# jamshed/CaPS-SA

Measured on AMD Instinct MI355X. Metric: suffixes/sec (SA+LCP build), higher is better.
Workload: dtype u32

## Files before the change

### caps-sa_amd/csrc/kernels.h

```cpp
#pragma once
#include "kernel_lang.h"
#include "text.h"

namespace caps {

#ifndef CAPS_TILE_E
#define CAPS_TILE_E 4096
#endif
#ifndef CAPS_TILE_NT
#define CAPS_TILE_NT 1024
#endif
#ifndef CAPS_TILE_WAVES
#define CAPS_TILE_WAVES 8
#endif
#ifndef CAPS_LOCK_K
#define CAPS_LOCK_K 4
#endif
constexpr uint32_t TILE_E = CAPS_TILE_E;
constexpr uint32_t TILE_NT = CAPS_TILE_NT;
constexpr uint32_t TILE_EPT = TILE_E / TILE_NT;
constexpr uint32_t LOCK_K = CAPS_LOCK_K < TILE_EPT ? CAPS_LOCK_K : TILE_EPT;
#define TILE_WAVES_PER_SIMD CAPS_TILE_WAVES
#ifdef CAPS_NO_WAVES_BOUND
#undef LAUNCH_BOUNDS2
// ... 557 lines not shown
#else
    constexpr uint32_t BPT = NBINS / TILE_NT;
    static_assert(BPT >= 1 && BPT * TILE_NT == NBINS, "counters per thread");
    __shared__ uint32_t wave_tot[TILE_NT / 64];
    const uint32_t tid = threadIdx.x, lane = tid & 63, wv = tid >> 6;
    uint32_t v[BPT], sum = 0;
    UNROLL
    for (uint32_t i = 0; i < BPT; ++i) { v[i] = h[tid * BPT + i]; sum += v[i]; }
    uint32_t x = sum;
#define CAPS_DPP_ADD(ctrl, rows) x += (uint32_t)__builtin_amdgcn_update_dpp(0, (int)x, ctrl, rows, 0xF, false)
    CAPS_DPP_ADD(0x111, 0xF);
    CAPS_DPP_ADD(0x112, 0xF);
    CAPS_DPP_ADD(0x114, 0xF);
    CAPS_DPP_ADD(0x118, 0xF);
    CAPS_DPP_ADD(0x142, 0xA);
    CAPS_DPP_ADD(0x143, 0xC);
#undef CAPS_DPP_ADD
    if (lane == 63) wave_tot[wv] = x;
    SYNC_LDS();
    uint32_t run = x - sum;
    if (TILE_NT / 64 <= 16) {
        const uint32_t wt = lane < TILE_NT / 64 ? wave_tot[lane] : 0u;
        uint32_t ws = wt;
#define CAPS_DPP_ADD(ctrl) ws += (uint32_t)__builtin_amdgcn_update_dpp(0, (int)ws, ctrl, 0xF, 0xF, false)
        CAPS_DPP_ADD(0x111);
        CAPS_DPP_ADD(0x112);
        CAPS_DPP_ADD(0x114);
        CAPS_DPP_ADD(0x118);
#undef CAPS_DPP_ADD
        const int wvs = __builtin_amdgcn_readfirstlane((int)wv);
        run += (uint32_t)__builtin_amdgcn_readlane((int)ws, wvs) - (uint32_t)__builtin_amdgcn_readlane((int)wt, wvs);
    } else {
        for (uint32_t w = 0; w < wv; ++w) run += wave_tot[w];
    }
    UNROLL
    for (uint32_t i = 0; i < BPT; ++i) { h[tid * BPT + i] = run; run += v[i]; }
    if (tid == TILE_NT - 1) h[NBINS] = run;
    SYNC_LDS();
#endif
}
DEV_INLINE void block_exclusive_scan_bins(KCTX uint32_t* hist) { block_exclusive_scan<TILE_BINS_>(KCTX_PASS hist); }

template <typename idx_t> struct FinalOut {
    idx_t* sa = nullptr;
    idx_t* lcp = nullptr;
    uint64_t* first_key = nullptr;
    uint64_t* last_key = nullptr;
    idx_t* first_sa = nullptr;
    idx_t* last_sa = nullptr;
};

#ifdef CAPS_EMUL
extern "C" void caps_emul_count_tile(bool fast, bool known_range);
extern "C" void caps_emul_count_tile2(bool two_level_ok);
extern "C" void caps_emul_count_tile3(bool equalised_ok);
#endif
constexpr uint32_t TILE_BINS = TILE_BINS_;
#ifndef CAPS_TILE_BIN_LIMIT
#define CAPS_TILE_BIN_LIMIT 48
#endif
#ifndef CAPS_EQ_BIN_LIMIT
#define CAPS_EQ_BIN_LIMIT 128
#endif
constexpr uint32_t TILE_BIN_LIMIT = CAPS_TILE_BIN_LIMIT;
constexpr uint32_t EQ_BIN_LIMIT = CAPS_EQ_BIN_LIMIT;

template <typename idx_t>
DEV_INLINE uint64_t lcp_capped(uint32_t l, uint64_t n, idx_t a, idx_t b)
{
    if (sizeof(idx_t) == 4) {
        const uint32_t room = (uint32_t)n - (uint32_t)(a > b ? a : b);
        return l < room ? l : room;
    }
    const uint64_t room = n - (uint64_t)(a > b ? a : b);
    return l < room ? l : room;
}
template <int BITS, bool RUNS, typename idx_t>
DEV_INLINE uint64_t tile_pair_lcp(const uint32_t* __restrict__ P, uint64_t n, uint64_t ka, idx_t a, uint64_t kb, idx_t b, uint32_t)
{
    const uint64_t x = ka ^ kb;
    if (x) return lcp_capped<idx_t>((uint32_t)caps_clz64(x) / BITS, n, a, b);
    return pair_lcp<BITS, RUNS>(P, n, ka, (uint64_t)a, kb, (uint64_t)b);
}
template <int BITS, bool RUNS, typename idx_t>
DEV_INLINE uint64_t tile_pair_lcp(const uint32_t* __restrict__ P, uint64_t n, uint32_t ka, idx_t a, uint32_t kb, idx_t b, uint32_t cs)
{
    return pair_lcp32<BITS, RUNS>(P, n, ka, (uint64_t)a, kb, (uint64_t)b, cs);
}

template <typename idx_t> HD idx_t tie_sentinel() { return (idx_t)~(idx_t)0; }
template <int BITS, bool RUNS, typename idx_t>
DEV_INLINE uint64_t deferring_pair_lcp(const uint32_t* __restrict__ P, uint64_t n, uint64_t* __restrict__ bflag, uint32_t g, uint64_t ka, idx_t a,
                                       uint64_t kb, idx_t b)
{
    if (bflag && ka == kb) { bflag[g] = 1; return (uint64_t)tie_sentinel<idx_t>(); }
    return tile_pair_lcp<BITS, RUNS>(P, n, ka, a, kb, b, 0u);
}

#if defined(CAPS_PHASE_CLOCK) && !defined(CAPS_EMUL)
__device__ unsigned long long caps_phase_clock[32];
#define PHASE_T0() unsigned long long pc_t_ = clock64()
#define PHASE_MARK(i) do { const unsigned long long t_ = clock64(); if (threadIdx.x == 0) atomicAdd(&caps_phase_clock[i], t_ - pc_t_); pc_t_ = clock64(); } while (0)
#else
#define PHASE_T0() ((void)0)
#define PHASE_MARK(i) ((void)0)
#endif

#if defined(CAPS_EQ_CHECK) && !defined(CAPS_EMUL)
__device__ unsigned int caps_eq_check[64];
#define EQ_OK(ok, id) ((ok) ? true : (atomicAdd(&caps_eq_check[id], 1u), false))
#else
#define EQ_OK(ok, id) (true)
#endif
#define EQ_CHK(ok, id) ((void)EQ_OK((ok), (id)))

DEV_INLINE const uint64_t* tile_src(const uint64_t* in, const uint64_t* out, bool from_out) { return from_out ? out : in; }
DEV_INLINE const uint32_t* tile_src(const uint32_t* in, const uint64_t*, bool) { return in; }

#define TILE_SORT_PROLOGUE                                                                                      \
    const uint32_t b = K_BLOCK_IDX;                                                                             \
    if (b >= sd.tile_off[sd.G]) return;                                                                         \
    const uint32_t g = sd.tile_rec[b].g;                                                                          \
    const TileInfo t = tile_info(sd, b);                                                                        \
    const uint64_t start = t.s0 + (uint64_t)t.tl * TILE_E;                                                      \
    const uint32_t cnt = (uint32_t)(t.s1 - start < TILE_E ? t.s1 - start : TILE_E);                             \
     \
     \
    const bool with_lcp = lcp_mode != 0 && (t.s1 - t.s0) <= TILE_E;                                             \
     \
     \
    const bool direct = with_lcp && fin.sa != nullptr;                                                          \
     \
     \
     \
     \
     \
     \
    const uint64_t in0 = slot_cap ? (uint64_t)g * slot_cap : start;
#define TILE_OUTGROWN (slot_cap != 0 && t.s1 - t.s0 > (uint64_t)slot_cap)

#define TILE_SRC_KEY in_key
#define TILE_SRC_SA in_sa
#define TILE_SORT_LOAD                                                                                          \
    PAR(tid) {                                                                                                  \
        if (tid == 0) { kmm[0] = ~0ull; kmm[1] = 0; flag[0] = 0; }                                              \
        for (uint32_t i = tid; i <= TILE_BINS; i += K_BLOCK_DIM) hist[i] = 0;                                   \
        UNROLL                                                                                                  \
        for (uint32_t k = 0; k < TILE_EPT; ++k) {                                                               \
            const uint32_t e = tid + k * TILE_NT;                                                               \
            if (e < cnt) {                                                                                      \
                uint64_t key;                                                                                   \
                idx_t sa;                                                                                       \
                if (FROM_TEXT) {                                                                                \
                    key = window64<BITS>(P, text_base + start + e);                                             \
                    sa = (idx_t)(text_base + start + e);                                                        \
                } else if (TILE_KEYS_FROM_TEXT) {    \
                    sa = STREAM_LOAD(&TILE_SRC_SA[in0 + e]);                                                    \
                    key = window64<BITS>(P, (uint64_t)sa);                                                      \
                } else {                                                                                        \
                    key = STREAM_LOAD(&TILE_SRC_KEY[in0 + e]);                                                  \
                    sa = STREAM_LOAD(&TILE_SRC_SA[in0 + e]);                                                    \
                }                                                                                               \
                TL(rk, tid, k) = (decltype(TL(rk, tid, k) + 0))key;                                             \
                TL(rs, tid, k) = sa;                                                                            \
            }                                                                                                   \
        }                                                                                                       \
    }

#define TILE_SYNC() SYNC()
#define TILE_SORT_RANGE                                                                                         \
    const bool known_range = seg_map != nullptr;                                                                \
    if (!known_range) {                                                                                         \
        TILE_SYNC();                                                                       \
        PAR(tid) {                                                                                              \
            uint64_t mn = ~0ull, mx = 0;                                                                        \
            UNROLL                                                                                              \
            for (uint32_t k = 0; k < TILE_EPT; ++k) {                                                           \
                const uint32_t e = tid + k * TILE_NT;                                                           \
                if (e < cnt) {                                                                                  \
                    const uint64_t key = (uint64_t)TL(rk, tid, k);                                              \
                    mn = key < mn ? key : mn;                                                                   \
                    mx = key > mx ? key : mx;                                                                   \
                }                                                                                               \
            }                                                                                                   \
            BLOCK_MINMAX_U64(&kmm[0], &kmm[1], mn, mx);                                                         \
        }                                                                                                       \
    }                                                                                                           \
    TILE_SYNC();                                                                                                \
    const BucketParams tb = known_range ? seg_map[g] : make_bucket_params(kmm[0], kmm[1], TILE_BINS);

#define TILE_SORT_PLACE_FINAL                                                                                   \
    PAR(tid) {                                                                                                  \
        UNROLL                                                                                                  \
        for (uint32_t k = 0; k < TILE_EPT; ++k) {                                                               \
            const uint32_t e = tid + k * TILE_NT;                                                               \
            if (e < cnt) {                                                                                      \
                const uint32_t d = TL(rd, tid, k);                                                              \
                skey[d] = TL(rk, tid, k);                                                                       \
                ssa[d] = TL(rs, tid, k);                                                                        \
            }                                                                                                   \
        }                                                                                                       \
    }                                                                                                           \
    TILE_SYNC();

#define TILE_SORT_EMIT TILE_SORT_EMIT_(0u)
#define TILE_EMIT_LCP_(ka, a, kb, b) tile_pair_lcp<BITS, TILE_RUNS>(P, n, ka, a, kb, b, TILE_KEY_SHIFT)
#define TILE_SORT_EMIT_(OV)                                                                                     \
    PAR(tid) {                                                                                                  \
        UNROLL                                                                                                  \
        for (uint32_t k = 0; k < TILE_EPT; ++k) {                                                               \
            const uint32_t e = tid + k * TILE_NT;                                                               \
            if (e < cnt) {                                                                                      \
                const uint64_t key = skey[e];                                                                   \
                const idx_t sa = ssa[e];                                                                        \
                uint64_t l = 0;                                                                                 \
                if (with_lcp && e) {                                                                            \
                    const uint32_t ov_ = (OV);                                                                  \
                    l = ov_ ? ov_ : TILE_EMIT_LCP_(skey[e - 1], ssa[e - 1], skey[e], sa);                          \
                }                                                                                               \
                if (direct) {                                                                                   \
                    STREAM_STORE(&fin.sa[start + e], sa);                                                       \
                    STREAM_STORE(&fin.lcp[start + e], (idx_t)l);                                                \
                    if (e == 0) { fin.first_key[g] = key; fin.first_sa[g] = sa; }                               \
                    if (e == cnt - 1) { fin.last_key[g] = key; fin.last_sa[g] = sa; }                           \
                } else {                                                                                        \
                    out_key[start + e] = key;                                                                   \
                    out_sa[start + e] = sa;                                                                     \
                    if (with_lcp) out_lcp[start + e] = (idx_t)l;                                                \
                }                                                                                               \
            }                                                                                                   \
        }                                                                                                       \
    }

template <typename idx_t, int BITS, bool FROM_TEXT, typename KT = uint64_t>
GLOBAL_FN LAUNCH_BOUNDS2(TILE_NT, TILE_WAVES_PER_SIMD) tile_sort_kernel(KCTX SegDesc sd, const uint32_t* __restrict__ P, uint64_t n,
                                                  uint64_t text_base, uint32_t lcp_mode, uint32_t slot_cap, const KT* in_key,
                                                  const idx_t* in_sa, uint64_t* out_key, idx_t* out_sa, idx_t* out_lcp,
                                                  FinalOut<idx_t> fin, const BucketParams* __restrict__ seg_map,
                                                  uint32_t* __restrict__ redo, const uint8_t* __restrict__ kshift)
{
    constexpr bool TILE_RUNS = false;
    constexpr bool K32 = sizeof(KT) == 4;
    constexpr bool TILE_KEYS_FROM_TEXT = false;
    static_assert(!K32 || !FROM_TEXT, "32-bit keys come from the slots of level B");
    TILE_SORT_PROLOGUE
    const uint32_t TILE_KEY_SHIFT = K32 ? kshift[g] : 0u;
    const uint32_t tie_from = K32 ? (TILE_KEY_SHIFT + 32u) / BITS : TextTraits<BITS>::KCH;
    SHARED_ARRAY(KT, skey, TILE_E);
    SHARED_ARRAY(idx_t, ssa, TILE_E);
    SHARED_ARRAY(uint32_t, hist, TILE_BINS + 1);
    SHARED_ARRAY(uint64_t, kmm, 2);
    SHARED_ARRAY(uint32_t, flag, 1);
    constexpr bool SLOT_ORDER = sizeof(idx_t) == 4;
    SHARED_ARRAY(uint16_t, sbin, SLOT_ORDER ? TILE_E : 1);
    SHARED_ARRAY(uint16_t, perm, SLOT_ORDER ? TILE_E : 1);
    TL_DECL(KT, rk, TILE_EPT);
    TL_DECL(idx_t, rs, TILE_EPT);
    TL_DECL(uint32_t, rd, TILE_EPT);
    TL_DECL(uint32_t, rb, TILE_EPT);

    PHASE_T0();
    TILE_SORT_LOAD
    TILE_SORT_RANGE
    PHASE_MARK(0);
    bool fast = cnt > 1 && tb.range > 0;
    if (fast) {
        PAR(tid) {
            UNROLL
            for (uint32_t k = 0; k < TILE_EPT; ++k) {
                const uint32_t e = tid + k * TILE_NT;
                if (e < cnt) {
                    const uint32_t bin = bucket_of(tb, TL(rk, tid, k));
                    const uint32_t r = FETCH_ADD_U32(&hist[bin], 1u);
                    if (r >= TILE_BIN_LIMIT) flag[0] = 1;
                    TL(rb, tid, k) = bin;
                    TL(rd, tid, k) = r;
                }
            }
        }
        SYNC();
        fast = flag[0] == 0;
        PHASE_MARK(1);
    }
    if (cnt == 1) {
        PAR(tid) { if (tid == 0) { skey[0] = TL(rk, tid, 0); ssa[0] = TL(rs, tid, 0); } }
        SYNC();
        fast = true;
    } else if (fast) {
        block_exclusive_scan_bins(KCTX_PASS hist);
        PHASE_MARK(2);
        PAR(tid) {
            UNROLL
            for (uint32_t k = 0; k < TILE_EPT; ++k) {
                const uint32_t e = tid + k * TILE_NT;
                if (e < cnt) {
                    const uint32_t slot = hist[TL(rb, tid, k)] + TL(rd, tid, k);
                    skey[slot] = TL(rk, tid, k);
                    ssa[slot] = TL(rs, tid, k);
                    if (SLOT_ORDER) sbin[slot] = (uint16_t)TL(rb, tid, k);
                    else TL(rd, tid, k) = slot;
                }
            }
        }
        SYNC();
        PHASE_MARK(3);
        PAR(tid) {
            UNROLL
            for (uint32_t k = 0; k < TILE_EPT; ++k) {
                const uint32_t e = tid + k * TILE_NT;
                if (e < cnt) {
                    const uint32_t slot = SLOT_ORDER ? e : TL(rd, tid, k), bin = SLOT_ORDER ? (uint32_t)sbin[slot] : TL(rb, tid, k);
                    const uint32_t bs = hist[bin], be = hist[bin + 1];
                    const uint64_t key = SLOT_ORDER ? (uint64_t)skey[slot] : (uint64_t)TL(rk, tid, k);
                    uint32_t less = 0;
                    for (uint32_t j = bs; j < be; ++j) {
                        const uint64_t kj = skey[j];
                        less += kj < key ? 1u : 0u;
                        if (kj == key && j != slot) {
                            const uint64_t sa = SLOT_ORDER ? (uint64_t)ssa[slot] : (uint64_t)TL(rs, tid, k);
                            const uint32_t c = suffix_less_tie_bounded<BITS>(P, n, (uint64_t)ssa[j], sa, tie_from);
                            if (c == 2u) flag[0] = 1;
                            less += c & 1u;
                        }
                    }
                    if (SLOT_ORDER) RACY_STORE_U16(&perm[bs + less], (uint16_t)slot);
                    else TL(rd, tid, k) = bs + less;
                }
            }
        }
        SYNC();
        fast = flag[0] == 0;
        PHASE_MARK(4);
        if (fast && !SLOT_ORDER) {
            TILE_SORT_PLACE_FINAL
            PHASE_MARK(5);
        }
    }
#ifdef CAPS_EMUL
    caps_emul_count_tile(fast, known_range);
#endif
    if (!fast) {
        PAR(tid) { if (tid == 0) redo[1 + FETCH_ADD_U32(&redo[0], 1u)] = b; }
        return;
    }
    if (SLOT_ORDER && cnt > 1) {
        PAR(tid) {
            UNROLL
            for (uint32_t k = 0; k < TILE_EPT; ++k) {
                const uint32_t e = tid + k * TILE_NT;
                if (e < cnt) {
                    const uint32_t sl = perm[e];
                    const KT key = skey[sl];
                    const idx_t sa = ssa[sl];
                    uint64_t l = 0;
                    if (with_lcp && e) { const uint32_t sp = perm[e - 1]; l = TILE_EMIT_LCP_(skey[sp], ssa[sp], key, sa); }
                    if (direct) {
                        STREAM_STORE(&fin.sa[start + e], sa);
                        STREAM_STORE(&fin.lcp[start + e], (idx_t)l);
                        if (e == 0) { fin.first_key[g] = key; fin.first_sa[g] = sa; }
                        if (e == cnt - 1) { fin.last_key[g] = key; fin.last_sa[g] = sa; }
                    } else {
                        out_key[start + e] = key;
                        out_sa[start + e] = sa;
                        if (with_lcp) out_lcp[start + e] = (idx_t)l;
                    }
                }
            }
        }
    } else {
        TILE_SORT_EMIT
    }
    PHASE_MARK(6);
}

GLOBAL_FN LAUNCH_BOUNDS(256) hot_tiles_kernel(KCTX SegDesc sd, uint32_t slot_cap, TileInfo* __restrict__ hot)
{
    PAR(tid) {
        const uint32_t nt = sd.tile_off[sd.G];
        const uint32_t i = K_BLOCK_IDX * K_BLOCK_DIM + tid;
        if (i < nt) {
            TileInfo t = sd.tile_rec[i];
            if (t.s1 - t.s0 > (uint64_t)slot_cap) { t.s1 = t.s0; t.tl = 0; }
            hot[i] = t;
        }
    }
}

GLOBAL_FN LAUNCH_BOUNDS(256) queue_all_tiles_kernel(KCTX SegDesc sd, uint32_t* __restrict__ redo)
{
    PAR(tid) {
        const uint32_t nt = sd.tile_off[sd.G];
        const uint32_t i = K_BLOCK_IDX * K_BLOCK_DIM + tid;
        if (i < nt) redo[1 + i] = i;
        if (i == 0) redo[0] = nt;
    }
}

#ifndef CAPS_EQ_ROUNDS
#define CAPS_EQ_ROUNDS 2
#endif
constexpr uint32_t EQ_ROUNDS = CAPS_EQ_ROUNDS;
#ifndef CAPS_TIE_G1
#define CAPS_TIE_G1 8
#endif
#ifndef CAPS_TIE_LIST_MAX
#define CAPS_TIE_LIST_MAX 2
#endif
constexpr uint32_t TIE_G1 = CAPS_TIE_G1;
constexpr uint32_t TIE_G2 = 64;
constexpr uint32_t TIE_LIST_CAP = TILE_E / 8;
constexpr uint32_t TIE_LIST_MAX = CAPS_TIE_LIST_MAX;
constexpr uint32_t TIE_DEEP_CAP = 64;
constexpr uint32_t TIE_VDEEP_CAP = 32;
constexpr uint32_t TIE_BIG_CAP = 1024;
constexpr uint32_t TIE_BIG_LANES = 64;
constexpr uint32_t EQ_FRAC_BITS = 13;
static_assert((uint64_t)TILE_BINS_ << EQ_FRAC_BITS <= (1u << 24), "positions fit 24 bits");

DEV_INLINE uint32_t eq_pos(const BucketParams& bp, uint64_t key)
{
    const uint32_t top = (bp.B << EQ_FRAC_BITS) - 1u;
    if (key <= bp.kmin) return 0;
    const uint64_t d = key - bp.kmin;
    if (d >= bp.range) return top;
    const uint32_t d32 = (uint32_t)((d << bp.shift) >> 32);
    const uint64_t prod = (uint64_t)d32 * bp.m;
    const uint32_t sh = 32u + bp.post;
    const uint32_t x = (uint32_t)(sh >= EQ_FRAC_BITS ? prod >> (sh - EQ_FRAC_BITS) : prod << (EQ_FRAC_BITS - sh));
    return x < top ? x : top;
}

DEV_INLINE uint32_t eq_big_lcp(const uint16_t* vslot, const uint32_t* vlcp, uint32_t cnt, uint32_t e)
{
    uint32_t l = 0;
    for (uint32_t q = 0; q < cnt && q < TIE_VDEEP_CAP; ++q)
        if (vslot[q] == e) l = vlcp[q];
    return l;
}

template <int BITS, bool TEXT, typename idx_t>
DEV_INLINE uint64_t eq_emit_lcp(const uint32_t* __restrict__ P, uint64_t n, uint64_t ka, idx_t a, uint64_t kb, idx_t b, uint32_t* lost, bool test_drop)
{
    if (TEXT) return pair_lcp<BITS, false>(P, n, ka, (uint64_t)a, kb, (uint64_t)b);
    const uint64_t x = ka ^ kb;
    if (x == 0) {
#ifdef CAPS_EMUL
        if (!test_drop) { std::fprintf(stderr, "eq_emit_lcp: neighbours %llu, %llu with equal keys and no lcp from the tie phases\n", (unsigned long long)a, (unsigned long long)b); std::abort(); }
#endif
        *lost = 1;
    }
    return lcp_capped<idx_t>(x ? (uint32_t)caps_clz64(x) / BITS : TextTraits<BITS>::KCH, n, a, b);
}

#ifndef CAPS_EQ_WAVES
#define CAPS_EQ_WAVES TILE_WAVES_PER_SIMD
// ... 1058 lines not shown
        PAR(tid) {
            const uint32_t x = tid & 31, y = tid >> 5;
            for (uint32_t yy = y; yy < 32; yy += 8)
                if (r0 + yy < rows && c0 + x < cols) tile[yy * 33 + x] = in[(uint64_t)(r0 + yy) * cols + c0 + x];
        }
        SYNC();
        PAR(tid) {
            const uint32_t x = tid & 31, y = tid >> 5;
            for (uint32_t yy = y; yy < 32; yy += 8)
                if (c0 + yy < cols && r0 + x < rows) out[(uint64_t)(c0 + yy) * rows + r0 + x] = tile[x * 33 + yy];
        }
        SYNC();
    }
}

template <typename idx_t>
DEV_INLINE uint32_t run_of(const idx_t* row, uint32_t lo, uint32_t hi, uint64_t x)
{
    while (lo < hi) {
        const uint32_t mid = (lo + hi + 1) >> 1;
        if ((uint64_t)row[mid] <= x) lo = mid; else hi = mid - 1;
    }
    return lo;
}

template <typename idx_t>
GLOBAL_FN LAUNCH_BOUNDS(256) runs_plan_kernel(KCTX SegDesc sd, const idx_t* __restrict__ rulerT, uint32_t G1,
                                              uint32_t* __restrict__ first_run)
{
    PAR(tid) {
        const uint64_t b = (uint64_t)K_BLOCK_IDX * K_BLOCK_DIM + tid;
        if (b < sd.tile_off[sd.G]) {
            const uint32_t j = sd.tile_rec[b].g;
            const TileInfo t = tile_info(sd, (uint32_t)b);
            first_run[b] = run_of<idx_t>(rulerT + (uint64_t)j * G1, 0u, G1 - 1, (uint64_t)t.tl * TILE_E);
        }
    }
}

#define RUNS_TILE_SETUP                                                                                         \
    const uint32_t run_a = FROM_RUNS ? rsrc.first_run[b] : 0u;                                                  \
    const uint32_t run_b = !FROM_RUNS ? 0u : (start + cnt >= t.s1) ? rsrc.G1 - 1 : rsrc.first_run[b + 1];       \
    const uint32_t run_ns = run_b - run_a + 1;                                                                  \
    const bool runs_staged = run_ns <= TILE_E;                                                                  \
    const idx_t* run_rowR = rsrc.rulerT + (uint64_t)g * rsrc.G1;                                                \
    const idx_t* run_rowA = rsrc.PmT + (uint64_t)g * rsrc.G1;                                                   \
    const uint64_t run_x0 = start - t.s0;                                                                       \
    (void)run_a; (void)run_b; (void)run_ns; (void)runs_staged; (void)run_rowR; (void)run_rowA; (void)run_x0;

#define RUNS_STAGE(tid)                                                                                         \
    if (runs_staged)                                                                                            \
        for (uint32_t k = tid; k < run_ns; k += K_BLOCK_DIM) {                                                  \
            const idx_t r = run_rowR[run_a + k];                                                                \
            lrow[k] = r;                                                                                        \
            lsrc[k] = rsrc.sub_start[run_a + k] + (uint64_t)run_rowA[run_a + k] - (uint64_t)r;                  \
        }

template <typename idx_t>
DEV_INLINE uint64_t run_source(const RunSrc<idx_t>& rsrc, bool staged, const idx_t* lrow, const uint64_t* lsrc, uint32_t ns,
                               const idx_t* rowR, const idx_t* rowA, uint32_t ga, uint32_t gb, uint64_t x)
{
    if (staged) return lsrc[run_of<idx_t>(lrow, 0u, ns - 1, x)] + x;
    const uint32_t r = run_of<idx_t>(rowR, ga, gb, x);
    return rsrc.sub_start[r] + (uint64_t)rowA[r] + (x - (uint64_t)rowR[r]);
}

constexpr int SRC_ARRAYS = 0, SRC_TEXT = 1, SRC_RUNS = 2;

#ifndef CAPS_BUCKET_EIGHTHS
#define CAPS_BUCKET_EIGHTHS 7
#endif
#ifndef CAPS_SCATTER_SWZ
#define CAPS_SCATTER_SWZ 1
#endif
#ifndef CAPS_COLLATE_SWZ
#define CAPS_COLLATE_SWZ 0
#endif
#ifndef CAPS_TILE_SWZ
#define CAPS_TILE_SWZ 0
#endif
constexpr uint32_t BUCKET_TARGET = (TILE_E * CAPS_BUCKET_EIGHTHS) / 8;
constexpr uint32_t BUCKET_LDS = TILE_BINS_;

DEV_INLINE void key32_range(uint64_t& kmin, uint64_t& kmax, bool kmin_exclusive, uint32_t cs)
{
    const uint64_t lo = kmin_exclusive ? kmin + 1 : kmin;
    if (lo > kmax || (kmin_exclusive && kmin == ~0ull)) { kmin = kmax = 0; return; }
    kmin = key32_of(lo, cs);
    kmax = key32_of(kmax, cs);
}

GLOBAL_FN LAUNCH_BOUNDS(256) bucket_plan_kernel(KCTX const uint64_t* __restrict__ seg_start, const uint64_t* __restrict__ seg_end,
                                                uint32_t G, uint32_t range_mode,
                                                const uint64_t* __restrict__ pkey, uint32_t part_off, uint32_t part_total,
                                                uint32_t enable, uint32_t fine, uint32_t sub,
                                                BucketParams* __restrict__ bp, uint64_t* __restrict__ segB,
                                                const uint8_t* __restrict__ gshift)
{
    PAR(tid) {
        const uint32_t g = K_BLOCK_IDX * K_BLOCK_DIM + tid;
        if (g < G) {
            const uint32_t parent = g / sub, first = parent * sub;
            uint64_t len = 0;
            for (uint32_t x = 0; x < sub && first + x < G; ++x) len += seg_end_of(seg_start, seg_end, first + x) - seg_start[first + x];
            uint64_t kmin = 0, kmax = ~0ull;
            if (range_mode >= 1) {
                const uint32_t j = part_off + parent;
                if (j > 0) kmin = pkey[j - 1];
                if (j + 1 < part_total) kmax = pkey[j];
                if (range_mode == 2) key32_range(kmin, kmax, j > 0, gshift[j]);
            }
            uint32_t B = 1;
            if (enable && len > TILE_E && kmax > kmin) B = (uint32_t)((len + BUCKET_TARGET - 1) / BUCKET_TARGET);
            if (sub > 1 && B < 2) B = 2;
            if (fine > 1 && B > 1 && B <= BUCKET_LDS) {
                const uint32_t k = BUCKET_LDS / B < fine ? BUCKET_LDS / B : fine;
                B *= k;
            }
            const BucketParams q = make_bucket_params(kmin, kmax, B);
            bp[g] = q;
            segB[g] = (g % sub == sub - 1 || g == G - 1) ? B : 0;
        }
    }
}

GLOBAL_FN LAUNCH_BOUNDS(256) bucket_group_kernel(KCTX uint32_t G, const uint64_t* __restrict__ segB, const uint64_t* __restrict__ bstart,
                                                 const uint64_t* __restrict__ fsegB, const uint64_t* __restrict__ fstart,
                                                 const uint64_t* __restrict__ fcount, uint64_t* __restrict__ count,
                                                 uint32_t* __restrict__ gfirst)
{
    SHARED_ARRAY(uint64_t, fc, BUCKET_LDS);
    for (uint32_t g = K_BLOCK_IDX; g < G; g += K_GRID_DIM) {
        const uint32_t B = (uint32_t)segB[g], F = (uint32_t)fsegB[g];
        const uint64_t b0 = bstart[g], f0 = fstart[g];
        if (B > BUCKET_LDS || F <= B || F > BUCKET_LDS) {
            PAR(tid) {
                for (uint32_t i = tid; i < B; i += K_BLOCK_DIM) { count[b0 + i] = i < F ? fcount[f0 + i] : 0; gfirst[b0 + i] = i; }
            }
            continue;
        }
        PAR(tid) { for (uint32_t f = tid; f < F; f += K_BLOCK_DIM) fc[f] = fcount[f0 + f]; }
        SYNC();
        PAR(tid) {
            if (tid == 0) {
                uint64_t cap = TILE_E, total = 0;
                for (uint32_t f = 0; f < F; ++f) total += fc[f];
                for (uint64_t lo = TILE_E, hi = total > TILE_E ? total : TILE_E;;) {
                    const uint64_t c_try = lo == TILE_E ? lo : (lo + hi) / 2;
                    uint32_t need = 1;
                    uint64_t run = 0;
                    for (uint32_t f = 0; f < F; ++f) {
                        const uint64_t c = fc[f];
                        if (run > 0 && run + c > c_try) { ++need; run = 0; }
                        run += c;
                    }
                    if (need <= B) { cap = c_try; hi = c_try; if (c_try == TILE_E) break; }
                    else lo = c_try + 1;
                    if (lo >= hi) { cap = hi; break; }
                }
                uint32_t gi = 0;
                uint64_t sum = 0;
                gfirst[b0] = 0;
                for (uint32_t f = 0; f < F; ++f) {
                    const uint64_t c = fc[f];
                    if (sum > 0 && sum + c > cap && gi + 1 < B) {
                        count[b0 + gi] = sum;
                        ++gi;
                        gfirst[b0 + gi] = f;
                        sum = 0;
                    }
                    sum += c;
                }
                count[b0 + gi] = sum;
                for (uint32_t i = gi + 1; i < B; ++i) { count[b0 + i] = 0; gfirst[b0 + i] = F; }
            }
        }
        SYNC();
    }
}

GLOBAL_FN LAUNCH_BOUNDS(256) bucket_ranges_kernel(KCTX const uint64_t* __restrict__ bstart, uint32_t G,
                                                  const BucketParams* __restrict__ bps, const uint64_t* __restrict__ pkey,
                                                  uint32_t range_mode, uint32_t part_off, uint32_t part_total, uint32_t sub,
                                                  BucketParams* __restrict__ tile_map,
                                                  const BucketParams* __restrict__ fbps, const uint32_t* __restrict__ gfirst,
                                                  const uint8_t* __restrict__ gshift, uint8_t* __restrict__ kshift)
{
    PAR(tid) {
        const uint64_t i = (uint64_t)K_BLOCK_IDX * K_BLOCK_DIM + tid;
        if (i < bstart[G]) {
            uint32_t a = 0, b = G;
            while (b - a > 1) {
                const uint32_t mid = (a + b) / 2;
                if (bstart[mid] <= i) a = mid; else b = mid;
            }
            const uint32_t g = a;
            const BucketParams bp = bps[g];
            uint64_t kmin = 0, kmax = ~0ull;
            if (range_mode >= 1) {
                const uint32_t j = part_off + g / sub;
                if (j > 0) kmin = pkey[j - 1];
                if (j + 1 < part_total) kmax = pkey[j];
                if (range_mode == 2) { key32_range(kmin, kmax, j > 0, gshift[j]); kshift[i] = gshift[j]; }
            }
            const uint32_t bk = (uint32_t)(i - bstart[g]);
            const double range1 = (double)(kmax - kmin) + 1.0;
            uint64_t l = kmin, h = kmax;
            if (bp.B > 1) {
                uint32_t lo = bk, hi = bk + 1, div = bp.B;
                if (gfirst) {
                    div = fbps[g].B;
                    lo = gfirst[i];
                    hi = bk + 1 < bp.B ? gfirst[i + 1] : div;
                    if (hi <= lo) hi = lo + 1;
                }
                const double dl = (double)lo / (double)div * range1, dh = (double)hi / (double)div * range1;
                if (lo > 0) l = kmin + (uint64_t)dl;
                if (hi < div) h = kmin + (uint64_t)dh;
                if (h < l) h = l;
            }
            tile_map[i] = make_bucket_params(l, h, TILE_BINS);
        }
    }
}

constexpr uint32_t TEXT_WIN = TILE_E / 4 + 24;
constexpr uint32_t SPLIT_LUT_BITS = TILE_E >= 4096 ? 12 : TILE_E >= 256 ? 8 : 4;
constexpr uint32_t SPLIT_LUT_CELLS = 1u << SPLIT_LUT_BITS;

template <int BITS> HD uint64_t text_win_base(uint64_t pos0) { return pos0 / TextTraits<BITS>::CPW; }

constexpr int MAP_LINEAR = 0, MAP_GROUPED = 1, MAP_SPLIT = 2;
HD uint32_t lds_swz(uint32_t i) { return i ^ ((i >> 4) & 15u) ^ ((i >> 8) & 15u); }
#ifdef CAPS_GA_NO_SWZ
#define GA_SWZ(i) (i)
#else
#define GA_SWZ(i) lds_swz(i)
#endif
constexpr uint32_t COUNT_CHUNK = 8;

template <typename idx_t, int BITS, int SRC, int MAP = MAP_LINEAR>
GLOBAL_FN LAUNCH_BOUNDS(TILE_NT) bucket_count_kernel(KCTX SegDesc sd, const uint32_t* __restrict__ P, uint64_t n_words,
                                                     uint64_t text_base, const uint64_t* __restrict__ in_key, RunSrc<idx_t> rsrc,
                                                     const BucketParams* __restrict__ bps, const uint64_t* __restrict__ bstart,
                                                     uint64_t* __restrict__ count, const uint64_t* __restrict__ split,
                                                     uint32_t split_stride, uint32_t in_sub, uint16_t* __restrict__ bid)
{
    constexpr bool FROM_TEXT = SRC == SRC_TEXT, FROM_RUNS = SRC == SRC_RUNS;
    SHARED_ARRAY(uint32_t, hist, BUCKET_LDS);
    SHARED_ARRAY(uint64_t, stab, MAP == MAP_SPLIT ? BUCKET_LDS : 1);
    SHARED_ARRAY(uint32_t, twin, FROM_TEXT ? TEXT_WIN : 1);
    SHARED_ARRAY(uint64_t, lsrc, FROM_RUNS ? TILE_E : 1);
    SHARED_ARRAY(idx_t, lrow, FROM_RUNS ? TILE_E : 1);
    const uint32_t n_tiles = sd.tile_off[sd.G];
    const uint32_t want = n_tiles / (4u * K_GRID_DIM);
    const uint32_t CH = want < 1u ? 1u : want > COUNT_CHUNK ? COUNT_CHUNK : want;
    const uint32_t n_chunks = (n_tiles + CH - 1) / CH;
    for (uint32_t v = K_BLOCK_IDX; v < n_chunks; v += K_GRID_DIM) {
    uint64_t cur_b0 = ~0ull;
    uint32_t cur_B = 0;
    const uint32_t b_end = (v + 1) * CH < n_tiles ? (v + 1) * CH : n_tiles;
    for (uint32_t b = v * CH; b < b_end; ++b) {
        const uint32_t g = sd.tile_rec[b].g;
        const TileInfo t = tile_info(sd, b);
        const uint64_t start = t.s0 + (uint64_t)t.tl * TILE_E;
        const uint32_t cnt = (uint32_t)(t.s1 - start < TILE_E ? t.s1 - start : TILE_E);
        const BucketParams bp = bps[g];
        const uint64_t b0 = bstart[g];
        if (bp.B == 1) {
            PAR(tid) { if (tid == 0) ATOMIC_ADD_U64(&count[b0], (uint64_t)cnt); }
            continue;
        }
        const bool lds = bp.B <= BUCKET_LDS;
        const uint64_t w0 = text_win_base<BITS>(text_base + start);
        RUNS_TILE_SETUP
        const uint32_t n_split = MAP == MAP_SPLIT ? bp.B - 1 : 0u;
        const uint64_t* tab = MAP == MAP_SPLIT ? split + (uint64_t)(g / in_sub) * split_stride : nullptr;
        const bool fresh = !lds || b0 != cur_b0 || bp.B != cur_B;
        PAR(tid) {
            if (fresh) {
                for (uint32_t i = tid; i < cur_B; i += K_BLOCK_DIM)
                    if (hist[i]) ATOMIC_ADD_U64(&count[cur_b0 + i], (uint64_t)hist[i]);
                if (lds) for (uint32_t i = tid; i < bp.B; i += K_BLOCK_DIM) hist[i] = 0;
                if (MAP == MAP_SPLIT && lds) for (uint32_t i = tid; i < n_split; i += K_BLOCK_DIM) stab[lds_swz(i)] = tab[i];
            }
            if (FROM_TEXT)
// ... 338 lines not shown
                    STREAM_STORE2(&out_key[dst], skey[q]);
                    STREAM_STORE2(&out_sa[dst], ssa[q]);
                }
            }
        }
        if (SPILL) {
            const uint32_t nl = nlong[0];
            for (uint32_t r = 0; r < nl && r < SPILL_LONG_CAP; ++r) {
                const uint64_t at = lr_at[r];
                const idx_t old = lr_old[r];
                const uint32_t c = lr_c[r], bb = lr_b[r];
                for (uint32_t j = tid; j < c; j += K_BLOCK_DIM) { spill.bucket[at + j] = bb; spill.rel[at + j] = (idx_t)(old + j); }
            }
        }
    }
}

template <typename idx_t>
GLOBAL_FN LAUNCH_BOUNDS(256) spill_gather_kernel(KCTX const uint64_t* __restrict__ seg_start, uint32_t NB, uint64_t slot_cap,
                                                 const uint8_t* __restrict__ skip, const uint64_t* __restrict__ slot_key,
                                                 const idx_t* __restrict__ slot_sa, uint64_t* __restrict__ dst_key,
                                                 idx_t* __restrict__ dst_sa)
{
    SHARED_ARRAY(uint32_t, lst, 256);
    SHARED_ARRAY(uint32_t, ln, 1);
    for (uint64_t base = (uint64_t)K_BLOCK_IDX * 256u; base < NB; base += (uint64_t)K_GRID_DIM * 256u) {
        PAR(tid) { if (tid == 0) ln[0] = 0; }
        SYNC();
        PAR(tid) {
            const uint64_t b = base + tid;
            if (b < NB) {
                const uint64_t len = seg_start[b + 1] - seg_start[b];
                if (len > slot_cap || (len && skip && skip[b])) lst[FETCH_ADD_U32(&ln[0], 1u)] = (uint32_t)b;
            }
        }
        SYNC();
        const uint32_t m = ln[0];
        for (uint32_t q = 0; q < m; ++q) {
            const uint32_t b = lst[q];
            const uint64_t s0 = seg_start[b], len = seg_start[b + 1] - s0;
            const uint64_t cnt = len < slot_cap ? len : slot_cap;
            PAR(tid) {
                for (uint64_t i = tid; i < cnt; i += K_BLOCK_DIM) {
                    dst_key[s0 + i] = slot_key[(uint64_t)b * slot_cap + i];
                    dst_sa[s0 + i] = slot_sa[(uint64_t)b * slot_cap + i];
                }
            }
        }
        SYNC();
    }
}

template <typename idx_t>
GLOBAL_FN LAUNCH_BOUNDS(256) spill_place_kernel(KCTX Spill<idx_t> sp, uint64_t cnt, const uint64_t* __restrict__ seg_start,
                                                uint64_t* __restrict__ dst_key, idx_t* __restrict__ dst_sa)
{
    PAR(tid) {
        for (uint64_t i = (uint64_t)K_BLOCK_IDX * K_BLOCK_DIM + tid; i < cnt; i += (uint64_t)K_GRID_DIM * K_BLOCK_DIM) {
            const uint32_t b = sp.bucket[i];
            if (b == ~0u) continue;
            const uint64_t d = seg_start[b] + (uint64_t)sp.rel[i];
            dst_key[d] = sp.key[i];
            dst_sa[d] = sp.sa[i];
        }
    }
}

#ifndef CAPS_GA_TILES
#define CAPS_GA_TILES 4
#endif
constexpr uint32_t GA_TILES = CAPS_GA_TILES;
constexpr uint32_t GA_E = GA_TILES * TILE_E;
constexpr uint32_t GA_EPT = GA_E / TILE_NT;
static_assert(GA_E <= (1u << 14) && BUCKET_LDS <= (1u << 11), "group << 14 | position fits a register");

template <typename idx_t, int BITS, typename KT = uint64_t>
GLOBAL_FN LAUNCH_BOUNDS2(TILE_NT, TILE_WAVES_PER_SIMD) group_scatter_kernel(KCTX const uint32_t* __restrict__ P, uint64_t n_words,
                                                      uint64_t text_base, uint64_t len, const uint64_t* __restrict__ split, uint32_t K1,
                                                      const uint16_t* __restrict__ split_lut, const uint32_t* __restrict__ split_span,
                                                      uint32_t sub, uint64_t slot_cap, idx_t* __restrict__ cursor,
                                                      KT* __restrict__ out_key, idx_t* __restrict__ out_sa,
                                                      uint32_t tile_first, uint32_t tile_stride,
                                                      const uint64_t* __restrict__ region_start, const uint64_t* __restrict__ region_cap,
                                                      const uint8_t* __restrict__ gshift, uint32_t own_lo, uint32_t own_hi)
{
    constexpr bool K32 = sizeof(KT) == 4;
    constexpr uint32_t DROP = ~0u;
    SHARED_ARRAY(uint8_t, scs, K32 ? BUCKET_LDS : 1);
    constexpr uint32_t CPW = TextTraits<BITS>::CPW;
    constexpr uint32_t WIN = GA_E / CPW + 8;
    const idx_t NO_SLOT = (idx_t)~(idx_t)0;
    SHARED_ARRAY(uint32_t, twin, WIN);
    SHARED_ARRAY(uint64_t, stab, BUCKET_LDS);
    SHARED_ARRAY(uint16_t, slut, SPLIT_LUT_CELLS + 2);
    SHARED_ARRAY(uint32_t, hist, TILE_BINS + 1);
    SHARED_ARRAY(idx_t, obase, TILE_BINS);
    SHARED_ARRAY(uint32_t, perm, TILE_E);
    TL_DECL(uint32_t, pk, GA_EPT);
    const uint64_t start = ((uint64_t)tile_first + (uint64_t)K_BLOCK_IDX * tile_stride) * GA_E;
    if (start >= len) return;
    const uint32_t cnt = (uint32_t)(len - start < GA_E ? len - start : GA_E);
    const uint32_t sx = sub > 1 ? K_BLOCK_IDX % sub : 0u;
    const uint32_t n_split = K1 - 1;
    const uint64_t pos0 = text_base + start;
    const uint64_t w0 = pos0 / CPW;
    const uint32_t top = pow2_above(split_span[0]);
    PAR(tid) {
        for (uint32_t i = tid; i <= TILE_BINS; i += K_BLOCK_DIM) hist[i] = 0;
        for (uint32_t i = tid; i < WIN; i += K_BLOCK_DIM) twin[i] = w0 + i < n_words ? P[w0 + i] : 0u;
        for (uint32_t i = tid; i < n_split; i += K_BLOCK_DIM) stab[GA_SWZ(i)] = split[i];
        for (uint32_t i = tid; i <= SPLIT_LUT_CELLS; i += K_BLOCK_DIM) slut[i] = split_lut[i];
        if (K32) for (uint32_t i = tid; i < K1; i += K_BLOCK_DIM) scs[i] = gshift[i];
    }
    SYNC();
    const bool RUN_OF_POS = BITS == 2 && GA_EPT == CPW && pos0 % CPW == 0;
    PAR(tid) {
        uint64_t wA = 0;
        uint32_t wC = 0;
        if (RUN_OF_POS) {
            const uint32_t wi = (uint32_t)(pos0 / CPW - w0) + tid;
            wA = ((uint64_t)twin[wi] << 32) | twin[wi + 1];
            wC = twin[wi + 2];
        }
        UNROLL
        for (uint32_t kk = 0; kk < GA_EPT; kk += 4) {
            uint64_t key[4];
            uint32_t lo[4], hi[4];
            UNROLL
            for (uint32_t j = 0; j < 4; ++j) {
                const uint32_t e = RUN_OF_POS ? tid * GA_EPT + kk + j : tid + (kk + j) * TILE_NT;
                const uint32_t sh = BITS * (kk + j);
                key[j] = e >= cnt ? 0 : !RUN_OF_POS ? window64<BITS>(twin, pos0 + e - w0 * CPW)
                                                    : sh ? (wA << sh) | (uint64_t)(wC >> (32u - sh)) : wA;
                const uint32_t cell = (uint32_t)(key[j] >> (64 - SPLIT_LUT_BITS));
                lo[j] = slut[cell];
                hi[j] = slut[cell + 1];
            }
            for (uint32_t st = top >> 1; st >= 1; st >>= 1) {
                UNROLL
                for (uint32_t j = 0; j < 4; ++j) {
                    const uint32_t idx = lo[j] + st - 1;
                    const uint64_t mk = stab[GA_SWZ(idx < n_split ? idx : (n_split ? n_split - 1 : 0))];
                    if (idx < hi[j] && mk < key[j]) lo[j] += st;
                }
            }
            UNROLL
            for (uint32_t j = 0; j < 4; ++j) {
                const uint32_t e = RUN_OF_POS ? tid * GA_EPT + kk + j : tid + (kk + j) * TILE_NT;
                uint32_t v = DROP;
                if (e < cnt && lo[j] >= own_lo && lo[j] < own_hi) v = (lo[j] << 14) | FETCH_ADD_U32(&hist[lo[j]], 1u);
                TL(pk, tid, kk + j) = v;
            }
        }
    }
    SYNC();
    constexpr uint32_t GPT = (TILE_BINS + TILE_NT - 1) / TILE_NT;
    TL_DECL(idx_t, co, GPT);
    TL_DECL(uint32_t, cc, GPT);
    PAR(tid) {
        UNROLL
        for (uint32_t j = 0; j < GPT; ++j) {
            const uint32_t i = tid + j * TILE_NT;
            const uint32_t c = i < K1 ? hist[i] : 0u;
            TL(cc, tid, j) = c;
            TL(co, tid, j) = 0;
            if (c) TL(co, tid, j) = caps_fetch_add(&cursor[(uint64_t)sx * K1 + i], (idx_t)c);
        }
    }
    block_exclusive_scan_bins(KCTX_PASS hist);
    PAR(tid) {
        UNROLL
        for (uint32_t k = 0; k < GA_EPT; ++k) {
            const uint32_t v = TL(pk, tid, k), g = v >> 14;
            if (v != DROP) TL(pk, tid, k) = (g << 14) | (hist[g] + (v & 0x3FFFu));
        }
        UNROLL
        for (uint32_t j = 0; j < GPT; ++j) {
            const uint32_t i = tid + j * TILE_NT;
            if (i < K1) {
                const uint32_t c = TL(cc, tid, j);
                idx_t ob = 0;
                if (c) {
                    const idx_t old = TL(co, tid, j);
                    const uint64_t st = (uint64_t)(i - own_lo) * sub + sx;
                    const uint64_t r0 = region_start ? region_start[st] - region_start[0] : st * slot_cap, rc = region_start ? region_cap[st] : slot_cap;
                    ob = (uint64_t)old + c <= rc ? (idx_t)(r0 + old) : NO_SLOT;
                }
                obase[i] = ob;
            }
        }
    }
    const uint32_t kept = hist[TILE_BINS];
    for (uint32_t c0 = 0; c0 < kept; c0 += TILE_E) {
        PAR(tid) {
            UNROLL
            for (uint32_t k = 0; k < GA_EPT; ++k) {
                const uint32_t e = RUN_OF_POS ? tid * GA_EPT + k : tid + k * TILE_NT;
                const uint32_t v = TL(pk, tid, k), q = v & 0x3FFFu;
                if (v != DROP && q - c0 < TILE_E) perm[q - c0] = (v & ~0x3FFFu) | e;
            }
        }
        SYNC_LDS();
        PAR(tid) {
            UNROLL
            for (uint32_t k = 0; k < TILE_EPT; ++k) {
                const uint32_t q = c0 + tid + k * TILE_NT;
                if (q < kept) {
                    const uint32_t v = perm[q - c0], g = v >> 14, e = v & 0x3FFFu;
                    const idx_t ob = obase[g];
                    if (ob != NO_SLOT) {
                        const uint64_t dst = (uint64_t)ob + (q - hist[g]);
                        const uint64_t key = window64<BITS>(twin, pos0 + e - w0 * CPW);
                        STREAM_STORE2(&out_key[dst], K32 ? (KT)key32_of(key, scs[g]) : (KT)key);
                        STREAM_STORE2(&out_sa[dst], (idx_t)(pos0 + e));
                    }
                }
            }
        }
        SYNC_LDS();
    }
}

template <typename idx_t>
GLOBAL_FN LAUNCH_BOUNDS(256) stream_report_kernel(KCTX const idx_t* __restrict__ cursor, uint32_t n_streams, uint64_t cap,
                                                  const uint32_t* __restrict__ flag, uint64_t* __restrict__ out,
                                                  const uint64_t* __restrict__ region_cap, uint32_t K1, uint32_t sub, uint32_t own_lo,
                                                  uint32_t own_hi)
{
    PAR(tid) {
        const uint32_t s = K_BLOCK_IDX * K_BLOCK_DIM + tid;
        if (s < n_streams) {
            const uint64_t z = (uint64_t)cursor[s];
            out[s] = z;
            uint64_t room = cap;
            if (region_cap) {
                const uint32_t g = s % K1, sx = s / K1;
                room = g >= own_lo && g < own_hi ? region_cap[(uint64_t)(g - own_lo) * sub + sx] : 0;
            }
            if (z > room) ATOMIC_MAX_U64(&out[n_streams + 1], z);
        }
        if (s == n_streams) out[n_streams] = flag[0];
    }
}

template <typename idx_t>
GLOBAL_FN LAUNCH_BOUNDS(256) widen_kernel(KCTX const idx_t* __restrict__ in, uint64_t cnt, uint64_t* __restrict__ out)
{
    PAR(tid) {
        const uint64_t i = (uint64_t)K_BLOCK_IDX * K_BLOCK_DIM + tid;
        if (i < cnt) out[i] = (uint64_t)in[i];
    }
}

template <typename idx_t>
GLOBAL_FN LAUNCH_BOUNDS(256) unify_kernel(KCTX SegDesc sd, const uint64_t* __restrict__ key1, const idx_t* __restrict__ sa1,
                                          uint64_t* __restrict__ key0, idx_t* __restrict__ sa0)
{
    const uint32_t b = K_BLOCK_IDX;
    if (b >= sd.tile_off[sd.G]) return;
    const TileInfo t = tile_info(sd, b);
    if ((passes_for(t.s1 - t.s0) & 1u) == 0) return;
    const uint64_t start = t.s0 + (uint64_t)t.tl * TILE_E;
    const uint32_t cnt = (uint32_t)(t.s1 - start < TILE_E ? t.s1 - start : TILE_E);
    PAR(tid) {
        for (uint32_t e = tid; e < cnt; e += K_BLOCK_DIM) {
            key0[start + e] = key1[start + e];
            sa0[start + e] = sa1[start + e];
        }
    }
}

template <typename idx_t>
GLOBAL_FN LAUNCH_BOUNDS(256) sample_kernel(KCTX const uint64_t* __restrict__ seg_start, uint32_t G, uint32_t ppp,
                                           const uint64_t* __restrict__ key, const idx_t* __restrict__ sa,
                                           uint64_t* __restrict__ out_key, idx_t* __restrict__ out_sa)
{
    PAR(tid) {
        const uint64_t t = (uint64_t)K_BLOCK_IDX * K_BLOCK_DIM + tid;
        if (t < (uint64_t)G * ppp) {
            const uint32_t g = (uint32_t)(t / ppp), k = (uint32_t)(t % ppp);
            const uint64_t s0 = seg_start[g], len = seg_start[g + 1] - s0;
            const uint64_t at = s0 + ((uint64_t)(2 * k + 1) * len) / (2 * (uint64_t)ppp);
            out_key[t] = key[at];
            out_sa[t] = sa[at];
        }
    }
}

template <typename idx_t>
GLOBAL_FN LAUNCH_BOUNDS(256) pick_pivots_kernel(KCTX const uint64_t* __restrict__ skey, const idx_t* __restrict__ ssa, uint64_t m,
                                                uint32_t p, uint64_t* __restrict__ pkey, idx_t* __restrict__ psa)
{
    PAR(tid) {
        const uint64_t j = (uint64_t)K_BLOCK_IDX * K_BLOCK_DIM + tid;
        if (j + 1 < p) {
            const uint64_t at = ((j + 1) * m) / p;
            pkey[j] = skey[at];
            psa[j] = ssa[at];
        }
    }
}

DEV_INLINE uint64_t mix64(uint64_t x)
{
    x += 0x9E3779B97F4A7C15ull;
    x = (x ^ (x >> 30)) * 0xBF58476D1CE4E5B9ull;
    x = (x ^ (x >> 27)) * 0x94D049BB133111EBull;
    return x ^ (x >> 31);
}

template <typename idx_t, int BITS>
GLOBAL_FN LAUNCH_BOUNDS(256) sample_text_kernel(KCTX const uint32_t* __restrict__ P, uint64_t pos0, uint64_t len, uint64_t m,
                                                uint64_t* __restrict__ out_key, idx_t* __restrict__ out_sa)
{
    PAR(tid) {
        const uint64_t t = (uint64_t)K_BLOCK_IDX * K_BLOCK_DIM + tid;
        if (t < m) {
            const uint64_t q = len / m, r = len % m;
            const uint64_t lo = t * q + (t * r) / m, hi = (t + 1) * q + ((t + 1) * r) / m;
            const uint64_t pos = pos0 + lo + mix64(t) % (hi - lo);
            out_key[t] = window64<BITS>(P, pos);
            out_sa[t] = (idx_t)pos;
        }
    }
}

GLOBAL_FN LAUNCH_BOUNDS(256) group_keys_kernel(KCTX const uint64_t* __restrict__ pkey, uint32_t p, uint32_t PG, uint32_t K1,
                                               uint64_t* __restrict__ gkey, uint32_t* __restrict__ flag)
{
    PAR(tid) {
        const uint32_t j = K_BLOCK_IDX * K_BLOCK_DIM + tid;
        if (j + 2 < p && pkey[j] >= pkey[j + 1]) {
            flag[0] = 1;
            if (j == 0 || pkey[j - 1] != pkey[j]) {
                uint32_t len = 2;
                while (j + len < p - 1 && pkey[j + len] == pkey[j]) ++len;
#ifdef CAPS_EMUL
                if (len > flag[3]) flag[3] = len;
#else
                atomicMax(&flag[3], len);
#endif
            }
        }
        if (j + 1 < K1) gkey[j] = pkey[(uint64_t)(j + 1) * PG - 1];
        if (j + 1 == K1) gkey[j] = ~0ull;
    }
}

GLOBAL_FN LAUNCH_BOUNDS(256) group_shift_kernel(KCTX const uint64_t* __restrict__ gkey, uint32_t K1, uint8_t* __restrict__ gshift)
{
    PAR(tid) {
        const uint32_t g = K_BLOCK_IDX * K_BLOCK_DIM + tid;
        if (g < K1) {
            const uint64_t lo = g ? gkey[g - 1] + 1 : 0, hi = g + 1 < K1 ? gkey[g] : ~0ull;
            const uint64_t x = lo ^ hi;
            const uint32_t c = x ? (uint32_t)caps_clz64(x) : 32u;
            gshift[g] = (uint8_t)(lo > hi ? 0u : c < 32u ? c : 32u);
        }
    }
}


GLOBAL_FN LAUNCH_BOUNDS(256) split_lut_kernel(KCTX const uint64_t* __restrict__ split, uint32_t n_split, uint16_t* __restrict__ lut,
                                              uint32_t* __restrict__ span)
{
    PAR(tid) {
        const uint32_t c = K_BLOCK_IDX * K_BLOCK_DIM + tid;
        if (c <= SPLIT_LUT_CELLS) {
            uint32_t lo = 0, hi = n_split;
            if (c < SPLIT_LUT_CELLS) {
                const uint64_t cell_lo = (uint64_t)c << (64 - SPLIT_LUT_BITS);
                while (lo < hi) { const uint32_t mid = (lo + hi) >> 1; if (split[mid] < cell_lo) lo = mid + 1; else hi = mid; }
            } else lo = n_split;
            lut[c] = (uint16_t)lo;
            if (c < SPLIT_LUT_CELLS) {
                uint32_t a = lo, z = n_split;
                if (c + 1 < SPLIT_LUT_CELLS) {
                    const uint64_t next_lo = (uint64_t)(c + 1) << (64 - SPLIT_LUT_BITS);
                    while (a < z) { const uint32_t mid = (a + z) >> 1; if (split[mid] < next_lo) a = mid + 1; else z = mid; }
                } else a = n_split;
#ifdef CAPS_EMUL
                if (a - lo > span[0]) span[0] = a - lo;
#else
                if (a > lo) atomicMax(&span[0], a - lo);
#endif
            }
        }
    }
}

template <typename idx_t>
GLOBAL_FN LAUNCH_BOUNDS(256) slot_segments_kernel(KCTX const idx_t* __restrict__ sizes, uint32_t K1, uint32_t sub, uint32_t stream_major,
                                                  uint64_t cap, const uint64_t* __restrict__ region_start,
                                                  const uint64_t* __restrict__ region_cap, uint64_t* __restrict__ seg_start,
                                                  uint64_t* __restrict__ seg_end, uint64_t* __restrict__ total)
{
    PAR(tid) {
        const uint32_t G = K1 * sub;
        const uint32_t s = K_BLOCK_IDX * K_BLOCK_DIM + tid;
        if (s < G) {
            const uint64_t z = (uint64_t)sizes[stream_major ? (uint64_t)(s % sub) * K1 + s / sub : s];
            const uint64_t r0 = region_start ? region_start[s] : (uint64_t)s * cap, rc = region_start ? region_cap[s] : cap;
            seg_start[s] = r0;
            seg_end[s] = r0 + (z < rc ? z : rc);
            ATOMIC_ADD_U64(total, z);
            if (z > rc) ATOMIC_MAX_U64(total + 1, z);
        }
        if (s == G) seg_start[s] = region_start ? region_start[G - 1] + region_cap[G - 1] : (uint64_t)G * cap;
    }
}

constexpr double SKEW_MIN = 0.7;

GLOBAL_FN LAUNCH_BOUNDS(256) skew_probe_kernel(KCTX const uint64_t* __restrict__ pkey, uint32_t p, uint32_t PG, uint32_t K1,
                                               uint32_t* __restrict__ flag)
{
    PAR(tid) {
        const uint32_t j = K_BLOCK_IDX * K_BLOCK_DIM + tid;
        if (j < p) {
            const uint32_t g = j / PG, j0 = g * PG, j1 = (j0 + PG < p ? j0 + PG : p);
            if (j1 - j0 >= 2) {
                const double glo = j0 ? (double)pkey[j0 - 1] : 0.0, ghi = j1 < p ? (double)pkey[j1 - 1] : 18446744073709551615.0;
                const double lo = j ? (double)pkey[j - 1] : 0.0, hi = j + 1 < p ? (double)pkey[j] : 18446744073709551615.0;
                if (ghi > glo && (hi - lo) * (double)(j1 - j0) < SKEW_MIN * (ghi - glo)) flag[0] = 1;
            }
        }
    }
}

GLOBAL_FN LAUNCH_BOUNDS(256) knots_kernel(KCTX const uint64_t* __restrict__ skey, uint64_t m, uint64_t NB, uint32_t KPG, uint32_t K1,
                                          uint64_t* __restrict__ knots, uint64_t* __restrict__ gkey)
{
    PAR(tid) {
        const uint64_t k = (uint64_t)K_BLOCK_IDX * K_BLOCK_DIM + tid;
        if (k < NB) {
            uint64_t v = k + 1 < NB ? skey[((k + 1) * m) / NB] : ~0ull;
            if (k + 2 < NB) {
                const uint64_t nx = skey[((k + 2) * m) / NB];
                const uint64_t pv = k ? skey[(k * m) / NB] : 0;
                if (nx == v && (k == 0 ? v > 0 : pv + 1 < v)) --v;
// ... 1190 lines not shown
```

### caps-sa_amd/csrc/pipeline.h

```cpp
#pragma once
#include <algorithm>
#include <cmath>
#include <cstdlib>
#include <cstdio>
#include <limits>
#include <stdexcept>
#include <string>
#include <vector>

#include "kernels.h"
#include "bounded.h"
#include "../../include/caps_sa_hip.h"

#ifndef CAPS_BACKEND_DEFINED
#include "hip_backend.h"
#endif

namespace caps {

template <typename idx_t> struct ElemBuf {
    uint64_t* key = nullptr;
    idx_t* sa = nullptr;
    idx_t* lcp = nullptr;
    size_t region_bytes = 0;
};

struct Arena {
    char* base = nullptr;
    size_t off = 0;
    template <typename T> T* take(size_t count)
    {
        off = (off + 255) & ~size_t(255);
        T* p = base ? reinterpret_cast<T*>(base + off) : nullptr;
        off += count * sizeof(T);
        return p;
    }
};

struct SegBufs {
    uint64_t* seg_start = nullptr;
    uint64_t* seg_end = nullptr;
    uint32_t* tile_off = nullptr;
    TileInfo* tile_rec = nullptr;
    uint64_t* out2 = nullptr;
    uint32_t G = 0;
    SegDesc desc() const { return SegDesc{seg_start, tile_off, tile_rec, G}; }
};

constexpr uint32_t kMaxPasses = 96;

#ifndef CAPS_DIRECT_SUB
#define CAPS_DIRECT_SUB 8
#endif
constexpr uint32_t DIRECT_SUB = CAPS_DIRECT_SUB;
#ifndef CAPS_BUCKET_Q_32NDS
#define CAPS_BUCKET_Q_32NDS 24
#endif
#ifndef CAPS_QUANTILE_SPB
#define CAPS_QUANTILE_SPB 64
#endif
constexpr uint32_t BUCKET_Q = (TILE_E * CAPS_BUCKET_Q_32NDS) / 32;
constexpr uint32_t QUANTILE_SPB = CAPS_QUANTILE_SPB;

#ifndef CAPS_EQ_FINE
#define CAPS_EQ_FINE 16
#endif
constexpr uint32_t EQ_FINE = CAPS_EQ_FINE;

struct BucketBufs {
    BucketParams* params = nullptr;
    uint64_t* segB = nullptr;
    uint64_t* bstart = nullptr;
    uint64_t* count = nullptr;
    void* cursor = nullptr;
    uint64_t* scan_tmp = nullptr;
    uint64_t *first_key = nullptr, *last_key = nullptr;
    BucketParams* tile_map = nullptr;
    void *first_sa = nullptr, *last_sa = nullptr;
    SegBufs sub;
    BucketParams* fparams = nullptr;
    uint64_t* fsegB = nullptr;
    uint64_t* fstart = nullptr;
    uint64_t* fcount = nullptr;
    uint32_t* gfirst = nullptr;
    uint8_t* kshift = nullptr;
    uint8_t* skip = nullptr;
    uint64_t* run_list = nullptr;
    uint32_t nb_cap = 0;
    uint64_t tile_cap = 0;
    static uint32_t bucket_bound(uint64_t n_elems, uint32_t G) { return (uint32_t)(n_elems / BUCKET_Q + 2 * (uint64_t)G + 2); }
};

template <typename idx_t> struct Plan {
    uint64_t n = 0;
    int text_bits = 8;
    uint32_t p = 0;
    uint32_t ppp = 0;
    uint64_t m = 0;
    uint64_t tile_cap = 0;
    uint32_t* P = nullptr;
    ElemBuf<idx_t> A, B, SA_, SB_;
    uint64_t* pkey = nullptr;
    idx_t* psa = nullptr;
    idx_t* Pm = nullptr;
    idx_t* ruler = nullptr;
    idx_t* PmT = nullptr;
    idx_t* rulerT = nullptr;
    uint64_t* sizes = nullptr;
    uint64_t* gkey = nullptr;
    uint64_t* dstat = nullptr;
    idx_t* dcur = nullptr;
    uint16_t* glut = nullptr;
    uint8_t* gshift = nullptr;
    uint64_t* knots = nullptr;
    uint64_t* rcap = nullptr;
    uint64_t* rstart = nullptr;
    uint64_t* partial = nullptr;
    SegBufs seg1, seg2, segS;
    TileDesc* desc = nullptr;
    BucketBufs bk;
    uint64_t* pass_elems = nullptr;
    uint32_t* present = nullptr;
    uint8_t* lut = nullptr;
    size_t bytes = 0;
};

inline void effective_params(uint64_t n, uint64_t p_arg, uint32_t* p_eff, uint32_t* ppp)
{
    uint64_t p = p_arg > 0 ? p_arg : 8192;
    if (n / 16 < p) p = n / 16;
    if (p < 2) { *p_eff = (uint32_t)p; *ppp = 0; return; }
    const uint64_t a = (uint64_t)std::ceil(32.0 * std::log((double)n));
    const uint64_t b = n / p - 1;
    *p_eff = (uint32_t)p;
    *ppp = (uint32_t)(a < b ? a : b);
}

template <typename idx_t>
Plan<idx_t> make_plan(uint64_t n, uint64_t p_arg, char* base, int text_bits = 8)
{
    Plan<idx_t> pl;
    pl.n = n;
    pl.text_bits = text_bits;
    effective_params(n, p_arg, &pl.p, &pl.ppp);
    Arena ar;
    ar.base = base;
    const uint64_t nn = n ? n : 1;
    const bool split = pl.p >= 2;
    const uint32_t p = split ? pl.p : 1;
    const uint32_t gseg = std::max<uint32_t>(p, DIRECT_SUB * std::min<uint32_t>(p, BUCKET_LDS));
    pl.m = split ? (uint64_t)p * pl.ppp : 0;
    pl.bk.nb_cap = BucketBufs::bucket_bound(nn, p);
    pl.bk.tile_cap = nn / TILE_E + pl.bk.nb_cap + 2;
    pl.tile_cap = pl.bk.tile_cap;
    pl.P = ar.take<uint32_t>(text_alloc_words(nn, text_bits));
    for (ElemBuf<idx_t>* b : {&pl.A, &pl.B}) {
        b->key = ar.take<uint64_t>(nn);
        const size_t at = ar.off - nn * sizeof(uint64_t);
        b->sa = ar.take<idx_t>(nn);
        b->lcp = ar.take<idx_t>(nn);
        b->region_bytes = ar.off - at;
    }
    auto segs = [&](SegBufs& s, uint32_t G, uint64_t cap) {
        s.G = G;
        s.seg_start = ar.take<uint64_t>((size_t)G + 1);
        s.tile_off = ar.take<uint32_t>((size_t)G + 1);
        s.tile_rec = ar.take<TileInfo>(cap);
        s.out2 = ar.take<uint64_t>(2);
    };
    segs(pl.seg1, p, pl.tile_cap);
    if (split) {
        for (ElemBuf<idx_t>* b : {&pl.SA_, &pl.SB_}) {
            b->key = ar.take<uint64_t>(pl.m);
            b->sa = ar.take<idx_t>(pl.m);
            b->lcp = ar.take<idx_t>(pl.m);
        }
        pl.pkey = ar.take<uint64_t>(p);
        pl.psa = ar.take<idx_t>(p);
        pl.Pm = ar.take<idx_t>((size_t)p * (p + 1));
        pl.ruler = ar.take<idx_t>((size_t)p * p);
        pl.PmT = ar.take<idx_t>((size_t)p * (p + 1));
        pl.rulerT = ar.take<idx_t>((size_t)p * p);
        pl.sizes = ar.take<uint64_t>(p);
        pl.gkey = ar.take<uint64_t>(p);
        pl.dstat = ar.take<uint64_t>(4);
        pl.dcur = ar.take<idx_t>(gseg);
        pl.glut = ar.take<uint16_t>(SPLIT_LUT_CELLS + 2);
        pl.gshift = ar.take<uint8_t>(gseg);
        pl.knots = ar.take<uint64_t>(pl.bk.nb_cap);
        pl.rcap = ar.take<uint64_t>(gseg);
        pl.rstart = ar.take<uint64_t>((size_t)gseg + 1);
        pl.partial = ar.take<uint64_t>((size_t)PART_CHUNKS * p);
        segs(pl.seg2, gseg, pl.tile_cap);
        pl.seg2.G = p;
        pl.seg2.seg_end = ar.take<uint64_t>((size_t)gseg + 1);
        segs(pl.segS, 1, pl.m / TILE_E + 3);
    }
    pl.desc = ar.take<TileDesc>(pl.tile_cap + 1);
    pl.bk.params = ar.take<BucketParams>(gseg);
    pl.bk.segB = ar.take<uint64_t>(gseg);
    pl.bk.bstart = ar.take<uint64_t>((size_t)gseg + 1);
    pl.bk.count = ar.take<uint64_t>(pl.bk.nb_cap);
    pl.bk.cursor = ar.take<idx_t>(pl.bk.nb_cap);
    pl.bk.scan_tmp = ar.take<uint64_t>(2 * ((size_t)pl.bk.nb_cap / SCAN_CHUNK + 2));
    pl.bk.tile_map = ar.take<BucketParams>(pl.bk.nb_cap);
    pl.bk.first_key = ar.take<uint64_t>(pl.bk.nb_cap);
    pl.bk.last_key = ar.take<uint64_t>(pl.bk.nb_cap);
    pl.bk.first_sa = ar.take<idx_t>(pl.bk.nb_cap);
    pl.bk.last_sa = ar.take<idx_t>(pl.bk.nb_cap);
    segs(pl.bk.sub, pl.bk.nb_cap, pl.bk.tile_cap);
    pl.bk.fparams = ar.take<BucketParams>(gseg);
    pl.bk.fsegB = ar.take<uint64_t>(gseg);
    pl.bk.fstart = ar.take<uint64_t>((size_t)gseg + 1);
    pl.bk.fcount = ar.take<uint64_t>((size_t)EQ_FINE * pl.bk.nb_cap);
    pl.bk.gfirst = ar.take<uint32_t>(pl.bk.nb_cap);
    pl.bk.kshift = ar.take<uint8_t>(pl.bk.nb_cap);
    pl.bk.skip = ar.take<uint8_t>(pl.bk.nb_cap);
    pl.bk.run_list = ar.take<uint64_t>(1 + 4 * RUN_BUCKET_MAX);
    pl.pass_elems = ar.take<uint64_t>(kMaxPasses);
    pl.present = ar.take<uint32_t>(16);
    pl.lut = ar.take<uint8_t>(256);
    pl.bytes = ar.off + 256;
    return pl;
}

struct KernelClock {
    std::vector<std::pair<BackendEvent, BackendEvent>> spans;
    std::vector<uint64_t> elems;
};

inline int build_lut(const uint32_t present[8], uint8_t lut[256])
{
    int sigma = 0;
    for (int c = 0; c < 256; ++c) sigma += (present[c >> 5] >> (c & 31)) & 1;
    if (sigma <= 4) {
        for (int c = 0; c < 256; ++c) lut[c] = 0xFF;
        int rank = 0;
        for (int v = -128; v < 128; ++v) {
            const int c = v & 0xFF;
            if ((present[c >> 5] >> (c & 31)) & 1) lut[c] = (uint8_t)rank++;
        }
        return 2;
    }
    for (int c = 0; c < 256; ++c) lut[c] = (uint8_t)(c ^ 0x80);
    return 8;
}

#define CAPS_UNPAREN(...) __VA_ARGS__
#define CAPS_LAUNCH_RUNS(kernel, targs, grid, block, be, ...)                                            \
    do {                                                                                                 \
        if ((be).long_runs) CAPS_LAUNCH((kernel<CAPS_UNPAREN targs, true>), grid, block, be, __VA_ARGS__); \
        else CAPS_LAUNCH((kernel<CAPS_UNPAREN targs, false>), grid, block, be, __VA_ARGS__);             \
    } while (0)

inline void build_run_table(Backend& be, uint32_t* P, uint64_t n, int bits)
{
    const uint64_t entries = run_table_entries(n, bits);
    const uint32_t chunks = (uint32_t)run_table_chunks(entries);
    uint64_t* R = run_table_mut(P, n, bits);
    uint64_t* flag = R - 2;
    uint64_t* longest = R - 1;
    uint64_t* head = R + entries;
    uint64_t* carry = head + chunks;
    be.memset(flag, 0, 2 * sizeof(uint64_t));
    const uint64_t want = (entries + 255) / 256;
    const uint32_t grid = (uint32_t)(want < 16384 ? want : 16384);
    if (bits == 2) CAPS_LAUNCH(run_blocks_kernel<2>, grid, 256, be, (const uint32_t*)P, n, entries, R, flag);
    else CAPS_LAUNCH(run_blocks_kernel<8>, grid, 256, be, (const uint32_t*)P, n, entries, R, flag);
    CAPS_LAUNCH(run_chunk_heads_kernel, chunks, RUN_NT, be, (const uint64_t*)R, entries, (const uint64_t*)flag, head);
    CAPS_LAUNCH(run_carry_kernel, 1, 1024, be, (const uint64_t*)head, chunks, (const uint64_t*)flag, carry);
    CAPS_LAUNCH(run_resolve_kernel, chunks, RUN_NT, be, R, entries, (const uint64_t*)flag, (const uint64_t*)carry,
                (uint32_t)(64 / bits), longest);
    uint64_t longest_host = 0;
    be.d2h(&longest_host, longest, sizeof longest_host);
    be.sync();
    be.long_runs = longest_host >= RUN_LONG;
}

struct AlphabetError : std::length_error { AlphabetError() : std::length_error("the text has more than 4 distinct bytes, the workspace was sized for 2-bit codes") {} };
inline int prepare_text(Backend& be, const uint8_t* dT, uint64_t n, uint32_t* P, uint32_t* present_dev, uint8_t* lut_dev, int arena_bits = 8)
{
    auto alphabet = [&](uint64_t len, uint32_t present[8]) {
        be.memset(present_dev, 0, 16 * sizeof(uint32_t));
        const uint64_t want = (len + 16 * 256 - 1) / (16 * 256);
        const uint32_t grid = (uint32_t)(want < 4096 ? (want ? want : 1) : 4096);
        CAPS_LAUNCH(alphabet_kernel, grid, 256, be, dT, len, present_dev);
        be.d2h(present, present_dev, 8 * sizeof(uint32_t));
        be.sync();
    };
    auto pack = [&](int bits, const uint8_t lut[256], uint32_t* bad) {
        be.h2d(lut_dev, lut, 256);
        const uint64_t n_words = packed_words(n, bits);
        const uint64_t want = (n_words / (bits == 2 ? 1 : 4) + 255) / 256 + 1;
        const uint32_t grid = (uint32_t)(want < 65536 ? want : 65536);
        if (bits == 2) CAPS_LAUNCH(pack_kernel<2>, grid, 256, be, dT, n, (const uint8_t*)lut_dev, P, n_words, bad);
        else CAPS_LAUNCH(pack_kernel<8>, grid, 256, be, dT, n, (const uint8_t*)lut_dev, P, n_words, bad);
    };
    uint32_t present[8];
    uint8_t lut[256];
// ... 26 lines not shown
    const uint32_t chunks = (G + SCAN_CHUNK - 1) / SCAN_CHUNK;
    uint64_t* sums = tmp;
    uint64_t* offs = tmp + chunks + 1;
    CAPS_LAUNCH((block_scan_kernel<OutT>), chunks ? chunks : 1, 1024, be, in, (uint64_t)G, out, sums);
    CAPS_LAUNCH(scan_sizes_kernel, 1, 1024, be, (const uint64_t*)sums, chunks, offs);
    CAPS_LAUNCH((add_offsets_kernel<OutT>), chunks ? chunks : 1, 1024, be, out, (uint64_t)G, (const uint64_t*)offs, chunks);
}

#ifdef CAPS_EMUL
constexpr uint32_t kSmallScan = 48;
#else
constexpr uint32_t kSmallScan = 32768;
#endif

inline void prepare_segments(Backend& be, const SegBufs& s, uint64_t tile_bound, uint64_t* big_tmp = nullptr,
                             uint64_t* big_cnt = nullptr, bool use_end = false, const uint8_t* skip = nullptr)
{
    be.memset(s.out2, 0, 2 * sizeof(uint64_t));
    const uint64_t* send = use_end ? s.seg_end : nullptr;
    if (s.G <= kSmallScan || !big_tmp) {
        CAPS_LAUNCH(seg_prepare_kernel, 1, 1024, be, (const uint64_t*)s.seg_start, send, s.G, s.tile_off, s.out2, skip);
    } else {
        CAPS_LAUNCH(tile_count_kernel, (s.G + 255) / 256, 256, be, (const uint64_t*)s.seg_start, send, s.G, big_cnt, s.out2, skip);
        device_exclusive_scan<uint32_t>(be, big_cnt, s.G, s.tile_off, big_tmp);
        CAPS_LAUNCH(tile_total_kernel, 1, 64, be, (const uint32_t*)s.tile_off, s.G, s.out2);
    }
    const uint32_t grid = (uint32_t)((tile_bound + 255) / 256);
    CAPS_LAUNCH(tile_map_kernel, grid ? grid : 1, 256, be, (const uint64_t*)s.seg_start, send, (const uint32_t*)s.tile_off, s.G, s.tile_rec);
}

inline uint32_t tiles_of(uint64_t len) { return (uint32_t)((len + TILE_E - 1) / TILE_E); }

template <typename idx_t> struct SortResult {
    ElemBuf<idx_t> buf[2];
    uint32_t passes = 0;
    bool skip_finished = false;
    bool unified = false;
    bool k32 = false;
    bool failed = false;
    SegBufs segs;
    struct RunBucket { uint64_t s0, s1, key; };
    std::vector<RunBucket> run_buckets;
    SegBufs run_tables;
    const BucketBufs* run_bk = nullptr;
    TileDesc* run_desc = nullptr;
    uint64_t total = 0;
    uint64_t* defer_flags = nullptr;
    TileDesc* defer_desc = nullptr;
    uint64_t cap = 0;
    mutable bool msd_failed = false;
    KernelClock* finish_clock = nullptr;
    KernelClock* runb_clock = nullptr;
    KernelClock* msd_clock = nullptr;
    mutable uint64_t msd_groups = 0, msd_elems = 0;
    mutable uint32_t msd_levels = 0;
    uint32_t n_tiles = 0;
    FinalOut<idx_t> fin;
    ElemBuf<idx_t> uniform() const { return unified ? buf[0] : buf[passes & 1]; }
    PingPong<idx_t> pingpong() const
    {
        PingPong<idx_t> pp;
        for (int i = 0; i < 2; ++i) { pp.key[i] = buf[i].key; pp.sa[i] = buf[i].sa; pp.lcp[i] = buf[i].lcp; }
        return pp;
    }
};

struct SortOpts {
    bool from_text = false;
    uint64_t text_base = 0;
    bool need_lcp = false;
    bool skip_finished = false;
    bool no_equalise = false;
    const BucketBufs* bk = nullptr;
    uint32_t range_mode = 0;
    const uint64_t* pkey = nullptr;
    uint32_t part_off = 0, part_total = 0;
    bool speculate = false;
    uint32_t* slot_stats = nullptr;
    bool seg_ends = false;
    uint32_t sub = 1;
    const uint64_t* in_key = nullptr;
    const void* in_sa = nullptr;
    const uint8_t* gshift = nullptr;
    bool k32 = false;
    bool keys_only = false;
    bool comparison_only = false;
    bool skewed_keys = false;
    const uint64_t* knots = nullptr;
    uint32_t knots_per_parent = 0;
    bool knots_have_prev = false;
    bool spill_slots = false;
    TileInfo* hot_tile_rec = nullptr;
    uint64_t* spill_stats = nullptr;
    uint64_t in_extent = 0;
    const SegBufs* run_tables = nullptr;
    uint64_t* defer_flags = nullptr;
    const void* runs = nullptr;
    bool unify = false;
    void* final_sa = nullptr;
    void* final_lcp = nullptr;
    struct { uint64_t *first_key, *last_key; void *first_sa, *last_sa; } bnd = {nullptr, nullptr, nullptr, nullptr};
    KernelClock* tile_clock = nullptr;
    KernelClock* merge_clock = nullptr;
    KernelClock* scatter_clock = nullptr;
    KernelClock* count_clock = nullptr;
    uint64_t* pass_counters = nullptr;
};

template <typename idx_t, int BITS>
SortResult<idx_t> segmented_sort(Backend& be, const uint32_t* P, uint64_t n, TileDesc* desc, const SegBufs& s, uint32_t n_tiles,
                                 uint64_t max_len, ElemBuf<idx_t> cur, ElemBuf<idx_t> oth, uint64_t n_elems, const SortOpts& o)
{
    if (o.keys_only) {
        if (o.from_text || o.need_lcp || o.runs) throw std::invalid_argument("a keys-only sort takes (key, index) arrays and emits no LCPs");
        n = 0;
    }
    SortResult<idx_t> r;
    r.buf[0] = cur;
    r.buf[1] = oth;
    r.skip_finished = o.skip_finished;
    r.segs = s;
    r.n_tiles = n_tiles;
    if (n_tiles == 0) return r;
    const bool dbg = std::getenv("CAPS_SA_DEBUG") != nullptr;
    auto mark = [&](const char* what) { if (dbg) { be.sync(); std::fprintf(stderr, "[sort] %s\n", what); } };
    bool from_text = o.from_text;
    const BucketParams* seg_map = nullptr;
    SegBufs segs = s;
    bool skip = o.skip_finished;
    uint32_t slot_cap = 0;
    uint64_t* slot_key = nullptr;
    idx_t* slot_sa = nullptr;
    if (o.bk && (max_len > TILE_E || o.seg_ends)) {
        const BucketBufs& bk = *o.bk;
        const SegDesc psd = s.desc();
        const uint64_t* s_end = o.seg_ends ? (const uint64_t*)s.seg_end : (const uint64_t*)nullptr;
        const bool by_knots = o.knots != nullptr;
        if (by_knots) {
            const uint64_t NB = (uint64_t)(s.G / o.sub) * o.knots_per_parent;
            if (NB > bk.nb_cap) throw std::invalid_argument("more knot buckets than the bucket tables hold");
            CAPS_LAUNCH(knot_plan_kernel, (s.G + 255) / 256, 256, be, s.G, o.sub, o.knots_per_parent, bk.params, bk.segB);
            CAPS_LAUNCH(scan_sizes_kernel, 1, 1024, be, (const uint64_t*)bk.segB, s.G, bk.bstart);
            CAPS_LAUNCH(knot_ranges_kernel, (uint32_t)((NB + 255) / 256), 256, be, o.knots, NB, bk.tile_map, o.knots_have_prev ? 1u : 0u);
        } else {
        CAPS_LAUNCH(bucket_plan_kernel, (s.G + 255) / 256, 256, be, (const uint64_t*)s.seg_start, s_end, s.G, o.range_mode, o.pkey, o.part_off,
                    o.part_total ? o.part_total : s.G, 1u, 1u, o.sub,
                    bk.params, bk.segB, o.gshift);
        CAPS_LAUNCH(scan_sizes_kernel, 1, 1024, be, (const uint64_t*)bk.segB, s.G, bk.bstart);
        CAPS_LAUNCH(bucket_ranges_kernel, (bk.nb_cap + 255) / 256, 256, be, (const uint64_t*)bk.bstart, s.G,
                    (const BucketParams*)bk.params, o.pkey, o.range_mode, o.part_off, o.part_total ? o.part_total : s.G, o.sub,
                    bk.tile_map, (const BucketParams*)nullptr, (const uint32_t*)nullptr, o.gshift, bk.kshift);
        }
        seg_map = bk.tile_map;
        mark("bucket plan");
        const uint32_t pgrid = n_tiles < be.persistent_blocks() ? n_tiles : be.persistent_blocks();
        const bool runs = o.runs != nullptr;
        const RunSrc<idx_t> rsrc = runs ? *static_cast<const RunSrc<idx_t>*>(o.runs) : RunSrc<idx_t>();
        const uint64_t n_words = from_text ? packed_words(n, BITS) : 0;
        const uint64_t tbase = from_text ? o.text_base : 0;
        const uint64_t* src_key = o.in_key ? o.in_key : (const uint64_t*)cur.key;
        const idx_t* src_sa = o.in_key ? static_cast<const idx_t*>(o.in_sa) : (const idx_t*)cur.sa;
        uint16_t* bid = nullptr;
        if (by_knots && o.in_extent && !from_text && !o.runs && oth.region_bytes && !std::getenv("CAPS_SA_NO_BUCKET_IDS")) {
            const size_t room = (size_t)((reinterpret_cast<char*>(oth.key) + oth.region_bytes) - reinterpret_cast<char*>(oth.lcp));
            const uint64_t extent = o.in_key ? o.in_extent : n_elems;
            if (room >= extent * sizeof(uint16_t)) bid = reinterpret_cast<uint16_t*>(oth.lcp);
        }
        auto scatter = [&](const uint64_t* sub_start, uint32_t cap, uint64_t* okey, idx_t* osa, bool grouped = false) {
            const BucketParams* fbps = grouped ? bk.fparams : nullptr;
            const uint32_t* gfirst = grouped ? bk.gfirst : nullptr;
            BackendEvent s0 = be.record();
#define CAPS_SCATTER_LAUNCH(SRC_, MAP_, ikey, isa)                                                                          \
            CAPS_LAUNCH((bucket_scatter_kernel<idx_t, BITS, SRC_, MAP_>), n_tiles, TILE_NT, be, psd, P, n_words, tbase, ikey, isa, rsrc, \
                        (const BucketParams*)bk.params, (const uint64_t*)bk.bstart, sub_start, (uint64_t)cap, static_cast<idx_t*>(bk.cursor),       \
                        okey, osa, fbps, gfirst, o.knots, (const uint16_t*)nullptr, (const uint32_t*)nullptr, 1u, o.knots_per_parent, o.sub, \
                        (const uint16_t*)bid, Spill<idx_t>())
            const uint64_t* nokey = nullptr;
            const idx_t* nosa = nullptr;
            if (from_text) { if (grouped) CAPS_SCATTER_LAUNCH(SRC_TEXT, MAP_GROUPED, nokey, nosa); else CAPS_SCATTER_LAUNCH(SRC_TEXT, MAP_LINEAR, nokey, nosa); }
            else if (runs) { if (grouped) CAPS_SCATTER_LAUNCH(SRC_RUNS, MAP_GROUPED, src_key, src_sa);
                             else CAPS_SCATTER_LAUNCH(SRC_RUNS, MAP_LINEAR, src_key, src_sa); }
            else if (by_knots) CAPS_SCATTER_LAUNCH(SRC_ARRAYS, MAP_SPLIT, src_key, src_sa);
            else { if (grouped) CAPS_SCATTER_LAUNCH(SRC_ARRAYS, MAP_GROUPED, src_key, src_sa);
                   else CAPS_SCATTER_LAUNCH(SRC_ARRAYS, MAP_LINEAR, src_key, src_sa); }
#undef CAPS_SCATTER_LAUNCH
            BackendEvent s1 = be.record();
            if (o.scatter_clock) { o.scatter_clock->spans.push_back({s0, s1}); o.scatter_clock->elems.push_back(n_elems); }
        };
        uint64_t out2[2] = {0, 0};
        auto adopt_buckets = [&]() {
            device_exclusive_scan<uint64_t>(be, bk.count, bk.nb_cap, bk.sub.seg_start, bk.scan_tmp);
        };
        const bool run_buckets = by_knots && o.need_lcp && o.final_sa && bk.skip && !std::getenv("CAPS_SA_NO_RUN_BUCKETS") &&
                                 n < (1ull << RunKey<(int)sizeof(idx_t)>::RB);
        auto bucket_tiles = [&]() {
            segs = bk.sub;
            segs.G = bk.nb_cap;
            uint64_t rl[1 + 4 * RUN_BUCKET_MAX];
            if (run_buckets) {
                const uint64_t NB = (uint64_t)(s.G / o.sub) * o.knots_per_parent;
                be.memset(bk.skip, 0, bk.nb_cap);
                be.memset(bk.run_list, 0, sizeof(uint64_t));
                CAPS_LAUNCH(run_bucket_mark_kernel, (uint32_t)((NB + 255) / 256), 256, be, o.knots, NB, o.knots_have_prev ? 1u : 0u, (uint32_t)BITS,
                            (const uint64_t*)bk.sub.seg_start, bk.skip, bk.run_list);
            }
            prepare_segments(be, segs, bk.tile_cap, bk.scan_tmp, bk.count, false, run_buckets ? bk.skip : nullptr);
            be.d2h(out2, segs.out2, sizeof out2);
            if (run_buckets) be.d2h(rl, bk.run_list, sizeof rl);
            be.sync();
            if (run_buckets) {
                const uint64_t cnt = rl[0] < RUN_BUCKET_MAX ? rl[0] : RUN_BUCKET_MAX;
                for (uint64_t j = 0; j < cnt; ++j) r.run_buckets.push_back({rl[2 + 4 * j], rl[3 + 4 * j], rl[4 + 4 * j]});
                std::sort(r.run_buckets.begin(), r.run_buckets.end(),
                          [](const typename SortResult<idx_t>::RunBucket& a, const typename SortResult<idx_t>::RunBucket& b) { return a.s0 < b.s0; });
                r.run_tables = o.run_tables ? *o.run_tables : bk.sub;
                r.run_bk = &bk;
                r.run_desc = desc;
                r.total = n_elems;
            }
        };
        const uint64_t nb_here = std::min<uint64_t>(bk.nb_cap, n_elems / BUCKET_TARGET + 2 * (uint64_t)(s.G / o.sub) + 2);
        const uint64_t slot_elems = nb_here * TILE_E;
        bool slots = false;
        if (by_knots && (from_text || runs)) throw std::invalid_argument("quantile buckets read (key, sa) arrays");
        if (o.k32 && (from_text || runs || by_knots || !o.speculate || !o.in_key || !o.final_sa))
            throw std::invalid_argument("32-bit keys: a slot split of (key32, sa) arrays with direct output");
        const bool can_slot = o.speculate && !by_knots &&
                              oth.region_bytes >= slot_elems * ((o.k32 ? sizeof(uint32_t) : sizeof(uint64_t)) + sizeof(idx_t)) &&
                              slot_elems + TILE_E < (uint64_t)std::numeric_limits<idx_t>::max();
        if (o.k32 && !can_slot) { r.failed = true; return r; }
        if (can_slot) {
            slot_key = oth.key;
            slot_sa = reinterpret_cast<idx_t*>(reinterpret_cast<char*>(oth.key) + slot_elems * sizeof(uint64_t));
            be.memset(bk.cursor, 0, (size_t)bk.nb_cap * sizeof(idx_t));
// ... 21 lines not shown
        }
        if (by_knots && o.spill_slots && o.hot_tile_rec && !from_text && !runs && o.final_sa && o.final_lcp && o.need_lcp &&
            !std::getenv("CAPS_SA_NO_SPILL_SLOTS")) {
            const uint64_t NB = (uint64_t)(s.G / o.sub) * o.knots_per_parent;
            const uint64_t idx_max = (uint64_t)std::numeric_limits<idx_t>::max() - TILE_E - 1;
            char* lcp_lo = reinterpret_cast<char*>((reinterpret_cast<uintptr_t>(o.final_lcp) + 15) & ~uintptr_t(15));
            char* lcp_hi = reinterpret_cast<char*>(static_cast<idx_t*>(o.final_lcp) + n_elems);
            char* sa_lo = reinterpret_cast<char*>((reinterpret_cast<uintptr_t>(o.final_sa) + 15) & ~uintptr_t(15));
            char* sa_hi = reinterpret_cast<char*>(static_cast<idx_t*>(o.final_sa) + n_elems);
            uint64_t scap = 0;
            if (lcp_hi > lcp_lo + 64 && sa_hi > sa_lo + 64)
                scap = std::min<uint64_t>((uint64_t)(lcp_hi - lcp_lo) / sizeof(uint64_t), (uint64_t)(sa_hi - sa_lo - 32) / (2 * sizeof(idx_t) + sizeof(uint32_t)));
            const char* cap_env = std::getenv("CAPS_SA_TEST_SPILL_CAP");
            if (cap_env) scap = std::min<uint64_t>(scap, std::strtoull(cap_env, nullptr, 10));
            uint64_t cap_s = TILE_E;
            if (NB) cap_s = std::min<uint64_t>(cap_s, oth.region_bytes / (sizeof(uint64_t) + sizeof(idx_t)) / NB);
            const uint64_t want_stream = std::min<uint64_t>(scap, n_elems / 8 + 1024);
            if (NB && idx_max > want_stream) cap_s = std::min<uint64_t>(cap_s, (idx_max - want_stream) / NB);
            cap_s &= ~uint64_t(31);
            const char* slot_env = std::getenv("CAPS_SA_TEST_SPILL_SLOT");
            if (slot_env) cap_s = std::min<uint64_t>(cap_s, std::strtoull(slot_env, nullptr, 10));
            const uint64_t slot_total = NB * cap_s;
            if (slot_total < idx_max) scap = std::min<uint64_t>(scap, idx_max - slot_total);
            const bool fits = NB != 0 && NB <= bk.nb_cap && o.knots_per_parent <= BUCKET_LDS && (cap_env ? scap >= 1 : scap >= 1024) && slot_total < idx_max &&
                              (slot_env || cap_s >= (BUCKET_Q / 6) * 7) &&
                              oth.region_bytes >= slot_total * (sizeof(uint64_t) + sizeof(idx_t)) && bk.run_list;
            if (fits) {
                slot_key = oth.key;
                slot_sa = reinterpret_cast<idx_t*>(reinterpret_cast<char*>(oth.key) + slot_total * sizeof(uint64_t));
                Spill<idx_t> sp;
                sp.count = bk.run_list;
                sp.cap = scap;
                sp.base = slot_total;
                sp.key = reinterpret_cast<uint64_t*>(lcp_lo);
                sp.sa = reinterpret_cast<idx_t*>(sa_lo);
                sp.rel = sp.sa + scap;
                sp.bucket = reinterpret_cast<uint32_t*>(sp.rel + scap);
                const uint64_t fixed = (uint64_t)n_tiles * SPILL_CHUNK <= scap / 4 && !std::getenv("CAPS_SA_NO_SPILL_CHUNKS") ? (uint64_t)n_tiles * SPILL_CHUNK : 0;
                sp.chunk = fixed ? SPILL_CHUNK : 0u;
                be.memset(bk.cursor, 0, (size_t)bk.nb_cap * sizeof(idx_t));
                be.h2d(sp.count, &fixed, sizeof(uint64_t));
                if (fixed) be.memset(sp.bucket, 0xFF, (size_t)fixed * sizeof(uint32_t));
                BackendEvent s0 = be.record();
                CAPS_LAUNCH((bucket_scatter_kernel<idx_t, BITS, SRC_ARRAYS, MAP_SPLIT, uint64_t, true>), n_tiles, TILE_NT, be, psd, P, (uint64_t)0,
                            (uint64_t)0, src_key, src_sa, rsrc, (const BucketParams*)bk.params, (const uint64_t*)bk.bstart,
                            (const uint64_t*)nullptr, cap_s, static_cast<idx_t*>(bk.cursor), slot_key, slot_sa,
                            (const BucketParams*)nullptr, (const uint32_t*)nullptr, o.knots, (const uint16_t*)nullptr,
                            (const uint32_t*)nullptr, 1u, o.knots_per_parent, o.sub, (const uint16_t*)nullptr, sp);
                uint64_t spilled = 0;
                be.d2h(&spilled, sp.count, sizeof spilled);
                CAPS_LAUNCH((widen_kernel<idx_t>), (bk.nb_cap + 255) / 256, 256, be, (const idx_t*)static_cast<idx_t*>(bk.cursor),
                            (uint64_t)bk.nb_cap, bk.count);
                adopt_buckets();
                bucket_tiles();
                slots = spilled <= scap;
                if (o.spill_stats) { ++o.spill_stats[slots ? 0 : 1]; o.spill_stats[2] += spilled; }
                if (dbg) std::fprintf(stderr, "[sort] split by knots with slots of %llu: %llu on the stream (room for %llu), largest bucket %llu -> %s\n",
                                      (unsigned long long)cap_s, (unsigned long long)spilled, (unsigned long long)scap, (unsigned long long)out2[1],
                                      slots ? "kept" : "redone");
                if (slots) {
                    const uint32_t ggrid_ = (uint32_t)std::min<uint64_t>((NB + 255) / 256, 16384);
                    CAPS_LAUNCH((spill_gather_kernel<idx_t>), ggrid_, 256, be, (const uint64_t*)bk.sub.seg_start, (uint32_t)NB, cap_s,
                                run_buckets ? (const uint8_t*)bk.skip : (const uint8_t*)nullptr, (const uint64_t*)slot_key, (const idx_t*)slot_sa,
                                cur.key, cur.sa);
                    if (spilled)
                        CAPS_LAUNCH((spill_place_kernel<idx_t>), (uint32_t)std::min<uint64_t>((spilled + 255) / 256, 16384), 256, be, sp, spilled,
                                    (const uint64_t*)bk.sub.seg_start, cur.key, cur.sa);
                    BackendEvent s1 = be.record();
                    if (o.scatter_clock) { o.scatter_clock->spans.push_back({s0, s1}); o.scatter_clock->elems.push_back(n_elems); }
                    slot_cap = (uint32_t)cap_s;
                } else {
                    BackendEvent s1 = be.record();
                    if (o.scatter_clock) { o.scatter_clock->spans.push_back({s0, s1}); o.scatter_clock->elems.push_back(n_elems); }
                }
            }
        }
        if (!slots) {
            const bool equalise = !by_knots && bk.fcount != nullptr && !o.no_equalise && !std::getenv("CAPS_SA_NO_EQUALISE");
            const BucketParams* cparams = bk.params;
            const uint64_t* cstart = bk.bstart;
            uint64_t* ccount = bk.count;
            if (equalise) {
                CAPS_LAUNCH(bucket_plan_kernel, (s.G + 255) / 256, 256, be, (const uint64_t*)s.seg_start, s_end, s.G, o.range_mode, o.pkey, o.part_off,
                            o.part_total ? o.part_total : s.G, 1u, EQ_FINE, o.sub, bk.fparams, bk.fsegB, o.gshift);
                CAPS_LAUNCH(scan_sizes_kernel, 1, 1024, be, (const uint64_t*)bk.fsegB, s.G, bk.fstart);
                be.memset(bk.fcount, 0, (size_t)EQ_FINE * bk.nb_cap * sizeof(uint64_t));
                cparams = bk.fparams;
                cstart = bk.fstart;
                ccount = bk.fcount;
            }
            be.memset(bk.count, 0, (size_t)bk.nb_cap * sizeof(uint64_t));
            be.memset(bk.cursor, 0, (size_t)bk.nb_cap * sizeof(idx_t));
            BackendEvent c0 = be.record();
            const uint64_t* no_tab = nullptr;
            if (from_text)
                CAPS_LAUNCH((bucket_count_kernel<idx_t, BITS, SRC_TEXT>), pgrid, TILE_NT, be, psd, P, n_words, tbase, (const uint64_t*)nullptr, rsrc,
                            cparams, cstart, ccount, no_tab, 0u, 1u, (uint16_t*)nullptr);
            else if (runs)
                CAPS_LAUNCH((bucket_count_kernel<idx_t, BITS, SRC_RUNS>), pgrid, TILE_NT, be, psd, P, n_words, tbase, src_key, rsrc,
                            cparams, cstart, ccount, no_tab, 0u, 1u, (uint16_t*)nullptr);
            else if (by_knots)
                CAPS_LAUNCH((bucket_count_kernel<idx_t, BITS, SRC_ARRAYS, MAP_SPLIT>), pgrid, TILE_NT, be, psd, P, n_words, tbase, src_key, rsrc,
                            cparams, cstart, ccount, o.knots, o.knots_per_parent, o.sub, bid);
            else
                CAPS_LAUNCH((bucket_count_kernel<idx_t, BITS, SRC_ARRAYS>), pgrid, TILE_NT, be, psd, P, n_words, tbase, src_key, rsrc,
                            cparams, cstart, ccount, no_tab, 0u, 1u, (uint16_t*)nullptr);
            if (equalise) {
                CAPS_LAUNCH(bucket_group_kernel, s.G < 16384 ? (s.G ? s.G : 1) : 16384, 256, be, s.G, (const uint64_t*)bk.segB, (const uint64_t*)bk.bstart,
                            (const uint64_t*)bk.fsegB, (const uint64_t*)bk.fstart, (const uint64_t*)bk.fcount, bk.count, bk.gfirst);
                CAPS_LAUNCH(bucket_ranges_kernel, (bk.nb_cap + 255) / 256, 256, be, (const uint64_t*)bk.bstart, s.G,
                            (const BucketParams*)bk.params, o.pkey, o.range_mode, o.part_off, o.part_total ? o.part_total : s.G, o.sub,
                            bk.tile_map, (const BucketParams*)bk.fparams, (const uint32_t*)bk.gfirst, o.gshift, bk.kshift);
            }
            BackendEvent c1 = be.record();
            if (o.count_clock) { o.count_clock->spans.push_back({c0, c1}); o.count_clock->elems.push_back(n_elems); }
            adopt_buckets();
            ElemBuf<idx_t> dst = from_text ? cur : oth;
            scatter((const uint64_t*)bk.sub.seg_start, 0u, dst.key, dst.sa, equalise);
            if (!from_text) {
                std::swap(cur, oth);
                r.buf[0] = cur;
                r.buf[1] = oth;
            }
            bucket_tiles();
        } else if (!slot_cap) {
            slot_cap = TILE_E;
        }
        mark("bucket scatter");
        n_tiles = (uint32_t)out2[0];
        max_len = out2[1];
        if (dbg) std::fprintf(stderr, "[sort] buckets: tiles %u max_len %llu\n", n_tiles, (unsigned long long)max_len);
        from_text = false;
        skip = true;
        r.skip_finished = true;
        r.segs = segs;
        r.n_tiles = n_tiles;
    }
    const SegDesc sd = segs.desc();
    SegDesc sd_hot = sd;
    if (slot_cap && max_len > slot_cap && o.hot_tile_rec) {
        CAPS_LAUNCH(hot_tiles_kernel, (n_tiles + 255) / 256, 256, be, sd, slot_cap, o.hot_tile_rec);
        sd_hot.tile_rec = o.hot_tile_rec;
    } else if (slot_cap && max_len > slot_cap) {
        throw std::invalid_argument("slots with outgrown buckets need room for the second tile table");
    }
    const uint32_t lcp_mode = o.need_lcp ? 1u : 0u;
    FinalOut<idx_t> fin;
    if (o.need_lcp && o.final_sa) {
        fin.sa = static_cast<idx_t*>(o.final_sa);
        fin.lcp = static_cast<idx_t*>(o.final_lcp);
        fin.first_key = o.bnd.first_key;
        fin.last_key = o.bnd.last_key;
        fin.first_sa = static_cast<idx_t*>(o.bnd.first_sa);
        fin.last_sa = static_cast<idx_t*>(o.bnd.last_sa);
    }
    r.fin = fin;
    uint32_t* redo = reinterpret_cast<uint32_t*>(desc);
    uint32_t* redo2 = redo + ((size_t)n_tiles + 2);
    uint32_t* redo3 = redo2 + ((size_t)n_tiles + 2);
    static_assert(sizeof(TileDesc) >= 3 * sizeof(uint32_t) + 1, "three queues fit the descriptor array");
    be.memset(redo, 0, sizeof(uint32_t));
    be.memset(redo2, 0, sizeof(uint32_t));
    be.memset(redo3, 0, sizeof(uint32_t));
    const uint32_t ggrid = n_tiles < 4 * be.persistent_blocks() ? n_tiles : 4 * be.persistent_blocks();
    const bool eq_tiles = !std::getenv("CAPS_SA_NO_EQ_TILES");
    const uint32_t drop = std::getenv("CAPS_SA_TEST_DROP_NOTE") ? 2u : 0u;
    if (!eq_tiles) redo3 = redo2 = redo;
    uint64_t* bflag = o.defer_flags && o.need_lcp && o.final_sa && !o.keys_only && !(o.k32 && slot_cap) ? o.defer_flags : nullptr;
    if (bflag) {
        be.memset(bflag, 0, (size_t)segs.G * sizeof(uint64_t));
        r.defer_flags = bflag;
        r.defer_desc = desc;
    }
    r.total = n_elems;
    r.cap = n_elems;
    auto defer_check = [&](uint32_t tiles_to_compare) {
        if (bflag && (uint64_t)tiles_to_compare * TILE_E > n_elems / 2) { bflag = nullptr; r.defer_flags = nullptr; }
    };
    BackendEvent t0 = be.record();
    if (o.seg_ends && segs.seg_start == s.seg_start)
        throw std::invalid_argument("segments in fixed-capacity regions must be bucketed (results are written compactly)");
    const uint64_t* in_key = slot_cap ? slot_key : (o.in_key && segs.seg_start == s.seg_start) ? o.in_key : cur.key;
    const idx_t* in_sa = slot_cap ? slot_sa : (o.in_key && segs.seg_start == s.seg_start) ? static_cast<const idx_t*>(o.in_sa) : cur.sa;
    const uint8_t* no_shift = nullptr;
    r.k32 = o.k32 && slot_cap != 0;
    if (from_text) {
        CAPS_LAUNCH((tile_sort_kernel<idx_t, BITS, true>), n_tiles, TILE_NT, be, sd, P, n, o.text_base, lcp_mode, 0u,
                    (const uint64_t*)nullptr, (const idx_t*)nullptr, cur.key, cur.sa, cur.lcp, fin, seg_map, redo, no_shift);
        if (eq_tiles) CAPS_LAUNCH((tile_sort_eq_kernel<idx_t, BITS, true>), ggrid, TILE_NT, be, sd, P, n, o.text_base, lcp_mode, 0u,
                    (const uint64_t*)nullptr, (const idx_t*)nullptr, cur.key, cur.sa, cur.lcp, fin, seg_map, (const uint32_t*)redo, redo3, 0u | drop, redo2);
        if (eq_tiles) CAPS_LAUNCH((tile_sort_eq_kernel<idx_t, BITS, true, true>), ggrid, TILE_NT, be, sd, P, n, o.text_base, lcp_mode, 0u,
                    (const uint64_t*)nullptr, (const idx_t*)nullptr, cur.key, cur.sa, cur.lcp, fin, seg_map, (const uint32_t*)redo2, redo3, 0u, (uint32_t*)nullptr);
        CAPS_LAUNCH_RUNS(tile_sort_general_kernel, (idx_t, BITS, true), ggrid, TILE_NT, be, sd, P, n, o.text_base, lcp_mode, 0u,
                    (const uint64_t*)nullptr, (const idx_t*)nullptr, cur.key, cur.sa, cur.lcp, fin, (const uint32_t*)redo3, 0u, bflag);
    } else if (r.k32) {
        CAPS_LAUNCH((tile_sort_kernel<idx_t, BITS, false, uint32_t>), n_tiles, TILE_NT, be, sd, P, n, (uint64_t)0, lcp_mode, slot_cap,
                    reinterpret_cast<const uint32_t*>(in_key), in_sa, cur.key, cur.sa, cur.lcp, fin, seg_map, redo, (const uint8_t*)o.bk->kshift);
        if (eq_tiles) CAPS_LAUNCH((tile_sort_eq_kernel<idx_t, BITS, false>), ggrid, TILE_NT, be, sd, P, n, (uint64_t)0, lcp_mode, slot_cap,
                    (const uint64_t*)nullptr, in_sa, cur.key, cur.sa, cur.lcp, fin, (const BucketParams*)nullptr, (const uint32_t*)redo, redo3, 1u | drop, redo2);
        if (eq_tiles) CAPS_LAUNCH((tile_sort_eq_kernel<idx_t, BITS, false, true>), ggrid, TILE_NT, be, sd, P, n, (uint64_t)0, lcp_mode, slot_cap,
                    (const uint64_t*)nullptr, in_sa, cur.key, cur.sa, cur.lcp, fin, (const BucketParams*)nullptr, (const uint32_t*)redo2, redo3, 1u, (uint32_t*)nullptr);
        CAPS_LAUNCH_RUNS(tile_sort_general_kernel, (idx_t, BITS, false), ggrid, TILE_NT, be, sd, P, n, (uint64_t)0, lcp_mode, slot_cap,
                    (const uint64_t*)nullptr, in_sa, cur.key, cur.sa, cur.lcp, fin, (const uint32_t*)redo3, 1u, bflag);
    } else {
        const bool all_queued = o.skewed_keys && eq_tiles && !o.comparison_only;
        const bool per_tile = all_queued && (uint64_t)n_tiles * TILE_NT <= 0xFFFFFFFFull && !std::getenv("CAPS_SA_EQ_PERSISTENT");
        if (o.comparison_only) {
            CAPS_LAUNCH(queue_all_tiles_kernel, (n_tiles + 255) / 256, 256, be, sd, redo3);
            CAPS_LAUNCH_RUNS(tile_sort_general_kernel, (idx_t, BITS, false), ggrid, TILE_NT, be, sd, P, n, (uint64_t)0, lcp_mode, slot_cap,
                        in_key, in_sa, cur.key, cur.sa, cur.lcp, fin, (const uint32_t*)redo3, 0u, bflag);
        } else {
        if (all_queued && !per_tile) CAPS_LAUNCH(queue_all_tiles_kernel, (n_tiles + 255) / 256, 256, be, sd, redo);
        else if (!all_queued) CAPS_LAUNCH((tile_sort_kernel<idx_t, BITS, false>), n_tiles, TILE_NT, be, sd_hot, P, n, (uint64_t)0, lcp_mode, slot_cap,
                    in_key, in_sa, cur.key, cur.sa, cur.lcp, fin, seg_map, redo, no_shift);
        if (per_tile) {
            CAPS_LAUNCH((tile_sort_eq_kernel<idx_t, BITS, false, false, false>), n_tiles, TILE_NT, be, sd_hot, P, n, (uint64_t)0, lcp_mode, slot_cap,
                        in_key, in_sa, cur.key, cur.sa, cur.lcp, fin, seg_map, (const uint32_t*)nullptr, redo3, 0u | drop, redo2);
            uint32_t qn[2] = {0, 0};
            be.d2h(&qn[0], redo2, sizeof(uint32_t));
            be.d2h(&qn[1], redo3, sizeof(uint32_t));
            be.sync();
            if (qn[0]) CAPS_LAUNCH((tile_sort_eq_kernel<idx_t, BITS, false, true, false>), qn[0], TILE_NT, be, sd, P, n, (uint64_t)0, lcp_mode, slot_cap,
                        in_key, in_sa, cur.key, cur.sa, cur.lcp, fin, seg_map, (const uint32_t*)redo2, redo3, 0u, (uint32_t*)nullptr);
            const uint32_t ng = qn[0] + qn[1];
            if (bflag && qn[0]) {
                uint32_t q3 = 0;
                be.d2h(&q3, redo3, sizeof q3);
                be.sync();
                defer_check(q3);
            } else defer_check(qn[1]);
            if (ng && be.long_runs)
                CAPS_LAUNCH((tile_sort_general_kernel<idx_t, BITS, false, true, false>), ng, TILE_NT, be, sd, P, n, (uint64_t)0, lcp_mode, slot_cap,
                            in_key, in_sa, cur.key, cur.sa, cur.lcp, fin, (const uint32_t*)redo3, 0u, bflag);
            else if (ng)
                CAPS_LAUNCH((tile_sort_general_kernel<idx_t, BITS, false, false, false>), ng, TILE_NT, be, sd, P, n, (uint64_t)0, lcp_mode, slot_cap,
                            in_key, in_sa, cur.key, cur.sa, cur.lcp, fin, (const uint32_t*)redo3, 0u, bflag);
        } else {
            if (eq_tiles) CAPS_LAUNCH((tile_sort_eq_kernel<idx_t, BITS, false>), ggrid, TILE_NT, be, sd_hot, P, n, (uint64_t)0, lcp_mode, slot_cap,
                        in_key, in_sa, cur.key, cur.sa, cur.lcp, fin, seg_map, (const uint32_t*)redo, redo3, 0u | drop, redo2);
            if (eq_tiles) CAPS_LAUNCH((tile_sort_eq_kernel<idx_t, BITS, false, true>), ggrid, TILE_NT, be, sd, P, n, (uint64_t)0, lcp_mode, slot_cap,
                        in_key, in_sa, cur.key, cur.sa, cur.lcp, fin, seg_map, (const uint32_t*)redo2, redo3, 0u, (uint32_t*)nullptr);
            if (bflag) {
                uint32_t ng = 0;
                be.d2h(&ng, redo3, sizeof ng);
                be.sync();
                defer_check(ng);
            }
            CAPS_LAUNCH_RUNS(tile_sort_general_kernel, (idx_t, BITS, false), ggrid, TILE_NT, be, sd, P, n, (uint64_t)0, lcp_mode, slot_cap,
                        in_key, in_sa, cur.key, cur.sa, cur.lcp, fin, (const uint32_t*)redo3, 0u, bflag);
        }
        }
    }
    BackendEvent t1 = be.record();
    mark("tile sort");
    if (dbg) {
        uint32_t q[3] = {0, 0, 0};
        be.d2h(&q[0], redo, 4); be.d2h(&q[1], redo2, 4); be.d2h(&q[2], redo3, 4);
        be.sync();
        std::fprintf(stderr, "[sort] queues after the tile sorts: %u %u %u of %u tiles, deferring %d\n", q[0], q[1], q[2], n_tiles, bflag ? 1 : 0);
    }
    if (o.tile_clock) { o.tile_clock->spans.push_back({t0, t1}); o.tile_clock->elems.push_back(n_elems); }
    const uint32_t grid = n_tiles < be.persistent_blocks() ? n_tiles : be.persistent_blocks();
    ElemBuf<idx_t> a = cur, b = oth;
    uint32_t* n_active = reinterpret_cast<uint32_t*>(desc + n_tiles);
    for (uint64_t R = TILE_E; R < max_len; R *= 2) {
        be.memset(n_active, 0, sizeof(uint32_t));
        CAPS_LAUNCH_RUNS(merge_partition_kernel, (idx_t, BITS), (n_tiles + 255) / 256, 256, be, sd, P, n, R, ~0ull, skip ? 1u : 0u,
                    lcp_mode, (const uint64_t*)a.key, (const idx_t*)a.sa, desc,
                    o.pass_counters ? o.pass_counters + r.passes : (uint64_t*)nullptr, bflag ? 1u : 0u, n_active);
        BackendEvent m0 = be.record();
        CAPS_LAUNCH_RUNS(merge_pass_kernel, (idx_t, BITS), grid, TILE_NT, be, (const TileDesc*)desc, (const uint32_t*)n_active, P, n,
                    (const uint64_t*)a.key, (const idx_t*)a.sa, b.key, b.sa, b.lcp, bflag);
        BackendEvent m1 = be.record();
        if (o.merge_clock) { o.merge_clock->spans.push_back({m0, m1}); o.merge_clock->elems.push_back(n_elems); }
        std::swap(a, b);
        ++r.passes;
        mark("merge pass");
    }
    if (o.unify && r.skip_finished && r.passes) {
        CAPS_LAUNCH((unify_kernel<idx_t>), n_tiles, 256, be, sd, (const uint64_t*)r.buf[1].key, (const idx_t*)r.buf[1].sa,
                    r.buf[0].key, r.buf[0].sa);
        r.unified = true;
    } else if (o.unify && r.skip_finished) {
        r.unified = true;
    }
    return r;
}

template <typename idx_t, int BITS>
void sort_run_buckets(Backend& be, const uint32_t* P, uint64_t n, const SortResult<idx_t>& r, idx_t* dSA, idx_t* dLCP)
{
    for (const auto& rb : r.run_buckets) {
        const uint64_t len = rb.s1 - rb.s0;
        const uint32_t grid = (uint32_t)std::min<uint64_t>((len + 255) / 256, 4096);
        SegBufs t = r.run_tables;
        t.G = 1;
        t.seg_end = nullptr;
// ... 539 lines not shown
            CAPS_LAUNCH((collate_kernel<idx_t>), n_tiles1, TILE_NT, be_, pl_.seg1.desc(), p, (const idx_t*)pl_.Pm,
                        (const idx_t*)pl_.ruler, (const uint64_t*)pl_.seg2.seg_start, (const uint32_t*)tile_plan,
                        (const uint64_t*)cur.key, (const idx_t*)cur.sa, oth.key, oth.sa);
            BackendEvent k1 = be_.record();
            collate_clock_.spans.push_back({k0, k1});
            collate_clock_.elems.push_back(n);
            in2 = oth;
            out2buf = cur;
        }
        e5_ = be_.record();

        SortOpts o2;
        o2.need_lcp = true;
        o2.skip_finished = true;
        o2.bk = &pl_.bk;
        o2.range_mode = 1;
        o2.pkey = pl_.pkey;
        if (fused) o2.runs = &rsrc;
        set_final(o2, dSA, dLCP);
        SortResult<idx_t> r2 = seg_sort<BITS>(pl_.seg2, n_tiles2, max_part_, in2, out2buf, n, o2, true);
        passes2_ = r2.passes;
        e6_ = be_.record();

        finalize<idx_t, BITS>(be_, pl_.P, n, r2, dSA, dLCP);
        e7_ = be_.record();
    }

    template <int BITS>
    bool run_direct(idx_t* dSA, idx_t* dLCP, uint32_t PG, uint32_t K1, BackendEvent e1, bool allow_k32 = true, bool defer = true)
    {
        const uint64_t n = pl_.n, m = pl_.m;
        const uint32_t p = pl_.p;
        CAPS_LAUNCH((sample_text_kernel<idx_t, BITS>), (uint32_t)((m + 255) / 256), 256, be_, (const uint32_t*)pl_.P, (uint64_t)0, n, m,
                    pl_.SA_.key, pl_.SA_.sa);
        CAPS_LAUNCH(uniform_segments_kernel, 1, 256, be_, pl_.segS.seg_start, 1u, m, m);
        prepare_segments(pl_.segS, tiles_of(m));
        SortOpts os;
        os.bk = &pl_.bk;
        os.unify = true;
        os.keys_only = true;
        SortResult<idx_t> rs = seg_sort<BITS>(pl_.segS, tiles_of(m), m, pl_.SA_, pl_.SB_, m, os, false);
        passesS_ = rs.passes;
        ElemBuf<idx_t> smp = rs.uniform();
        CAPS_LAUNCH((pick_pivots_kernel<idx_t>), (p + 255) / 256, 256, be_, (const uint64_t*)smp.key, (const idx_t*)smp.sa,
                    m, p, pl_.pkey, pl_.psa);
        be_.memset(pl_.dstat, 0, 4 * sizeof(uint64_t));
        uint32_t* dflag = reinterpret_cast<uint32_t*>(pl_.dstat + 2);
        CAPS_LAUNCH(group_keys_kernel, (p + 255) / 256, 256, be_, (const uint64_t*)pl_.pkey, p, PG, K1, pl_.gkey, dflag);
        CAPS_LAUNCH(skew_probe_kernel, (p + 255) / 256, 256, be_, (const uint64_t*)pl_.pkey, p, PG, K1, dflag + 2);
        uint32_t probe[4];
        be_.d2h(probe, dflag, sizeof probe);
        be_.sync();

        const ElemBuf<idx_t>& A = pl_.A;
        const uint32_t n_tilesA = tiles_of(n);
        const char* sub_env = std::getenv("CAPS_SA_DIRECT_SUB");
        uint32_t SUB = (n + GA_E - 1) / GA_E >= 32ull * DIRECT_SUB ? DIRECT_SUB : 1u;
        if (sub_env && std::atoi(sub_env) >= 1 && (uint32_t)std::atoi(sub_env) <= DIRECT_SUB) SUB = (uint32_t)std::atoi(sub_env);
        const uint32_t n_streams = K1 * SUB;
        uint64_t capA = A.region_bytes / ((sizeof(uint64_t) + sizeof(idx_t)) * (uint64_t)n_streams);
        const uint64_t idx_max = (uint64_t)std::numeric_limits<idx_t>::max() - TILE_E;
        if (capA > idx_max / n_streams) capA = idx_max / n_streams;
        capA = test_stream_cap(capA, n, n_streams);
        uint64_t* a_key = A.key;

        const char* mode_env = std::getenv("CAPS_SA_DIRECT_MODE");
        bool quantile = probe[0] != 0 || probe[2] != 0;
        if (mode_env && std::string(mode_env) == "linear") quantile = false;
        if (mode_env && std::string(mode_env) == "quantile") quantile = true;
        const uint64_t NBt = (n + BUCKET_Q - 1) / BUCKET_Q;
        const uint32_t KPG = (uint32_t)((NBt + K1 - 1) / K1);
        const uint64_t NB = (uint64_t)K1 * KPG;
        uint64_t m2 = NB * QUANTILE_SPB;
        if (m2 > n / 4) m2 = n / 4;
        if (quantile && (KPG < 2 || KPG > BUCKET_LDS || NB > pl_.bk.nb_cap || m2 < 8 * NB || m2 > (1ull << 31))) quantile = false;
        if (quantile && probe[3] > p / 4) { path_fallback_ = CAPS_SA_FB_PIVOT_TIES; return false; }
        if (!quantile && probe[0] != 0) { path_fallback_ = CAPS_SA_FB_PIVOT_TIES; return false; }
        uint64_t *rstart = nullptr, *rcap = nullptr;
        direct_quantile_ = quantile ? 1u : 0u;
        const char* keys_env = std::getenv("CAPS_SA_KEYS");
        const bool k32 = allow_k32 && !quantile && BITS == 2 && keys_env && std::string(keys_env) == "32";
        direct_k32_ = k32 ? 1u : 0u;
        idx_t* a_sa = reinterpret_cast<idx_t*>(reinterpret_cast<char*>(A.key) + (uint64_t)n_streams * capA * (k32 ? sizeof(uint32_t) : sizeof(uint64_t)));
        if (k32) CAPS_LAUNCH(group_shift_kernel, (K1 + 255) / 256, 256, be_, (const uint64_t*)pl_.gkey, K1, pl_.gshift);
        if (quantile) {
            CAPS_LAUNCH((sample_text_kernel<idx_t, BITS>), (uint32_t)((m2 + 255) / 256), 256, be_, (const uint32_t*)pl_.P, (uint64_t)0, n, m2,
                        pl_.A.key, pl_.A.sa);
            SegBufs sseg = pl_.seg1;
            sseg.G = 1;
            CAPS_LAUNCH(uniform_segments_kernel, 1, 256, be_, sseg.seg_start, 1u, m2, m2);
            prepare_segments(sseg, tiles_of(m2));
            SortOpts oq;
            oq.bk = &pl_.bk;
            oq.unify = true;
            oq.knots = pl_.gkey;
            oq.knots_per_parent = K1;
            oq.skewed_keys = probe[2] != 0;
            oq.keys_only = true;
            SortResult<idx_t> rq = seg_sort<BITS>(sseg, tiles_of(m2), m2, pl_.A, pl_.B, m2, oq, false);
            ElemBuf<idx_t> smp2 = rq.uniform();
            CAPS_LAUNCH(knots_kernel, (uint32_t)((NB + 255) / 256), 256, be_, (const uint64_t*)smp2.key, m2, NB, KPG, K1, pl_.knots, pl_.gkey);
            rstart = pl_.rstart;
            rcap = pl_.rcap;
            const uint64_t token = 2 * GA_E / K1 + 16;
            if (capA <= 2 * token) { path_fallback_ = CAPS_SA_FB_SHAPE; direct_quantile_ = 0; return false; }
            CAPS_LAUNCH(group_caps_kernel, (K1 + 255) / 256, 256, be_, (const uint64_t*)pl_.knots, NB, KPG, K1, SUB, capA - token, token, rcap);
            CAPS_LAUNCH(scan_sizes_kernel, 1, 1024, be_, (const uint64_t*)rcap, n_streams, rstart);
        }
        CAPS_LAUNCH(split_lut_kernel, (SPLIT_LUT_CELLS + 256) / 256, 256, be_, (const uint64_t*)pl_.gkey, K1 - 1, pl_.glut, dflag + 1);
        e3_ = be_.record();

        CAPS_LAUNCH(uniform_segments_kernel, 1, 256, be_, pl_.seg1.seg_start, 1u, n, n);
        SegBufs whole = pl_.seg1;
        whole.G = 1;
        prepare_segments(whole, n_tilesA);
        BucketParams one = make_bucket_params(0, ~0ull, K1);
        const uint64_t b01[2] = {0, K1};
        be_.h2d(pl_.bk.params, &one, sizeof one);
        be_.h2d(pl_.bk.bstart, b01, sizeof b01);
        be_.memset(pl_.dcur, 0, (size_t)n_streams * sizeof(idx_t));
        const char* la = std::getenv("CAPS_SA_LEVEL_A");
        const bool big_tiles = k32 || !(la && std::string(la) == "tile");
        {
            BackendEvent s0 = be_.record();
            if (k32)
                CAPS_LAUNCH((group_scatter_kernel<idx_t, BITS, uint32_t>), (uint32_t)((n + GA_E - 1) / GA_E), TILE_NT, be_, (const uint32_t*)pl_.P,
                            packed_words(n, BITS), (uint64_t)0, n, (const uint64_t*)pl_.gkey, K1, (const uint16_t*)pl_.glut,
                            (const uint32_t*)(dflag + 1), SUB, capA, pl_.dcur, reinterpret_cast<uint32_t*>(a_key), a_sa, 0u, 1u,
                            (const uint64_t*)rstart, (const uint64_t*)rcap, (const uint8_t*)pl_.gshift, 0u, K1);
            else if (big_tiles)
                CAPS_LAUNCH((group_scatter_kernel<idx_t, BITS>), (uint32_t)((n + GA_E - 1) / GA_E), TILE_NT, be_, (const uint32_t*)pl_.P,
                            packed_words(n, BITS), (uint64_t)0, n, (const uint64_t*)pl_.gkey, K1, (const uint16_t*)pl_.glut,
                            (const uint32_t*)(dflag + 1), SUB, capA, pl_.dcur, a_key, a_sa, 0u, 1u, (const uint64_t*)rstart, (const uint64_t*)rcap,
                            (const uint8_t*)nullptr, 0u, K1);
            else
                CAPS_LAUNCH((bucket_scatter_kernel<idx_t, BITS, SRC_TEXT, MAP_SPLIT>), n_tilesA, TILE_NT, be_, whole.desc(), (const uint32_t*)pl_.P,
                            packed_words(n, BITS), (uint64_t)0, (const uint64_t*)nullptr, (const idx_t*)nullptr, RunSrc<idx_t>(),
                            (const BucketParams*)pl_.bk.params, (const uint64_t*)pl_.bk.bstart, (const uint64_t*)nullptr, capA,
                            pl_.dcur, a_key, a_sa, (const BucketParams*)nullptr, (const uint32_t*)nullptr,
                            (const uint64_t*)pl_.gkey, (const uint16_t*)pl_.glut, (const uint32_t*)(dflag + 1), SUB, 0u, 1u, (const uint16_t*)nullptr,
                            Spill<idx_t>());
            BackendEvent s1 = be_.record();
            scatter_clock_.spans.push_back({s0, s1});
            scatter_clock_.elems.push_back(n);
            la0_ = s0;
            la1_ = s1;
        }
        SegBufs groups = pl_.seg2;
        groups.G = n_streams;
        CAPS_LAUNCH((slot_segments_kernel<idx_t>), (n_streams + 256) / 256, 256, be_, (const idx_t*)pl_.dcur, K1, SUB, big_tiles ? 1u : 0u, capA,
                    (const uint64_t*)rstart, (const uint64_t*)rcap, groups.seg_start, groups.seg_end, pl_.dstat);
        ::caps::prepare_segments(be_, groups, n / TILE_E + n_streams + 1, nullptr, nullptr, true);
        uint64_t out2[2], dstat[4];
        uint32_t W = (k32 || waves_ < 2 || !wave_scratch_.key) ? 1u : std::min<uint32_t>(waves_, K1);
        std::vector<idx_t> h_cur;
        if (W > 1) {
            h_cur.resize(n_streams);
            be_.d2h(h_cur.data(), pl_.dcur, (size_t)n_streams * sizeof(idx_t));
        }
        be_.d2h(out2, groups.out2, sizeof out2);
        be_.d2h(dstat, pl_.dstat, sizeof dstat);
        be_.sync();
        direct_groups_ = K1;
        direct_max_group_ = dstat[1] ? dstat[1] : out2[1];
        if (dstat[1] != 0 || dstat[0] != n) { path_fallback_ = CAPS_SA_FB_GROUP_OVERFLOW; return false; }
        max_part_ = out2[1];
        e2_ = e1;
        e4_ = e3_;
        e5_ = be_.record();

        SortOpts o2;
        o2.need_lcp = true;
        o2.skip_finished = true;
        o2.bk = &pl_.bk;
        o2.range_mode = 1;
        o2.pkey = pl_.gkey;
        o2.part_total = K1;
        o2.sub = SUB;
        o2.seg_ends = true;
        if (quantile) {
            o2.knots = pl_.knots;
            o2.knots_per_parent = KPG;
            o2.in_extent = (uint64_t)n_streams * capA;
            o2.spill_slots = spill_stats_[1] == 0;
            o2.spill_stats = spill_stats_;
            o2.hot_tile_rec = pl_.seg1.tile_rec;
        }
        o2.skewed_keys = quantile && probe[2] != 0 && !std::getenv("CAPS_SA_TRY_LINEAR_TILES");
        if (k32) { o2.k32 = true; o2.range_mode = 2; o2.gshift = pl_.gshift; }
        o2.in_key = a_key;
        o2.in_sa = a_sa;
        if (defer && !k32 && !std::getenv("CAPS_SA_NO_DEFER")) o2.defer_flags = pl_.bk.fcount;
        o2.run_tables = &pl_.seg1;
        passes2_ = 0;
        run_buckets_ = 0;
        tie_groups_ = tie_elems_ = 0;
        tie_levels_ = 0;
        std::vector<uint32_t> wave_end;
        if (W > 1) {
            auto group_size = [&](uint32_t g) {
                uint64_t z = 0;
                for (uint32_t x = 0; x < SUB; ++x) { const uint32_t s = g * SUB + x; z += (uint64_t)h_cur[big_tiles ? (size_t)(s % SUB) * K1 + s / SUB : s]; }
                return z;
            };
            const uint64_t target = std::min<uint64_t>((n + W - 1) / W, wave_scratch_elems_);
            uint64_t acc = 0;
            for (uint32_t g = 0; g < K1; ++g) {
                const uint64_t z = group_size(g);
                if (z > wave_scratch_elems_) { wave_end.clear(); break; }
                if (acc && acc + z > target) { wave_end.push_back(g); acc = 0; }
                acc += z;
                if (g + 1 == K1) wave_end.push_back(K1);
            }
            W = wave_end.empty() ? 1u : (uint32_t)wave_end.size();
        }
        uint64_t base = 0;
        for (uint32_t w = 0; w < W; ++w) {
            const uint32_t g0 = W > 1 && w ? wave_end[w - 1] : 0u, g1 = W > 1 ? wave_end[w] : K1;
            SegBufs gw = groups;
            uint32_t n_tiles_w = (uint32_t)out2[0];
            uint64_t max_len_w = out2[1], elems_w = n;
            SortOpts ow = o2;
            if (W > 1) {
                gw.seg_start = groups.seg_start + (size_t)g0 * SUB;
                gw.seg_end = groups.seg_end + (size_t)g0 * SUB;
                gw.G = (g1 - g0) * SUB;
                elems_w = 0;
                max_len_w = 0;
                uint64_t tiles = 0;
                for (uint32_t s = g0 * SUB; s < g1 * SUB; ++s) {
                    const uint64_t z = (uint64_t)h_cur[big_tiles ? (size_t)(s % SUB) * K1 + s / SUB : s];
                    elems_w += z;
                    max_len_w = std::max(max_len_w, z);
                    tiles += (z + TILE_E - 1) / TILE_E;
                }
                n_tiles_w = (uint32_t)tiles;
                ::caps::prepare_segments(be_, gw, tiles + 1, nullptr, nullptr, true);
                ow.part_off = g0;
                if (quantile) { ow.knots = pl_.knots + (size_t)g0 * KPG; ow.knots_have_prev = g0 > 0; }
            }
            set_final(ow, dSA + base, dLCP + base);
            if (elems_w) {
                SortResult<idx_t> r2 = seg_sort<BITS>(gw, n_tiles_w, max_len_w, W > 1 ? wave_scratch_ : pl_.A, pl_.B, elems_w, ow, true);
                if (r2.failed) {
                    if (sink_) sink_->reset(be_);
                    return run_direct<BITS>(dSA, dLCP, PG, K1, e1, false, defer);
                }
                passes2_ = std::max(passes2_, r2.passes);
                run_buckets_ += (uint32_t)r2.run_buckets.size();
                finalize<idx_t, BITS>(be_, pl_.P, n, r2, dSA + base, dLCP + base);
                if (r2.msd_failed) {
                    if (sink_) sink_->reset(be_);
                    return run_direct<BITS>(dSA, dLCP, PG, K1, e1, allow_k32, false);
                }
                tie_groups_ += r2.msd_groups;
                tie_elems_ += r2.msd_elems;
                tie_levels_ = std::max(tie_levels_, r2.msd_levels);
                if (base) CAPS_LAUNCH((wave_head_lcp_kernel<idx_t, BITS>), 1, 64, be_, (const uint32_t*)pl_.P, n, (const idx_t*)dSA, dLCP, base);
            }
            if (sink_ && elems_w) sink_->wave_done(be_, base, elems_w);
            base += elems_w;
        }
        sink_served_ = sink_ != nullptr;
        waves_used_ = W;
        e6_ = be_.record();
        e7_ = be_.record();
        return true;
    }

    template <int BITS>
    void run(idx_t* dSA, idx_t* dLCP, caps_sa_stats* st, BackendEvent e0, BackendEvent e1)
    {
// ... 93 lines not shown
```

### caps-sa_amd/csrc/shard.h

```cpp
#pragma once
#include <cstdio>
#include <cstdlib>
#include <memory>
#include <numeric>

#include "pipeline.h"

namespace caps {

struct DevAllocs;

struct ShardBase {
    virtual ~ShardBase() {}
    virtual void info(caps_sa_shard_info* out) const = 0;
    virtual void phase1(void* d_sample_keys, void* d_sample_sa) = 0;
    virtual void pivots(const void* d_all_keys, const void* d_all_sa, void* d_local_sizes) = 0;
    virtual void collate(const uint64_t* all_sizes, void* d_send_keys, void* d_send_sa, uint64_t* send_counts,
                         uint64_t* recv_counts) = 0;
    virtual void phase2(const void* d_recv_keys, const void* d_recv_sa, void* dSA, void* dLCP) = 0;
    virtual uint64_t last_sa() = 0;
    virtual void fix_first_lcp(uint64_t prev_sa, void* dLCP) = 0;
    virtual void scatter(void* d_send_keys, void* d_send_sa, void* d_report) = 0;
    virtual int plan(const uint64_t* all_reports, uint64_t* send_counts, uint64_t* recv_counts) = 0;
    virtual int sort_owned(const void* d_recv_keys, const void* d_recv_sa, void* dSA, void* dLCP) = 0;
    virtual void set_key_bits(int bits) = 0;
    virtual void phase1_arrays(void* d_keys_out, void* d_sa_out, uint64_t* count, uint64_t* subarray_len) = 0;
};

template <typename idx_t> class Shard : public ShardBase {
public:
    Shard(const void* dT, uint64_t n, uint64_t p_arg, int rank, int world, void* stream)
        : be_(static_cast<decltype(Backend::stream)>(stream)), dT_(static_cast<const uint8_t*>(dT)), n_(n), rank_(rank),
          world_(world)
    {
        effective_params(n, p_arg, &p_, &ppp_);
        if (p_ < 2) throw std::invalid_argument("sharded build needs an effective subproblem count >= 2 (n >= 32)");
        s_ = n / p_;
        g0_ = (uint32_t)((uint64_t)rank * p_ / world);
        g1_ = (uint32_t)((uint64_t)(rank + 1) * p_ / world);
        G_ = g1_ - g0_;
        text_base_ = (uint64_t)g0_ * s_;
        local_n_ = G_ ? (g1_ == p_ ? n : (uint64_t)g1_ * s_) - text_base_ : 0;
        m_local_ = (uint64_t)G_ * ppp_;
        m_total_ = (uint64_t)p_ * ppp_;
        direct_fb_ = direct_shape(n, p_, m_total_, &PG_, &K1_);
        if (const char* force = std::getenv("CAPS_SA_PATH")) if (std::string(force) == "classic") direct_fb_ = CAPS_SA_FB_FORCED;
        local_ = std::getenv("CAPS_SA_SHARD_EXCHANGE") == nullptr;
        const int tw = local_ ? 1 : world;
        const uint64_t ga_tiles = (n + GA_E - 1) / GA_E;
        my_tiles_ = local_ ? (uint32_t)ga_tiles : (uint32_t)(ga_tiles > (uint64_t)rank ? (ga_tiles - rank + world - 1) / world : 0);
        my_elems_ = (uint64_t)my_tiles_ * GA_E;
        if (my_tiles_ && (local_ || (ga_tiles - 1) % world == (uint64_t)rank)) my_elems_ -= ga_tiles * GA_E - n;
        if (direct_fb_ == CAPS_SA_FB_NONE) {
            SUB_ = ga_tiles / tw >= 32ull * DIRECT_SUB ? DIRECT_SUB : 1u;
            if (const char* e = std::getenv("CAPS_SA_DIRECT_SUB")) if (std::atoi(e) >= 1 && (uint32_t)std::atoi(e) <= DIRECT_SUB) SUB_ = (uint32_t)std::atoi(e);
            n_streams_ = K1_ * SUB_;
            own_lo_ = (uint32_t)((uint64_t)rank * K1_ / world);
            own_hi_ = (uint32_t)((uint64_t)(rank + 1) * K1_ / world);
            const double mean = (double)n / ((double)n_streams_ * tw);
            capA_ = (uint64_t)(mean * 1.10 + 6.0 * std::sqrt(mean) + 2.0 * GA_E / K1_ + 64.0);
            capA_ += capA_ & 1;
            capA_ = test_stream_cap(capA_, n, (uint64_t)n_streams_ * tw);
            if (n_streams_ * capA_ / (local_ ? world : 1) + TILE_E >= (uint64_t)std::numeric_limits<idx_t>::max()) direct_fb_ = CAPS_SA_FB_SHAPE;
            const uint64_t NBt = (n + BUCKET_Q - 1) / BUCKET_Q;
            KPG_ = (uint32_t)((NBt + K1_ - 1) / K1_);
            NB_ = (uint64_t)K1_ * KPG_;
            m2_ = NB_ * QUANTILE_SPB;
            if (m2_ > n / 4) m2_ = n / 4;
        }
        const uint32_t gseg = std::max<uint32_t>(p_, DIRECT_SUB * std::min<uint32_t>(p_, BUCKET_LDS)) + (uint32_t)world * DIRECT_SUB;
        try {
            const uint64_t share = n / (uint64_t)world + 1;
            cap_ = std::max<uint64_t>(local_n_, share + share / 4 + 16 * TILE_E);
            if (world == 1) cap_ = local_n_;
            if (direct_fb_ == CAPS_SA_FB_NONE) {
                const uint64_t own_max = ((uint64_t)K1_ + world - 1) / world * SUB_ * tw * capA_;
                cap_ = std::max<uint64_t>(cap_, own_max + TILE_E);
            }
            P_ = get<uint32_t>(text_alloc_words(n));
            present_ = get<uint32_t>(16);
            lut_ = get<uint8_t>(256);
            A_ = elems(cap_);
            B_ = elems(cap_);
            seg1_ = segs(G_ ? G_ : 1, cap_ / TILE_E + p_ + 2);
            seg1_.G = G_;
            seg2_ = segs(gseg, cap_ / TILE_E + gseg + 2);
            seg_cap_ = gseg;
            seg2_.G = p_;
            seg2_.seg_end = get<uint64_t>((size_t)gseg + 1);
            gkey_ = get<uint64_t>(p_);
            glut_ = get<uint16_t>(SPLIT_LUT_CELLS + 2);
            dcur_ = get<idx_t>(gseg);
            gshift_ = get<uint8_t>(gseg);
            rcap_ = get<uint64_t>((size_t)gseg + 1);
            rstart_ = get<uint64_t>((size_t)gseg + 2);
            quantile_ok_ = direct_fb_ == CAPS_SA_FB_NONE && local_ && KPG_ >= 2 && KPG_ <= BUCKET_LDS && m2_ >= 8 * NB_ && m2_ <= (1ull << 31) &&
                           m2_ <= cap_ && n_streams_ <= gseg && (uint64_t)(own_hi_ - own_lo_) * KPG_ <= BucketBufs::bucket_bound(cap_, gseg);
            knots_ = get<uint64_t>(quantile_ok_ ? NB_ : 1);
            dstat_ = get<uint64_t>(4);
            SA_ = elems(m_total_);
            SB_ = elems(m_total_);
            segS_ = segs(1, m_total_ / TILE_E + 3);
            pkey_ = get<uint64_t>(p_);
            psa_ = get<idx_t>(p_);
            Pm_ = get<idx_t>((size_t)(G_ ? G_ : 1) * (p_ + 1));
            ruler_ = get<idx_t>((size_t)(G_ ? G_ : 1) * p_);
            sizes_ = get<uint64_t>(p_);
            partial_ = get<uint64_t>((size_t)PART_CHUNKS * p_);
            lstart_ = get<uint64_t>((size_t)p_ + 1);
            bk_ = buckets(cap_, gseg);
            hot_rec_ = quantile_ok_ ? get<TileInfo>(bk_.tile_cap + 1) : nullptr;
            const uint64_t a = bk_.tile_cap + 3, b = m_total_ / TILE_E + 3;
            tdesc_ = get<TileDesc>(a > b ? a : b);
            desc_ = get<uint64_t>((size_t)3 * world * p_ + 3);
        } catch (...) {
            release();
            throw;
        }
    }
    ~Shard() override { release(); }

    void info(caps_sa_shard_info* o) const override
    {
        o->n = n_; o->p = p_; o->ppp = ppp_; o->rank = (uint32_t)rank_; o->world = (uint32_t)world_;
        o->g0 = g0_; o->g1 = g1_; o->bits_per_char = (uint32_t)bits_; o->idx_bytes = sizeof(idx_t);
        o->local_elems = local_n_; o->m_local = m_local_; o->m_total = m_total_;
        o->recv_total = recv_total_; o->slice_off = slice_off_; o->capacity = cap_;
        o->part_lo = jlo_; o->part_hi = jhi_;
        o->ms_phase1 = ms_phase1_; o->ms_pivots = ms_pivots_; o->ms_collate = ms_collate_; o->ms_phase2 = ms_phase2_;
        o->direct_fallback = (uint32_t)direct_fb_; o->direct_groups = K1_; o->direct_sub = SUB_;
        o->n_streams = n_streams_; o->stream_cap = capA_;
        o->send_capacity = std::max<uint64_t>(local_n_, direct_fb_ != CAPS_SA_FB_NONE ? 0 :
                                              local_ ? ((uint64_t)K1_ + world_ - 1) / world_ * SUB_ * capA_ : (uint64_t)n_streams_ * capA_);
        o->exchange = direct_fb_ == CAPS_SA_FB_NONE && local_ ? 0u : 1u;
        o->direct_quantile = quantile_ ? 1u : 0u;
        o->run_buckets = run_buckets_;
        o->tie_groups_deferred = tie_groups_;
        o->tie_levels = tie_levels_;
        o->reserved_ = 0;
        o->ms_scatter = ms_scatter_; o->ms_sort = ms_sort_;
        o->key_bytes = key_bits_ / 8;
        o->ms_level_a = ms_level_a_; o->ms_level_b = ms_level_b_ + ms_count_; o->ms_tile_sort = ms_tile_sort_; o->ms_merge_passes = ms_merge_;
        o->level_a_elems = my_elems_;
        o->slot_splits = slot_stats_[0]; o->slot_splits_redone = slot_stats_[1];
    }

    void phase1(void* d_sample_keys, void* d_sample_sa) override
    {
        slot_stats_[0] = slot_stats_[1] = 0;
        BackendEvent e0 = be_.record();
        bits_ = prepare_text(be_, dT_, n_, P_, present_, lut_);
        if (G_) {
            CAPS_LAUNCH(uniform_segments_kernel, (G_ + 256) / 256, 256, be_, seg1_.seg_start, G_, s_, local_n_);
            const uint64_t last = local_n_ - (uint64_t)(G_ - 1) * s_;
            n_tiles1_ = (G_ - 1) * tiles_of(s_) + tiles_of(last);
            prepare_segments(be_, seg1_, n_tiles1_);
            cur_ = (bits_ == 2 ? sort<2>(seg1_, n_tiles1_, last, true, A_, B_, local_n_, text_base_, false, false, &bk_, true)
                               : sort<8>(seg1_, n_tiles1_, last, true, A_, B_, local_n_, text_base_, false, false, &bk_, true)).uniform();
            oth_ = cur_.key == A_.key ? B_ : A_;
            CAPS_LAUNCH((sample_kernel<idx_t>), (uint32_t)((m_local_ + 255) / 256), 256, be_, (const uint64_t*)seg1_.seg_start, G_,
                        ppp_, (const uint64_t*)cur_.key, (const idx_t*)cur_.sa, static_cast<uint64_t*>(d_sample_keys),
                        static_cast<idx_t*>(d_sample_sa));
        }
        BackendEvent e1 = be_.record();
        be_.sync();
        ms_phase1_ = be_.elapsed_ms(e0, e1);
        be_.release_events();
    }

    void phase1_arrays(void* d_keys_out, void* d_sa_out, uint64_t* count, uint64_t* subarray_len) override
    {
        *count = local_n_;
        *subarray_len = s_;
        if (d_keys_out && cur_.key) be_.d2d(d_keys_out, cur_.key, local_n_ * sizeof(uint64_t));
        if (d_sa_out && cur_.sa) be_.d2d(d_sa_out, cur_.sa, local_n_ * sizeof(idx_t));
        be_.sync();
// ... 265 lines not shown
        BackendEvent e1 = be_.record();
        be_.sync();
        ms_sort_ = be_.elapsed_ms(e0, e1);
        double* out[4] = {&ms_tile_sort_, &ms_level_b_, &ms_count_, &ms_merge_};
        for (size_t c = 0; c < clocks_.size() && c < 4; ++c) {
            *out[c] = 0;
            for (auto& sp : clocks_[c].spans) *out[c] += be_.elapsed_ms(sp.first, sp.second);
        }
        clocks_.clear();
        be_.release_events();
        return code;
    }

    void set_key_bits(int bits) override { force64_ = bits == 64; }

    uint64_t last_sa() override
    {
        if (!recv_total_) return ~0ull;
        idx_t v = 0;
        be_.d2h(&v, dSA_ + (recv_total_ - 1), sizeof(idx_t));
        be_.sync();
        return (uint64_t)v;
    }

    void fix_first_lcp(uint64_t prev_sa, void* dLCP) override
    {
        if (!recv_total_ || prev_sa == ~0ull) return;
        if (bits_ == 2)
            CAPS_LAUNCH((first_lcp_kernel<idx_t, 2>), 1, 64, be_, (const uint32_t*)P_, n_, prev_sa, (const idx_t*)dSA_,
                        static_cast<idx_t*>(dLCP));
        else
            CAPS_LAUNCH((first_lcp_kernel<idx_t, 8>), 1, 64, be_, (const uint32_t*)P_, n_, prev_sa, (const idx_t*)dSA_,
                        static_cast<idx_t*>(dLCP));
        be_.sync();
    }

private:
    Backend be_;
    std::vector<void*> owned_;
    const uint8_t* dT_;
    uint64_t n_;
    int rank_, world_;
    uint32_t p_ = 0, ppp_ = 0, g0_ = 0, g1_ = 0, G_ = 0, G2_ = 0, jlo_ = 0, jhi_ = 0, n_tiles1_ = 0, n_tiles2_ = 0, n_desc_ = 0;
    uint64_t s_ = 0, text_base_ = 0, local_n_ = 0, m_local_ = 0, m_total_ = 0, recv_total_ = 0, slice_off_ = 0, max_len2_ = 0;
    int bits_ = 0;
    uint32_t slot_stats_[2] = {0, 0};
    uint32_t run_buckets_ = 0;
    uint64_t tie_groups_ = 0;
    uint32_t tie_levels_ = 0;
    uint32_t h_flag_ = 0;
    uint32_t* P_ = nullptr;
    uint32_t* present_ = nullptr;
    uint8_t* lut_ = nullptr;
    ElemBuf<idx_t> A_, B_, SA_, SB_, cur_, oth_;
    uint64_t cap_ = 0;
    idx_t* dSA_ = nullptr;
    BucketBufs bk_;
    TileDesc* tdesc_ = nullptr;
    SegBufs seg1_, segS_, seg2_;
    uint64_t *pkey_ = nullptr, *sizes_ = nullptr, *lstart_ = nullptr, *desc_ = nullptr, *partial_ = nullptr;
    idx_t *psa_ = nullptr, *Pm_ = nullptr, *ruler_ = nullptr;
    double ms_phase1_ = 0, ms_pivots_ = 0, ms_collate_ = 0, ms_phase2_ = 0, ms_scatter_ = 0, ms_sort_ = 0;
    double ms_level_a_ = 0, ms_level_b_ = 0, ms_tile_sort_ = 0, ms_count_ = 0, ms_merge_ = 0;
    BackendEvent a0_, a1_;
    std::vector<KernelClock> clocks_;
    int direct_fb_ = CAPS_SA_FB_SHAPE;
    bool direct_planned_ = false;
    uint32_t seg_cap_ = 0;
    bool local_ = true;
    bool quantile_ok_ = false, quantile_ = false, skewed_ = false, level_a_ran_ = false;
    uint32_t KPG_ = 0;
    uint64_t NB_ = 0, m2_ = 0;
    uint64_t *knots_ = nullptr, *rcap_ = nullptr, *rstart_ = nullptr;
    TileInfo* hot_rec_ = nullptr;
    uint64_t spill_stats_[3] = {0, 0, 0};
    std::vector<uint64_t> h_rstart_, h_rcap_;
    uint32_t PG_ = 0, K1_ = 0, SUB_ = 1, n_streams_ = 0, my_tiles_ = 0, own_lo_ = 0, own_hi_ = 0;
    uint64_t capA_ = 0, my_elems_ = 0;
    uint32_t key_bits_ = 64;
    const void* last_send_keys_ = nullptr;
    const void* last_send_sa_ = nullptr;
    bool force64_ = false;
    uint8_t* gshift_ = nullptr;
    uint64_t *gkey_ = nullptr, *dstat_ = nullptr;
    uint16_t* glut_ = nullptr;
    idx_t* dcur_ = nullptr;

    template <int BITS> void scatter_bits(void* d_send_keys, void* d_send_sa, uint32_t* dflag)
    {
        const uint64_t m = m_total_;
        CAPS_LAUNCH((sample_text_kernel<idx_t, BITS>), (uint32_t)((m + 255) / 256), 256, be_, (const uint32_t*)P_, (uint64_t)0, n_, m,
                    SA_.key, SA_.sa);
        CAPS_LAUNCH(uniform_segments_kernel, 1, 256, be_, segS_.seg_start, 1u, m, m);
        prepare_segments(be_, segS_, tiles_of(m));
        ElemBuf<idx_t> smp = sort<BITS>(segS_, tiles_of(m), m, false, SA_, SB_, m, 0, false, false).uniform();
        CAPS_LAUNCH((pick_pivots_kernel<idx_t>), (p_ + 255) / 256, 256, be_, (const uint64_t*)smp.key, (const idx_t*)smp.sa, m, p_,
                    pkey_, psa_);
        CAPS_LAUNCH(group_keys_kernel, (p_ + 255) / 256, 256, be_, (const uint64_t*)pkey_, p_, PG_, K1_, gkey_, dflag);
        const uint64_t* rs = nullptr;
        const uint64_t* rc = nullptr;
        if (quantile_ok_) {
            CAPS_LAUNCH(skew_probe_kernel, (p_ + 255) / 256, 256, be_, (const uint64_t*)pkey_, p_, PG_, K1_, dflag + 2);
            uint32_t probe[4];
            be_.d2h(probe, dflag, sizeof probe);
            be_.sync();
            quantile_ = probe[0] != 0 || probe[2] != 0 || be_.long_runs;
            if (const char* mode = std::getenv("CAPS_SA_DIRECT_MODE")) {
                if (std::string(mode) == "linear" && !be_.long_runs) quantile_ = false;
                if (std::string(mode) == "quantile") quantile_ = true;
            }
            skewed_ = probe[2] != 0;
            if (quantile_) key_bits_ = 64;
            const uint64_t token = 2 * GA_E / K1_ + 16;
            uint32_t& code = h_flag_;
            code = 0;
            if (quantile_ && probe[3] > p_ / 4) code = CAPS_SA_FB_PIVOT_TIES;
            else if (quantile_ && capA_ <= 2 * token) code = CAPS_SA_FB_SHAPE;
            if (quantile_ && code == 0) {
                CAPS_LAUNCH((sample_text_kernel<idx_t, BITS>), (uint32_t)((m2_ + 255) / 256), 256, be_, (const uint32_t*)P_, (uint64_t)0, n_, m2_,
                            A_.key, A_.sa);
                SegBufs sseg = seg1_;
                sseg.G = 1;
                CAPS_LAUNCH(uniform_segments_kernel, 1, 256, be_, sseg.seg_start, 1u, m2_, m2_);
                prepare_segments(be_, sseg, tiles_of(m2_));
                ElemBuf<idx_t> smp2 = sort<BITS>(sseg, tiles_of(m2_), m2_, false, A_, B_, m2_, 0, false, false, &bk_, true, false, nullptr, nullptr,
                                                 gkey_, K1_, skewed_).uniform();
                CAPS_LAUNCH(knots_kernel, (uint32_t)((NB_ + 255) / 256), 256, be_, (const uint64_t*)smp2.key, m2_, NB_, KPG_, K1_, knots_, gkey_);
                CAPS_LAUNCH(group_caps_kernel, (K1_ + 255) / 256, 256, be_, (const uint64_t*)knots_, NB_, KPG_, K1_, SUB_, capA_ - token, token, rcap_);
                CAPS_LAUNCH(scan_sizes_kernel, 1, 1024, be_, (const uint64_t*)rcap_, n_streams_, rstart_);
                const size_t own_streams = (size_t)(own_hi_ - own_lo_) * SUB_;
                h_rstart_.assign(own_streams + 1, 0);
                h_rcap_.assign(own_streams + 1, 0);
                be_.d2h(h_rstart_.data(), rstart_ + (size_t)own_lo_ * SUB_, (own_streams + 1) * sizeof(uint64_t));
                be_.d2h(h_rcap_.data(), rcap_ + (size_t)own_lo_ * SUB_, own_streams * sizeof(uint64_t));
                be_.sync();
                const uint64_t room = ((uint64_t)K1_ + world_ - 1) / world_ * SUB_ * capA_;
                if (h_rstart_[own_streams] - h_rstart_[0] > room) code = CAPS_SA_FB_GROUP_OVERFLOW;
                rs = rstart_ + (size_t)own_lo_ * SUB_;
                rc = rcap_ + (size_t)own_lo_ * SUB_;
            }
            if (quantile_ || code) be_.h2d(dflag, &code, sizeof code);
            if (code) { quantile_ = false; return; }
        }
        CAPS_LAUNCH(split_lut_kernel, (SPLIT_LUT_CELLS + 256) / 256, 256, be_, (const uint64_t*)gkey_, K1_ - 1, glut_, dflag + 1);
        be_.memset(dcur_, 0, (size_t)n_streams_ * sizeof(idx_t));
        if (key_bits_ == 32) CAPS_LAUNCH(group_shift_kernel, (K1_ + 255) / 256, 256, be_, (const uint64_t*)gkey_, K1_, gshift_);
        const uint32_t tile_first = local_ ? 0u : (uint32_t)rank_, tile_stride = local_ ? 1u : (uint32_t)world_;
        const uint32_t keep_lo = local_ ? own_lo_ : 0u, keep_hi = local_ ? own_hi_ : K1_;
        a0_ = be_.record();
        if (my_tiles_ && key_bits_ == 32)
            CAPS_LAUNCH((group_scatter_kernel<idx_t, BITS, uint32_t>), my_tiles_, TILE_NT, be_, (const uint32_t*)P_, packed_words(n_, BITS),
                        (uint64_t)0, n_, (const uint64_t*)gkey_, K1_, (const uint16_t*)glut_, (const uint32_t*)(dflag + 1), SUB_, capA_, dcur_,
                        static_cast<uint32_t*>(d_send_keys), static_cast<idx_t*>(d_send_sa), tile_first, tile_stride,
                        rs, rc, (const uint8_t*)gshift_, keep_lo, keep_hi);
        else if (my_tiles_)
            CAPS_LAUNCH((group_scatter_kernel<idx_t, BITS>), my_tiles_, TILE_NT, be_, (const uint32_t*)P_, packed_words(n_, BITS), (uint64_t)0,
                        n_, (const uint64_t*)gkey_, K1_, (const uint16_t*)glut_, (const uint32_t*)(dflag + 1), SUB_, capA_, dcur_,
                        static_cast<uint64_t*>(d_send_keys), static_cast<idx_t*>(d_send_sa), tile_first, tile_stride,
                        rs, rc, (const uint8_t*)nullptr, keep_lo, keep_hi);
        a1_ = be_.record();
        level_a_ran_ = true;
    }

    template <int BITS> bool sort_owned_bits(const void* d_recv_keys, const void* d_recv_sa, void* dSA, void* dLCP, bool defer, bool* retry)
    {
        *retry = false;
        tie_groups_ = 0;
        tie_levels_ = 0;
        SortOpts o;
        o.need_lcp = true;
        o.skip_finished = true;
        o.bk = &bk_;
        o.range_mode = 1;
        o.pkey = gkey_;
        o.part_off = jlo_;
        o.part_total = K1_;
        o.sub = (local_ ? 1u : (uint32_t)world_) * SUB_;
        o.seg_ends = true;
        o.in_key = static_cast<const uint64_t*>(d_recv_keys);
        o.in_sa = d_recv_sa;
        o.final_sa = dSA;
        o.final_lcp = dLCP;
        o.bnd.first_key = bk_.first_key;
        o.bnd.last_key = bk_.last_key;
        o.bnd.first_sa = bk_.first_sa;
        o.bnd.last_sa = bk_.last_sa;
        o.slot_stats = slot_stats_;
        o.speculate = std::getenv("CAPS_SA_NO_SLOTS") == nullptr;
        if (key_bits_ == 32) { o.k32 = true; o.range_mode = 2; o.gshift = gshift_; o.speculate = true; }
        if (defer && bk_.fcount) {
            o.defer_flags = bk_.fcount;
            o.run_tables = &seg1_;
        }
        if (quantile_) {
            o.knots = knots_ + (size_t)jlo_ * KPG_;
            o.knots_per_parent = KPG_;
            o.knots_have_prev = jlo_ > 0;
            o.in_extent = ((uint64_t)K1_ + world_ - 1) / world_ * SUB_ * capA_;
            o.skewed_keys = skewed_ && !std::getenv("CAPS_SA_TRY_LINEAR_TILES");
            o.spill_slots = hot_rec_ != nullptr;
            o.hot_tile_rec = hot_rec_;
            o.spill_stats = spill_stats_;
        }
        KernelClock tile_clock, scatter_clock, count_clock, merge_clock;
        o.tile_clock = &tile_clock;
        o.scatter_clock = &scatter_clock;
        o.count_clock = &count_clock;
        o.merge_clock = &merge_clock;
        SortResult<idx_t> r = segmented_sort<idx_t, BITS>(be_, P_, n_, tdesc_, seg2_, n_tiles2_, max_len2_, A_, B_, recv_total_, o);
        clocks_ = {tile_clock, scatter_clock, count_clock, merge_clock};
        run_buckets_ = (uint32_t)r.run_buckets.size();
        if (r.failed) return false;
        finalize<idx_t, BITS>(be_, P_, n_, r, static_cast<idx_t*>(dSA), static_cast<idx_t*>(dLCP));
        if (r.msd_failed) { *retry = true; return true; }
        tie_groups_ = r.msd_groups;
        tie_levels_ = r.msd_levels;
        return true;
    }

    template <typename T> T* get(size_t count)
    {
        T* p = static_cast<T*>(be_.alloc((count ? count : 1) * sizeof(T)));
        owned_.push_back(p);
        return p;
    }
    ElemBuf<idx_t> elems(uint64_t cnt)
    {
        ElemBuf<idx_t> b;
        const size_t c = cnt ? cnt : 1;
        const size_t key_bytes = (c * sizeof(uint64_t) + 255) & ~size_t(255), idx_bytes = (c * sizeof(idx_t) + 255) & ~size_t(255);
        char* base = get<char>(key_bytes + 2 * idx_bytes);
        b.key = reinterpret_cast<uint64_t*>(base);
        b.sa = reinterpret_cast<idx_t*>(base + key_bytes);
        b.lcp = reinterpret_cast<idx_t*>(base + key_bytes + idx_bytes);
        b.region_bytes = key_bytes + 2 * idx_bytes;
        return b;
    }
    SegBufs segs(uint32_t G, uint64_t cap)
    {
        SegBufs s;
        s.G = G;
        s.seg_start = get<uint64_t>((size_t)G + 1);
        s.tile_off = get<uint32_t>((size_t)G + 1);
        s.tile_rec = get<TileInfo>(cap);
        s.out2 = get<uint64_t>(2);
        return s;
    }
    void drop(void* p)
    {
        if (!p) return;
        for (size_t i = 0; i < owned_.size(); ++i)
            if (owned_[i] == p) { be_.free(p); owned_[i] = owned_.back(); owned_.pop_back(); return; }
    }
    void release()
    {
        for (void* p : owned_) be_.free(p);
        owned_.clear();
    }
    template <int BITS>
    SortResult<idx_t> sort(const SegBufs& s, uint32_t n_tiles, uint64_t max_len, bool from_text, ElemBuf<idx_t> a, ElemBuf<idx_t> b,
                           uint64_t n_elems, uint64_t text_base, bool need_lcp, bool skip_finished, const BucketBufs* bk = nullptr,
                           bool unify = false, bool between_pivots = false, void* final_sa = nullptr, void* final_lcp = nullptr,
                           const uint64_t* knots = nullptr, uint32_t knots_per_parent = 0, bool skewed = false)
    {
        SortOpts o;
        o.keys_only = knots != nullptr;
        o.knots = knots;
        o.knots_per_parent = knots_per_parent;
        o.skewed_keys = skewed;
        if (final_sa && bk) {
            o.final_sa = final_sa;
            o.final_lcp = final_lcp;
            o.bnd.first_key = bk->first_key;
            o.bnd.last_key = bk->last_key;
            o.bnd.first_sa = bk->first_sa;
            o.bnd.last_sa = bk->last_sa;
        }
        if (between_pivots) {
            o.range_mode = 1;
            o.pkey = pkey_;
            o.part_off = jlo_;
            o.part_total = p_;
        }
        o.from_text = from_text;
        o.text_base = text_base;
        o.need_lcp = need_lcp;
        o.skip_finished = skip_finished;
        o.bk = bk;
        o.unify = unify;
        o.slot_stats = slot_stats_;
        o.speculate = bk != nullptr && std::getenv("CAPS_SA_NO_SLOTS") == nullptr && slot_stats_[1] == 0;
        return segmented_sort<idx_t, BITS>(be_, P_, n_, tdesc_, s, n_tiles, max_len, a, b, n_elems, o);
    }
    BucketBufs buckets(uint64_t n_elems, uint32_t G)
    {
        BucketBufs k;
        k.nb_cap = BucketBufs::bucket_bound(n_elems ? n_elems : 1, G);
        k.tile_cap = (n_elems ? n_elems : 1) / TILE_E + k.nb_cap + 2;
        k.params = get<BucketParams>(G);
        k.segB = get<uint64_t>(G);
        k.bstart = get<uint64_t>((size_t)G + 1);
        k.count = get<uint64_t>(k.nb_cap);
        k.cursor = get<idx_t>(k.nb_cap);
        k.scan_tmp = get<uint64_t>(2 * ((size_t)k.nb_cap / SCAN_CHUNK + 2));
        k.tile_map = get<BucketParams>(k.nb_cap);
        k.first_key = get<uint64_t>(k.nb_cap);
        k.last_key = get<uint64_t>(k.nb_cap);
        k.first_sa = get<idx_t>(k.nb_cap);
        k.last_sa = get<idx_t>(k.nb_cap);
        k.sub = segs(k.nb_cap, k.tile_cap);
        k.fparams = get<BucketParams>(G);
        k.fsegB = get<uint64_t>(G);
        k.fstart = get<uint64_t>((size_t)G + 1);
        k.fcount = get<uint64_t>((size_t)EQ_FINE * k.nb_cap);
        k.gfirst = get<uint32_t>(k.nb_cap);
        k.kshift = get<uint8_t>(k.nb_cap);
        k.skip = get<uint8_t>(k.nb_cap);
        k.run_list = get<uint64_t>(1 + 4 * RUN_BUCKET_MAX);
        return k;
    }
};

}
```

### caps-sa_amd/csrc/text.h

```cpp
#pragma once
#include "kernel_lang.h"

namespace caps {

template <int BITS> struct TextTraits {
    static constexpr uint32_t CPW = 32 / BITS;
    static constexpr uint32_t KCH = 64 / BITS;
};

HD uint64_t packed_words(uint64_t n, int bits) { return (n + (32 / bits) - 1) / (32 / bits) + 4; }

template <int BITS>
HD uint64_t window64(const uint32_t* __restrict__ P, uint64_t pos)
{
    constexpr uint32_t CPW = TextTraits<BITS>::CPW;
    const uint64_t w = pos / CPW;
    const uint32_t sh = (uint32_t)(pos % CPW) * BITS;
    const uint64_t x0 = P[w], x1 = P[w + 1], x2 = P[w + 2];
#if defined(CAPS_W64_FUNNEL)
    const uint32_t a = (uint32_t)x0, b = (uint32_t)x1, c = (uint32_t)x2;
    const uint32_t hi = sh ? (a << sh) | (b >> (32u - sh)) : a, lo = sh ? (b << sh) | (c >> (32u - sh)) : b;
    return ((uint64_t)hi << 32) | lo;
#else
    return (((x0 << 32) | x1) << sh) | ((x2 << sh) >> 32);
// ... 33 lines not shown

template <int BITS> HD bool periodic128(uint64_t hi, uint64_t lo, uint32_t d)
{
    const uint32_t sh = d * BITS;
    return hi == ((hi << sh) | (lo >> (64 - sh))) && ((lo ^ (lo << sh)) >> sh) == 0;
}

#ifndef CAPS_RUN_ENTER
#define CAPS_RUN_ENTER 3
#endif
constexpr uint32_t RUN_ENTER = CAPS_RUN_ENTER;
template <int BITS, bool RUNS>
HD uint64_t deep_scan(const uint32_t* __restrict__ P, uint64_t n, uint64_t a, uint64_t b, uint64_t l, uint64_t maxlen,
                      uint64_t& wa, uint64_t& wb, bool in_run = false)
{
    constexpr uint32_t KCH = TextTraits<BITS>::KCH;
#ifdef CAPS_NO_RUN_TABLE
    constexpr bool plain = true;
#else
    constexpr bool plain = !RUNS;
#endif
    if (plain) {
        for (; l < maxlen; l += KCH) {
            wa = window64<BITS>(P, a + l);
            wb = window64<BITS>(P, b + l);
            if (wa != wb) return l + (uint32_t)caps_clz64(wa ^ wb) / BITS;
        }
        return maxlen;
    }
    for (uint32_t k = 0; k < (in_run ? 0u : RUN_ENTER) && l < maxlen; ++k, l += KCH) {
        wa = window64<BITS>(P, a + l);
        wb = window64<BITS>(P, b + l);
        if (wa != wb) return l + (uint32_t)caps_clz64(wa ^ wb) / BITS;
    }
    if (l >= maxlen) return maxlen;
    const uint64_t* __restrict__ R = run_table<BITS>(P, n);
    while (l < maxlen) {
        const uint64_t x = a + l, y = b + l;
        const uint64_t wa0 = window64<BITS>(P, x), wb0 = window64<BITS>(P, y);
        const uint64_t wa1 = window64<BITS>(P, x + KCH), wb1 = window64<BITS>(P, y + KCH);
        const uint64_t rx = R[(x + KCH - 1) / KCH], ry = R[(y + KCH - 1) / KCH];
        wa = wa0;
        wb = wb0;
        if (wa != wb) return l + (uint32_t)caps_clz64(wa ^ wb) / BITS;
        const uint64_t hi = wa;
        wa = wa1;
        wb = wb1;
        if (wa != wb) return l + KCH + (uint32_t)caps_clz64(wa ^ wb) / BITS;
        uint64_t step = 2 * KCH;
        if (rx) {
            const uint32_t d = (uint32_t)(rx >> 56);
            if ((uint32_t)(ry >> 56) == d && periodic128<BITS>(hi, wa, d)) {
                const uint64_t ex = (rx & RUN_POS_MASK) - x, ey = (ry & RUN_POS_MASK) - y;
                step = ex < ey ? ex : ey;
            }
        }
        l += step;
    }
    return maxlen;
}

template <int BITS, bool RUNS = true>
HD uint64_t deep_lcp(const uint32_t* __restrict__ P, uint64_t n, uint64_t a, uint64_t b, uint64_t from, bool in_run = false)
{
    if (a >= n || b >= n) return 0;
    const uint64_t maxlen = n - (a > b ? a : b);
    uint64_t wa, wb;
    const uint64_t l = deep_scan<BITS, RUNS>(P, n, a, b, from, maxlen, wa, wb, in_run);
    return l < maxlen ? l : maxlen;
}

template <int BITS, bool RUNS = true>
HD uint64_t pair_lcp(const uint32_t* __restrict__ P, uint64_t n, uint64_t ka, uint64_t a, uint64_t kb, uint64_t b)
{
    const uint64_t x = ka ^ kb;
    if (x) {
        const uint64_t maxlen = n - (a > b ? a : b);
        const uint64_t l = (uint32_t)caps_clz64(x) / BITS;
        return l < maxlen ? l : maxlen;
    }
    return deep_lcp<BITS, RUNS>(P, n, a, b, TextTraits<BITS>::KCH, RUNS && block_period<BITS>(ka) != 0);
}

HD uint32_t key32_of(uint64_t key, uint32_t cs) { return (uint32_t)((key << cs) >> 32); }

template <int BITS, bool RUNS = false>
HD uint64_t pair_lcp32(const uint32_t* __restrict__ P, uint64_t n, uint32_t ka, uint64_t a, uint32_t kb, uint64_t b, uint32_t cs)
{
    const uint32_t x = ka ^ kb;
    if (x) {
        const uint64_t maxlen = n - (a > b ? a : b);
        const uint64_t l = (cs + (uint32_t)__builtin_clz(x)) / BITS;
        return l < maxlen ? l : maxlen;
    }
    return deep_lcp<BITS, RUNS>(P, n, a, b, (cs + 32u) / BITS);
}

template <int BITS, bool RUNS = true>
HD bool suffix_less_tie(const uint32_t* __restrict__ P, uint64_t n, uint64_t a, uint64_t b, bool in_run = false)
{
    if (a >= n || b >= n) return a > b;
    const uint64_t maxlen = n - (a > b ? a : b);
    uint64_t wa = 0, wb = 0;
    const uint64_t l = deep_scan<BITS, RUNS>(P, n, a, b, TextTraits<BITS>::KCH, maxlen, wa, wb, in_run);
    if (l < maxlen) return wa < wb;
    return a > b;
}

#ifndef CAPS_TIE_WINDOWS
#define CAPS_TIE_WINDOWS 64
#endif
constexpr uint32_t TIE_WINDOWS = CAPS_TIE_WINDOWS;
template <int BITS>
HD uint32_t suffix_less_tie_bounded(const uint32_t* __restrict__ P, uint64_t n, uint64_t a, uint64_t b,
                                    uint32_t from = TextTraits<BITS>::KCH)
{
    constexpr uint32_t KCH = TextTraits<BITS>::KCH;
    if (a >= n || b >= n) return a > b ? 1u : 0u;
    const uint64_t maxlen = n - (a > b ? a : b);
    uint64_t l = from;
    for (uint32_t k = 0; k < TIE_WINDOWS && l < maxlen; ++k, l += KCH) {
        const uint64_t wa = window64<BITS>(P, a + l), wb = window64<BITS>(P, b + l);
        if (wa != wb) return wa < wb ? 1u : 0u;
    }
    if (l >= maxlen) return a > b ? 1u : 0u;
    return 2u;
}

template <int BITS>
HD uint32_t tie_order_lcp_bounded(const uint32_t* __restrict__ P, uint64_t n, uint64_t a, uint64_t b, uint32_t& lcp)
{
    constexpr uint32_t KCH = TextTraits<BITS>::KCH;
    lcp = 0;
    if (a >= n || b >= n) return a > b ? 1u : 0u;
    const uint64_t maxlen = n - (a > b ? a : b);
    uint64_t l = KCH;
    for (uint32_t k = 0; k < TIE_WINDOWS / 2 && l < maxlen; ++k, l += 2 * KCH) {
        const bool more = l + KCH < maxlen;
        const uint64_t l1 = more ? l + KCH : l;
        const uint64_t wa0 = window64<BITS>(P, a + l), wb0 = window64<BITS>(P, b + l);
        const uint64_t wa1 = window64<BITS>(P, a + l1), wb1 = window64<BITS>(P, b + l1);
        if (wa0 != wb0) {
            const uint64_t d = l + (uint32_t)caps_clz64(wa0 ^ wb0) / BITS;
            lcp = (uint32_t)(d < maxlen ? d : maxlen);
            return wa0 < wb0 ? 1u : 0u;
        }
        if (wa1 != wb1) {
            const uint64_t d = l1 + (uint32_t)caps_clz64(wa1 ^ wb1) / BITS;
            lcp = (uint32_t)(d < maxlen ? d : maxlen);
            return wa1 < wb1 ? 1u : 0u;
        }
    }
    if (l >= maxlen) { lcp = (uint32_t)maxlen; return a > b ? 1u : 0u; }
    return 2u;
}
static_assert(64 / 2 + TIE_WINDOWS * (64 / 2) < (1u << 15) && 64 / 8 + TIE_WINDOWS * (64 / 8) < (1u << 15), "bounded tie lcps fit 15 bits");

template <int BITS> HD uint64_t letter_pattern(uint32_t c)
{
    uint64_t p = c;
    for (uint32_t s = BITS; s < 64; s <<= 1) p |= p << s;
    return p;
}
template <int BITS> HD bool is_letter_key(uint64_t key)
{
    return key == letter_pattern<BITS>((uint32_t)(key >> (64 - BITS)));
}

template <int BITS>
HD uint64_t letter_run_end(const uint32_t* __restrict__ P, uint64_t n, uint64_t pos, uint64_t key)
{
    constexpr uint32_t KCH = TextTraits<BITS>::KCH;
    const uint64_t* __restrict__ R = run_table<BITS>(P, n);
    uint64_t x = pos + KCH;
    while (x < n) {
        const uint64_t w = window64<BITS>(P, x);
        if (w != key) { x += (uint32_t)caps_clz64(w ^ key) / BITS; break; }
        const uint64_t rb = R[(x - 1) / KCH];
        if ((rb >> 56) == 1u) { x = rb & RUN_POS_MASK; break; }
        x += KCH;
    }
    return x < n ? x : n;
}

template <int IDX_BYTES> struct RunKey {
    static constexpr uint32_t RB = IDX_BYTES == 4 ? 32 : 40;
    static constexpr uint32_t FB = 63 - RB;
    static constexpr uint64_t RMASK = (1ull << RB) - 1;
};
template <int IDX_BYTES, int BITS>
HD uint64_t run_key(const uint32_t* __restrict__ P, uint64_t n, uint64_t pos, uint64_t key)
{
    using RK = RunKey<IDX_BYTES>;
    const uint64_t e = letter_run_end<BITS>(P, n, pos, key);
    const uint64_t r = e - pos;
    if (e >= n) return r << RK::FB;
    const uint64_t w = window64<BITS>(P, e);
    const uint64_t cls = (w >> (64 - BITS)) < (key >> (64 - BITS)) ? 0u : 1u;
    return (cls << 63) | ((cls ? RK::RMASK - r : r) << RK::FB) | (w >> (64 - RK::FB));
}
template <int IDX_BYTES> HD uint64_t run_key_r(uint64_t rk)
{
    using RK = RunKey<IDX_BYTES>;
    const uint64_t f = (rk >> RK::FB) & RK::RMASK;
    return (rk >> 63) ? RK::RMASK - f : f;
}
template <int IDX_BYTES, int BITS>
HD uint64_t run_pair_lcp(const uint32_t* __restrict__ P, uint64_t n, uint64_t ka, uint64_t a, uint64_t kb, uint64_t b)
{
    const uint64_t ra = run_key_r<IDX_BYTES>(ka), rb = run_key_r<IDX_BYTES>(kb);
    if (ra != rb) return ra < rb ? ra : rb;
    if (a + ra >= n || b + rb >= n) return ra;
    return ra + deep_lcp<BITS, true>(P, n, a + ra, b + rb, 0);
}

template <int BITS, bool RUNS = true>
HD bool suffix_less(const uint32_t* __restrict__ P, uint64_t n, uint64_t ka, uint64_t a, uint64_t kb, uint64_t b)
{
    if (ka != kb) return ka < kb;
// ... 6 lines not shown
```

Measured before the change: 64.24 billion.

## Use base-offset 32-bit keys and defer tile tie resolution to a listed pass

After: 63.06 billion (median of 2 runs). 0.982x the previous value.

```diff
diff --git a/caps-sa_amd/csrc/kernels.h b/caps-sa_amd/csrc/kernels.h
--- a/caps-sa_amd/csrc/kernels.h
+++ b/caps-sa_amd/csrc/kernels.h
@@ -663,11 +663,6 @@
     if (x) return lcp_capped<idx_t>((uint32_t)caps_clz64(x) / BITS, n, a, b);
     return pair_lcp<BITS, RUNS>(P, n, ka, (uint64_t)a, kb, (uint64_t)b);
 }
-template <int BITS, bool RUNS, typename idx_t>
-DEV_INLINE uint64_t tile_pair_lcp(const uint32_t* __restrict__ P, uint64_t n, uint32_t ka, idx_t a, uint32_t kb, idx_t b, uint32_t cs)
-{
-    return pair_lcp32<BITS, RUNS>(P, n, ka, (uint64_t)a, kb, (uint64_t)b, cs);
-}
 
 template <typename idx_t> HD idx_t tie_sentinel() { return (idx_t)~(idx_t)0; }
 template <int BITS, bool RUNS, typename idx_t>
@@ -813,12 +808,16 @@
         }                                                                                                       \
     }
 
+constexpr uint32_t TIE32_LIST = TILE_NT < 256 ? TILE_NT : 256;
+constexpr uint32_t TIE32_MAX = 3;
+static_assert(TIE32_LIST <= TILE_NT && TILE_E <= (1u << 16) && TILE_BINS <= (1u << 16), "one lane per listed element; entry = bin << 16 | slot");
 template <typename idx_t, int BITS, bool FROM_TEXT, typename KT = uint64_t>
 GLOBAL_FN LAUNCH_BOUNDS2(TILE_NT, TILE_WAVES_PER_SIMD) tile_sort_kernel(KCTX SegDesc sd, const uint32_t* __restrict__ P, uint64_t n,
                                                   uint64_t text_base, uint32_t lcp_mode, uint32_t slot_cap, const KT* in_key,
                                                   const idx_t* in_sa, uint64_t* out_key, idx_t* out_sa, idx_t* out_lcp,
                                                   FinalOut<idx_t> fin, const BucketParams* __restrict__ seg_map,
-                                                  uint32_t* __restrict__ redo, const uint8_t* __restrict__ kshift)
+                                                  uint32_t* __restrict__ redo, const uint8_t* __restrict__ kshift,
+                                                  const uint64_t* __restrict__ kbase, uint32_t test_knobs = 0)
 {
     constexpr bool TILE_RUNS = false;
     constexpr bool K32 = sizeof(KT) == 4;
@@ -826,14 +825,19 @@
     static_assert(!K32 || !FROM_TEXT, "32-bit keys come from the slots of level B");
     TILE_SORT_PROLOGUE
     const uint32_t TILE_KEY_SHIFT = K32 ? kshift[g] : 0u;
-    const uint32_t tie_from = K32 ? (TILE_KEY_SHIFT + 32u) / BITS : TextTraits<BITS>::KCH;
+    const uint64_t TILE_KEY_BASE = K32 ? kbase[g] : 0ull;
+    const uint32_t tie_from = K32 ? (64u - TILE_KEY_SHIFT) / BITS : TextTraits<BITS>::KCH;
+    const uint32_t tie_cap = K32 && (test_knobs >> 8) && (test_knobs >> 8) < TIE32_LIST ? test_knobs >> 8 : TIE32_LIST;
+    const bool drop_notes = K32 && (test_knobs & 2u) != 0;
     SHARED_ARRAY(KT, skey, TILE_E);
     SHARED_ARRAY(idx_t, ssa, TILE_E);
     SHARED_ARRAY(uint32_t, hist, TILE_BINS + 1);
     SHARED_ARRAY(uint64_t, kmm, 2);
-    SHARED_ARRAY(uint32_t, flag, 1);
-    constexpr bool SLOT_ORDER = sizeof(idx_t) == 4;
+    SHARED_ARRAY(uint32_t, flag, K32 ? 3 : 1);
+    SHARED_ARRAY(uint32_t, tlist, K32 ? TIE32_LIST : 1);
+    constexpr bool SLOT_ORDER = sizeof(idx_t) == 4 || K32;
     SHARED_ARRAY(uint16_t, sbin, SLOT_ORDER ? TILE_E : 1);
+    uint16_t* const tnote = sbin;
     SHARED_ARRAY(uint16_t, perm, SLOT_ORDER ? TILE_E : 1);
     TL_DECL(KT, rk, TILE_EPT);
     TL_DECL(idx_t, rs, TILE_EPT);
@@ -841,6 +845,7 @@
     TL_DECL(uint32_t, rb, TILE_EPT);
 
     PHASE_T0();
+    if (K32) { PAR(tid) { if (tid == 0) { flag[1] = 0; flag[2] = 0; } } }
     TILE_SORT_LOAD
     TILE_SORT_RANGE
     PHASE_MARK(0);
@@ -892,17 +897,28 @@
                 if (e < cnt) {
                     const uint32_t slot = SLOT_ORDER ? e : TL(rd, tid, k), bin = SLOT_ORDER ? (uint32_t)sbin[slot] : TL(rb, tid, k);
                     const uint32_t bs = hist[bin], be = hist[bin + 1];
-                    const uint64_t key = SLOT_ORDER ? (uint64_t)skey[slot] : (uint64_t)TL(rk, tid, k);
+                    const KT key = SLOT_ORDER ? skey[slot] : TL(rk, tid, k);
                     uint32_t less = 0;
+                    uint32_t ties = 0;
                     for (uint32_t j = bs; j < be; ++j) {
-                        const uint64_t kj = skey[j];
+                        const KT kj = skey[j];
                         less += kj < key ? 1u : 0u;
                         if (kj == key && j != slot) {
-                            const uint64_t sa = SLOT_ORDER ? (uint64_t)ssa[slot] : (uint64_t)TL(rs, tid, k);
-                            const uint32_t c = suffix_less_tie_bounded<BITS>(P, n, (uint64_t)ssa[j], sa, tie_from);
-                            if (c == 2u) flag[0] = 1;
-                            less += c & 1u;
+                            if (K32) {
+                                ++ties;
+                                less += j < slot ? 1u : 0u;
+                            } else {
+                                const uint64_t sa = SLOT_ORDER ? (uint64_t)ssa[slot] : (uint64_t)TL(rs, tid, k);
+                                const uint32_t c = suffix_less_tie_bounded<BITS>(P, n, (uint64_t)ssa[j], sa, tie_from);
+                                if (c == 2u) flag[0] = 1;
+                                less += c & 1u;
+                            }
                         }
+                    }
+                    if (K32 && ties) {
+                        const uint32_t pi = ties <= TIE32_MAX ? FETCH_ADD_U32(&flag[1], 1u) : tie_cap;
+                        if (pi < tie_cap) tlist[pi] = (bin << 16) | slot;
+                        else flag[0] = 1;
                     }
                     if (SLOT_ORDER) RACY_STORE_U16(&perm[bs + less], (uint16_t)slot);
                     else TL(rd, tid, k) = bs + less;
@@ -912,6 +928,37 @@
         SYNC();
         fast = flag[0] == 0;
         PHASE_MARK(4);
+        if (K32 && fast && flag[1]) {
+            const uint32_t listed = flag[1];
+            PAR(tid) {
+                if (tid < listed) {
+                    const uint32_t en = tlist[tid], slot = en & 0xFFFFu, bin = en >> 16;
+                    const uint32_t bs = hist[bin], be = hist[bin + 1];
+                    const KT key = skey[slot];
+                    const uint64_t sa = (uint64_t)ssa[slot];
+                    uint32_t less = 0, before = 0, note = 0;
+                    bool deep = false;
+                    for (uint32_t j = bs; j < be; ++j) {
+                        const KT kj = skey[j];
+                        less += kj < key ? 1u : 0u;
+                        if (kj == key && j != slot) {
+                            uint32_t d = 0;
+                            const uint32_t c = tie_order_lcp_bounded<BITS>(P, n, (uint64_t)ssa[j], sa, d, tie_from);
+                            if (c == 2u) deep = true;
+                            else if (c == 1u) { ++before; note = d > note ? d : note; }
+                        }
+                    }
+                    if (deep) flag[0] = 1;
+                    else {
+                        RACY_STORE_U16(&perm[bs + less + before], (uint16_t)slot);
+                        tnote[slot] = (uint16_t)(before && !drop_notes ? 0x8000u | note : 0u);
+                    }
+                }
+            }
+            SYNC();
+            fast = flag[0] == 0;
+            PHASE_MARK(5);
+        }
         if (fast && !SLOT_ORDER) {
             TILE_SORT_PLACE_FINAL
             PHASE_MARK(5);
@@ -934,7 +981,18 @@
                     const KT key = skey[sl];
                     const idx_t sa = ssa[sl];
                     uint64_t l = 0;
-                    if (with_lcp && e) { const uint32_t sp = perm[e - 1]; l = TILE_EMIT_LCP_(skey[sp], ssa[sp], key, sa); }
+                    if (with_lcp && e) {
+                        const uint32_t sp = perm[e - 1];
+                        if (K32) {
+                            const uint32_t kp = (uint32_t)skey[sp], kc = (uint32_t)key;
+                            if (kp != kc) l = lcp_capped<idx_t>(key32_lcp<BITS>(kp, kc, TILE_KEY_SHIFT, TILE_KEY_BASE), n, ssa[sp], sa);
+                            else {
+                                const uint32_t v = tnote[sl];
+                                if (v & 0x8000u) l = v & 0x7FFFu;
+                                else flag[2] = 1;
+                            }
+                        } else l = TILE_EMIT_LCP_(skey[sp], ssa[sp], key, sa);
+                    }
                     if (direct) {
                         STREAM_STORE(&fin.sa[start + e], sa);
                         STREAM_STORE(&fin.lcp[start + e], (idx_t)l);
@@ -952,6 +1010,10 @@
         TILE_SORT_EMIT
     }
     PHASE_MARK(6);
+    if (K32) {
+        SYNC();
+        if (flag[2]) { PAR(tid) { if (tid == 0) redo[1 + FETCH_ADD_U32(&redo[0], 1u)] = b; } }
+    }
 }
 
 GLOBAL_FN LAUNCH_BOUNDS(256) hot_tiles_kernel(KCTX SegDesc sd, uint32_t slot_cap, TileInfo* __restrict__ hot)
@@ -2176,12 +2238,12 @@
 constexpr uint32_t BUCKET_TARGET = (TILE_E * CAPS_BUCKET_EIGHTHS) / 8;
 constexpr uint32_t BUCKET_LDS = TILE_BINS_;
 
-DEV_INLINE void key32_range(uint64_t& kmin, uint64_t& kmax, bool kmin_exclusive, uint32_t cs)
+DEV_INLINE void key32_range(uint64_t& kmin, uint64_t& kmax, bool kmin_exclusive, uint32_t s, uint64_t base)
 {
     const uint64_t lo = kmin_exclusive ? kmin + 1 : kmin;
     if (lo > kmax || (kmin_exclusive && kmin == ~0ull)) { kmin = kmax = 0; return; }
-    kmin = key32_of(lo, cs);
-    kmax = key32_of(kmax, cs);
+    kmin = key32_of(lo, s, (uint32_t)base);
+    kmax = key32_of(kmax, s, (uint32_t)base);
 }
 
 GLOBAL_FN LAUNCH_BOUNDS(256) bucket_plan_kernel(KCTX const uint64_t* __restrict__ seg_start, const uint64_t* __restrict__ seg_end,
@@ -2189,7 +2251,7 @@
                                                 const uint64_t* __restrict__ pkey, uint32_t part_off, uint32_t part_total,
                                                 uint32_t enable, uint32_t fine, uint32_t sub,
                                                 BucketParams* __restrict__ bp, uint64_t* __restrict__ segB,
-                                                const uint8_t* __restrict__ gshift)
+                                                const uint8_t* __restrict__ gshift, const uint64_t* __restrict__ gbase)
 {
     PAR(tid) {
         const uint32_t g = K_BLOCK_IDX * K_BLOCK_DIM + tid;
@@ -2202,7 +2264,7 @@
                 const uint32_t j = part_off + parent;
                 if (j > 0) kmin = pkey[j - 1];
                 if (j + 1 < part_total) kmax = pkey[j];
-                if (range_mode == 2) key32_range(kmin, kmax, j > 0, gshift[j]);
+                if (range_mode == 2) key32_range(kmin, kmax, j > 0, gshift[j], gbase[j]);
             }
             uint32_t B = 1;
             if (enable && len > TILE_E && kmax > kmin) B = (uint32_t)((len + BUCKET_TARGET - 1) / BUCKET_TARGET);
@@ -2278,7 +2340,8 @@
                                                   uint32_t range_mode, uint32_t part_off, uint32_t part_total, uint32_t sub,
                                                   BucketParams* __restrict__ tile_map,
                                                   const BucketParams* __restrict__ fbps, const uint32_t* __restrict__ gfirst,
-                                                  const uint8_t* __restrict__ gshift, uint8_t* __restrict__ kshift)
+                                                  const uint8_t* __restrict__ gshift, const uint64_t* __restrict__ gbase,
+                                                  uint8_t* __restrict__ kshift, uint64_t* __restrict__ kbase)
 {
     PAR(tid) {
         const uint64_t i = (uint64_t)K_BLOCK_IDX * K_BLOCK_DIM + tid;
@@ -2295,7 +2358,7 @@
                 const uint32_t j = part_off + g / sub;
                 if (j > 0) kmin = pkey[j - 1];
                 if (j + 1 < part_total) kmax = pkey[j];
-                if (range_mode == 2) { key32_range(kmin, kmax, j > 0, gshift[j]); kshift[i] = gshift[j]; }
+                if (range_mode == 2) { key32_range(kmin, kmax, j > 0, gshift[j], gbase[j]); kshift[i] = gshift[j]; kbase[i] = gbase[j]; }
             }
             const uint32_t bk = (uint32_t)(i - bstart[g]);
             const double range1 = (double)(kmax - kmin) + 1.0;
@@ -2800,11 +2863,13 @@
                                                       KT* __restrict__ out_key, idx_t* __restrict__ out_sa,
                                                       uint32_t tile_first, uint32_t tile_stride,
                                                       const uint64_t* __restrict__ region_start, const uint64_t* __restrict__ region_cap,
-                                                      const uint8_t* __restrict__ gshift, uint32_t own_lo, uint32_t own_hi)
+                                                      const uint8_t* __restrict__ gshift, const uint64_t* __restrict__ gbase,
+                                                      uint32_t own_lo, uint32_t own_hi)
 {
     constexpr bool K32 = sizeof(KT) == 4;
     constexpr uint32_t DROP = ~0u;
     SHARED_ARRAY(uint8_t, scs, K32 ? BUCKET_LDS : 1);
+    SHARED_ARRAY(uint32_t, sbase, K32 ? BUCKET_LDS : 1);
     constexpr uint32_t CPW = TextTraits<BITS>::CPW;
     constexpr uint32_t WIN = GA_E / CPW + 8;
     const idx_t NO_SLOT = (idx_t)~(idx_t)0;
@@ -2828,7 +2893,7 @@
         for (uint32_t i = tid; i < WIN; i += K_BLOCK_DIM) twin[i] = w0 + i < n_words ? P[w0 + i] : 0u;
         for (uint32_t i = tid; i < n_split; i += K_BLOCK_DIM) stab[GA_SWZ(i)] = split[i];
         for (uint32_t i = tid; i <= SPLIT_LUT_CELLS; i += K_BLOCK_DIM) slut[i] = split_lut[i];
-        if (K32) for (uint32_t i = tid; i < K1; i += K_BLOCK_DIM) scs[i] = gshift[i];
+        if (K32) for (uint32_t i = tid; i < K1; i += K_BLOCK_DIM) { scs[i] = gshift[i]; sbase[i] = (uint32_t)gbase[i]; }
     }
     SYNC();
     const bool RUN_OF_POS = BITS == 2 && GA_EPT == CPW && pos0 % CPW == 0;
@@ -2929,7 +2994,7 @@
                     if (ob != NO_SLOT) {
                         const uint64_t dst = (uint64_t)ob + (q - hist[g]);
                         const uint64_t key = window64<BITS>(twin, pos0 + e - w0 * CPW);
-                        STREAM_STORE2(&out_key[dst], K32 ? (KT)key32_of(key, scs[g]) : (KT)key);
+                        STREAM_STORE2(&out_key[dst], K32 ? (KT)key32_of(key, scs[g], sbase[g]) : (KT)key);
                         STREAM_STORE2(&out_sa[dst], (idx_t)(pos0 + e));
                     }
                 }
@@ -3065,15 +3130,17 @@
     }
 }
 
-GLOBAL_FN LAUNCH_BOUNDS(256) group_shift_kernel(KCTX const uint64_t* __restrict__ gkey, uint32_t K1, uint8_t* __restrict__ gshift)
+GLOBAL_FN LAUNCH_BOUNDS(256) group_shift_kernel(KCTX const uint64_t* __restrict__ gkey, uint32_t K1, uint8_t* __restrict__ gshift,
+                                                uint64_t* __restrict__ gbase)
 {
     PAR(tid) {
         const uint32_t g = K_BLOCK_IDX * K_BLOCK_DIM + tid;
         if (g < K1) {
             const uint64_t lo = g ? gkey[g - 1] + 1 : 0, hi = g + 1 < K1 ? gkey[g] : ~0ull;
-            const uint64_t x = lo ^ hi;
-            const uint32_t c = x ? (uint32_t)caps_clz64(x) : 32u;
-            gshift[g] = (uint8_t)(lo > hi ? 0u : c < 32u ? c : 32u);
+            const bool empty = lo > hi || (g && gkey[g - 1] == ~0ull);
+            const uint32_t sh = empty ? 0u : key32_shift(lo, hi);
+            gshift[g] = (uint8_t)sh;
+            gbase[g] = empty ? 0ull : lo >> sh;
         }
     }
 }
diff --git a/caps-sa_amd/csrc/pipeline.h b/caps-sa_amd/csrc/pipeline.h
--- a/caps-sa_amd/csrc/pipeline.h
+++ b/caps-sa_amd/csrc/pipeline.h
@@ -84,6 +84,7 @@
     uint64_t* fcount = nullptr;
     uint32_t* gfirst = nullptr;
     uint8_t* kshift = nullptr;
+    uint64_t* kbase = nullptr;
     uint8_t* skip = nullptr;
     uint64_t* run_list = nullptr;
     uint32_t nb_cap = 0;
@@ -112,6 +113,7 @@
     idx_t* dcur = nullptr;
     uint16_t* glut = nullptr;
     uint8_t* gshift = nullptr;
+    uint64_t* gbase = nullptr;
     uint64_t* knots = nullptr;
     uint64_t* rcap = nullptr;
     uint64_t* rstart = nullptr;
@@ -187,6 +189,7 @@
         pl.dcur = ar.take<idx_t>(gseg);
         pl.glut = ar.take<uint16_t>(SPLIT_LUT_CELLS + 2);
         pl.gshift = ar.take<uint8_t>(gseg);
+        pl.gbase = ar.take<uint64_t>(gseg);
         pl.knots = ar.take<uint64_t>(pl.bk.nb_cap);
         pl.rcap = ar.take<uint64_t>(gseg);
         pl.rstart = ar.take<uint64_t>((size_t)gseg + 1);
@@ -215,6 +218,7 @@
     pl.bk.fcount = ar.take<uint64_t>((size_t)EQ_FINE * pl.bk.nb_cap);
     pl.bk.gfirst = ar.take<uint32_t>(pl.bk.nb_cap);
     pl.bk.kshift = ar.take<uint8_t>(pl.bk.nb_cap);
+    pl.bk.kbase = ar.take<uint64_t>(pl.bk.nb_cap);
     pl.bk.skip = ar.take<uint8_t>(pl.bk.nb_cap);
     pl.bk.run_list = ar.take<uint64_t>(1 + 4 * RUN_BUCKET_MAX);
     pl.pass_elems = ar.take<uint64_t>(kMaxPasses);
@@ -407,6 +411,7 @@
     const uint64_t* in_key = nullptr;
     const void* in_sa = nullptr;
     const uint8_t* gshift = nullptr;
+    const uint64_t* gbase = nullptr;
     bool k32 = false;
     bool keys_only = false;
     bool comparison_only = false;
@@ -470,11 +475,11 @@
         } else {
         CAPS_LAUNCH(bucket_plan_kernel, (s.G + 255) / 256, 256, be, (const uint64_t*)s.seg_start, s_end, s.G, o.range_mode, o.pkey, o.part_off,
                     o.part_total ? o.part_total : s.G, 1u, 1u, o.sub,
-                    bk.params, bk.segB, o.gshift);
+                    bk.params, bk.segB, o.gshift, o.gbase);
         CAPS_LAUNCH(scan_sizes_kernel, 1, 1024, be, (const uint64_t*)bk.segB, s.G, bk.bstart);
         CAPS_LAUNCH(bucket_ranges_kernel, (bk.nb_cap + 255) / 256, 256, be, (const uint64_t*)bk.bstart, s.G,
                     (const BucketParams*)bk.params, o.pkey, o.range_mode, o.part_off, o.part_total ? o.part_total : s.G, o.sub,
-                    bk.tile_map, (const BucketParams*)nullptr, (const uint32_t*)nullptr, o.gshift, bk.kshift);
+                    bk.tile_map, (const BucketParams*)nullptr, (const uint32_t*)nullptr, o.gshift, o.gbase, bk.kshift, bk.kbase);
         }
         seg_map = bk.tile_map;
         mark("bucket plan");
@@ -662,7 +667,7 @@
             uint64_t* ccount = bk.count;
             if (equalise) {
                 CAPS_LAUNCH(bucket_plan_kernel, (s.G + 255) / 256, 256, be, (const uint64_t*)s.seg_start, s_end, s.G, o.range_mode, o.pkey, o.part_off,
-                            o.part_total ? o.part_total : s.G, 1u, EQ_FINE, o.sub, bk.fparams, bk.fsegB, o.gshift);
+                            o.part_total ? o.part_total : s.G, 1u, EQ_FINE, o.sub, bk.fparams, bk.fsegB, o.gshift, o.gbase);
                 CAPS_LAUNCH(scan_sizes_kernel, 1, 1024, be, (const uint64_t*)bk.fsegB, s.G, bk.fstart);
                 be.memset(bk.fcount, 0, (size_t)EQ_FINE * bk.nb_cap * sizeof(uint64_t));
                 cparams = bk.fparams;
@@ -690,7 +695,7 @@
                             (const uint64_t*)bk.fsegB, (const uint64_t*)bk.fstart, (const uint64_t*)bk.fcount, bk.count, bk.gfirst);
                 CAPS_LAUNCH(bucket_ranges_kernel, (bk.nb_cap + 255) / 256, 256, be, (const uint64_t*)bk.bstart, s.G,
                             (const BucketParams*)bk.params, o.pkey, o.range_mode, o.part_off, o.part_total ? o.part_total : s.G, o.sub,
-                            bk.tile_map, (const BucketParams*)bk.fparams, (const uint32_t*)bk.gfirst, o.gshift, bk.kshift);
+                            bk.tile_map, (const BucketParams*)bk.fparams, (const uint32_t*)bk.gfirst, o.gshift, o.gbase, bk.kshift, bk.kbase);
             }
             BackendEvent c1 = be.record();
             if (o.count_clock) { o.count_clock->spans.push_back({c0, c1}); o.count_clock->elems.push_back(n_elems); }
@@ -745,6 +750,8 @@
     const uint32_t ggrid = n_tiles < 4 * be.persistent_blocks() ? n_tiles : 4 * be.persistent_blocks();
     const bool eq_tiles = !std::getenv("CAPS_SA_NO_EQ_TILES");
     const uint32_t drop = std::getenv("CAPS_SA_TEST_DROP_NOTE") ? 2u : 0u;
+    const char* tl_env = std::getenv("CAPS_SA_TEST_TIE_LIST");
+    const uint32_t tie_list = tl_env && std::atoi(tl_env) > 0 ? (uint32_t)std::atoi(tl_env) << 8 : 0u;
     if (!eq_tiles) redo3 = redo2 = redo;
     uint64_t* bflag = o.defer_flags && o.need_lcp && o.final_sa && !o.keys_only && !(o.k32 && slot_cap) ? o.defer_flags : nullptr;
     if (bflag) {
@@ -766,7 +773,7 @@
     r.k32 = o.k32 && slot_cap != 0;
     if (from_text) {
         CAPS_LAUNCH((tile_sort_kernel<idx_t, BITS, true>), n_tiles, TILE_NT, be, sd, P, n, o.text_base, lcp_mode, 0u,
-                    (const uint64_t*)nullptr, (const idx_t*)nullptr, cur.key, cur.sa, cur.lcp, fin, seg_map, redo, no_shift);
+                    (const uint64_t*)nullptr, (const idx_t*)nullptr, cur.key, cur.sa, cur.lcp, fin, seg_map, redo, no_shift, (const uint64_t*)nullptr, 0u);
         if (eq_tiles) CAPS_LAUNCH((tile_sort_eq_kernel<idx_t, BITS, true>), ggrid, TILE_NT, be, sd, P, n, o.text_base, lcp_mode, 0u,
                     (const uint64_t*)nullptr, (const idx_t*)nullptr, cur.key, cur.sa, cur.lcp, fin, seg_map, (const uint32_t*)redo, redo3, 0u | drop, redo2);
         if (eq_tiles) CAPS_LAUNCH((tile_sort_eq_kernel<idx_t, BITS, true, true>), ggrid, TILE_NT, be, sd, P, n, o.text_base, lcp_mode, 0u,
@@ -775,7 +782,7 @@
                     (const uint64_t*)nullptr, (const idx_t*)nullptr, cur.key, cur.sa, cur.lcp, fin, (const uint32_t*)redo3, 0u, bflag);
     } else if (r.k32) {
         CAPS_LAUNCH((tile_sort_kernel<idx_t, BITS, false, uint32_t>), n_tiles, TILE_NT, be, sd, P, n, (uint64_t)0, lcp_mode, slot_cap,
-                    reinterpret_cast<const uint32_t*>(in_key), in_sa, cur.key, cur.sa, cur.lcp, fin, seg_map, redo, (const uint8_t*)o.bk->kshift);
+                    reinterpret_cast<const uint32_t*>(in_key), in_sa, cur.key, cur.sa, cur.lcp, fin, seg_map, redo, (const uint8_t*)o.bk->kshift, (const uint64_t*)o.bk->kbase, drop | tie_list);
         if (eq_tiles) CAPS_LAUNCH((tile_sort_eq_kernel<idx_t, BITS, false>), ggrid, TILE_NT, be, sd, P, n, (uint64_t)0, lcp_mode, slot_cap,
                     (const uint64_t*)nullptr, in_sa, cur.key, cur.sa, cur.lcp, fin, (const BucketParams*)nullptr, (const uint32_t*)redo, redo3, 1u | drop, redo2);
         if (eq_tiles) CAPS_LAUNCH((tile_sort_eq_kernel<idx_t, BITS, false, true>), ggrid, TILE_NT, be, sd, P, n, (uint64_t)0, lcp_mode, slot_cap,
@@ -792,7 +799,7 @@
         } else {
         if (all_queued && !per_tile) CAPS_LAUNCH(queue_all_tiles_kernel, (n_tiles + 255) / 256, 256, be, sd, redo);
         else if (!all_queued) CAPS_LAUNCH((tile_sort_kernel<idx_t, BITS, false>), n_tiles, TILE_NT, be, sd_hot, P, n, (uint64_t)0, lcp_mode, slot_cap,
-                    in_key, in_sa, cur.key, cur.sa, cur.lcp, fin, seg_map, redo, no_shift);
+                    in_key, in_sa, cur.key, cur.sa, cur.lcp, fin, seg_map, redo, no_shift, (const uint64_t*)nullptr, 0u);
         if (per_tile) {
             CAPS_LAUNCH((tile_sort_eq_kernel<idx_t, BITS, false, false, false>), n_tiles, TILE_NT, be, sd_hot, P, n, (uint64_t)0, lcp_mode, slot_cap,
                         in_key, in_sa, cur.key, cur.sa, cur.lcp, fin, seg_map, (const uint32_t*)nullptr, redo3, 0u | drop, redo2);
@@ -1498,7 +1505,7 @@
         const bool k32 = allow_k32 && !quantile && BITS == 2 && keys_env && std::string(keys_env) == "32";
         direct_k32_ = k32 ? 1u : 0u;
         idx_t* a_sa = reinterpret_cast<idx_t*>(reinterpret_cast<char*>(A.key) + (uint64_t)n_streams * capA * (k32 ? sizeof(uint32_t) : sizeof(uint64_t)));
-        if (k32) CAPS_LAUNCH(group_shift_kernel, (K1 + 255) / 256, 256, be_, (const uint64_t*)pl_.gkey, K1, pl_.gshift);
+        if (k32) CAPS_LAUNCH(group_shift_kernel, (K1 + 255) / 256, 256, be_, (const uint64_t*)pl_.gkey, K1, pl_.gshift, pl_.gbase);
         if (quantile) {
             CAPS_LAUNCH((sample_text_kernel<idx_t, BITS>), (uint32_t)((m2 + 255) / 256), 256, be_, (const uint32_t*)pl_.P, (uint64_t)0, n, m2,
                         pl_.A.key, pl_.A.sa);
@@ -1543,12 +1550,12 @@
                 CAPS_LAUNCH((group_scatter_kernel<idx_t, BITS, uint32_t>), (uint32_t)((n + GA_E - 1) / GA_E), TILE_NT, be_, (const uint32_t*)pl_.P,
                             packed_words(n, BITS), (uint64_t)0, n, (const uint64_t*)pl_.gkey, K1, (const uint16_t*)pl_.glut,
                             (const uint32_t*)(dflag + 1), SUB, capA, pl_.dcur, reinterpret_cast<uint32_t*>(a_key), a_sa, 0u, 1u,
-                            (const uint64_t*)rstart, (const uint64_t*)rcap, (const uint8_t*)pl_.gshift, 0u, K1);
+                            (const uint64_t*)rstart, (const uint64_t*)rcap, (const uint8_t*)pl_.gshift, (const uint64_t*)pl_.gbase, 0u, K1);
             else if (big_tiles)
                 CAPS_LAUNCH((group_scatter_kernel<idx_t, BITS>), (uint32_t)((n + GA_E - 1) / GA_E), TILE_NT, be_, (const uint32_t*)pl_.P,
                             packed_words(n, BITS), (uint64_t)0, n, (const uint64_t*)pl_.gkey, K1, (const uint16_t*)pl_.glut,
                             (const uint32_t*)(dflag + 1), SUB, capA, pl_.dcur, a_key, a_sa, 0u, 1u, (const uint64_t*)rstart, (const uint64_t*)rcap,
-                            (const uint8_t*)nullptr, 0u, K1);
+                            (const uint8_t*)nullptr, (const uint64_t*)nullptr, 0u, K1);
             else
                 CAPS_LAUNCH((bucket_scatter_kernel<idx_t, BITS, SRC_TEXT, MAP_SPLIT>), n_tilesA, TILE_NT, be_, whole.desc(), (const uint32_t*)pl_.P,
                             packed_words(n, BITS), (uint64_t)0, (const uint64_t*)nullptr, (const idx_t*)nullptr, RunSrc<idx_t>(),
@@ -1603,7 +1610,7 @@
             o2.hot_tile_rec = pl_.seg1.tile_rec;
         }
         o2.skewed_keys = quantile && probe[2] != 0 && !std::getenv("CAPS_SA_TRY_LINEAR_TILES");
-        if (k32) { o2.k32 = true; o2.range_mode = 2; o2.gshift = pl_.gshift; }
+        if (k32) { o2.k32 = true; o2.range_mode = 2; o2.gshift = pl_.gshift; o2.gbase = pl_.gbase; }
         o2.in_key = a_key;
         o2.in_sa = a_sa;
         if (defer && !k32 && !std::getenv("CAPS_SA_NO_DEFER")) o2.defer_flags = pl_.bk.fcount;
diff --git a/caps-sa_amd/csrc/shard.h b/caps-sa_amd/csrc/shard.h
--- a/caps-sa_amd/csrc/shard.h
+++ b/caps-sa_amd/csrc/shard.h
@@ -92,6 +92,7 @@
             glut_ = get<uint16_t>(SPLIT_LUT_CELLS + 2);
             dcur_ = get<idx_t>(gseg);
             gshift_ = get<uint8_t>(gseg);
+            gbase_ = get<uint64_t>(gseg);
             rcap_ = get<uint64_t>((size_t)gseg + 1);
             rstart_ = get<uint64_t>((size_t)gseg + 2);
             quantile_ok_ = direct_fb_ == CAPS_SA_FB_NONE && local_ && KPG_ >= 2 && KPG_ <= BUCKET_LDS && m2_ >= 8 * NB_ && m2_ <= (1ull << 31) &&
@@ -523,6 +524,7 @@
     const void* last_send_sa_ = nullptr;
     bool force64_ = false;
     uint8_t* gshift_ = nullptr;
+    uint64_t* gbase_ = nullptr;
     uint64_t *gkey_ = nullptr, *dstat_ = nullptr;
     uint16_t* glut_ = nullptr;
     idx_t* dcur_ = nullptr;
@@ -585,7 +587,7 @@
         }
         CAPS_LAUNCH(split_lut_kernel, (SPLIT_LUT_CELLS + 256) / 256, 256, be_, (const uint64_t*)gkey_, K1_ - 1, glut_, dflag + 1);
         be_.memset(dcur_, 0, (size_t)n_streams_ * sizeof(idx_t));
-        if (key_bits_ == 32) CAPS_LAUNCH(group_shift_kernel, (K1_ + 255) / 256, 256, be_, (const uint64_t*)gkey_, K1_, gshift_);
+        if (key_bits_ == 32) CAPS_LAUNCH(group_shift_kernel, (K1_ + 255) / 256, 256, be_, (const uint64_t*)gkey_, K1_, gshift_, gbase_);
         const uint32_t tile_first = local_ ? 0u : (uint32_t)rank_, tile_stride = local_ ? 1u : (uint32_t)world_;
         const uint32_t keep_lo = local_ ? own_lo_ : 0u, keep_hi = local_ ? own_hi_ : K1_;
         a0_ = be_.record();
@@ -593,12 +595,12 @@
             CAPS_LAUNCH((group_scatter_kernel<idx_t, BITS, uint32_t>), my_tiles_, TILE_NT, be_, (const uint32_t*)P_, packed_words(n_, BITS),
                         (uint64_t)0, n_, (const uint64_t*)gkey_, K1_, (const uint16_t*)glut_, (const uint32_t*)(dflag + 1), SUB_, capA_, dcur_,
                         static_cast<uint32_t*>(d_send_keys), static_cast<idx_t*>(d_send_sa), tile_first, tile_stride,
-                        rs, rc, (const uint8_t*)gshift_, keep_lo, keep_hi);
+                        rs, rc, (const uint8_t*)gshift_, (const uint64_t*)gbase_, keep_lo, keep_hi);
         else if (my_tiles_)
             CAPS_LAUNCH((group_scatter_kernel<idx_t, BITS>), my_tiles_, TILE_NT, be_, (const uint32_t*)P_, packed_words(n_, BITS), (uint64_t)0,
                         n_, (const uint64_t*)gkey_, K1_, (const uint16_t*)glut_, (const uint32_t*)(dflag + 1), SUB_, capA_, dcur_,
                         static_cast<uint64_t*>(d_send_keys), static_cast<idx_t*>(d_send_sa), tile_first, tile_stride,
-                        rs, rc, (const uint8_t*)nullptr, keep_lo, keep_hi);
+                        rs, rc, (const uint8_t*)nullptr, (const uint64_t*)nullptr, keep_lo, keep_hi);
         a1_ = be_.record();
         level_a_ran_ = true;
     }
@@ -628,7 +630,7 @@
         o.bnd.last_sa = bk_.last_sa;
         o.slot_stats = slot_stats_;
         o.speculate = std::getenv("CAPS_SA_NO_SLOTS") == nullptr;
-        if (key_bits_ == 32) { o.k32 = true; o.range_mode = 2; o.gshift = gshift_; o.speculate = true; }
+        if (key_bits_ == 32) { o.k32 = true; o.range_mode = 2; o.gshift = gshift_; o.gbase = gbase_; o.speculate = true; }
         if (defer && bk_.fcount) {
             o.defer_flags = bk_.fcount;
             o.run_tables = &seg1_;
@@ -756,6 +758,7 @@
         k.fcount = get<uint64_t>((size_t)EQ_FINE * k.nb_cap);
         k.gfirst = get<uint32_t>(k.nb_cap);
         k.kshift = get<uint8_t>(k.nb_cap);
+        k.kbase = get<uint64_t>(k.nb_cap);
         k.skip = get<uint8_t>(k.nb_cap);
         k.run_list = get<uint64_t>(1 + 4 * RUN_BUCKET_MAX);
         return k;
diff --git a/caps-sa_amd/csrc/text.h b/caps-sa_amd/csrc/text.h
--- a/caps-sa_amd/csrc/text.h
+++ b/caps-sa_amd/csrc/text.h
@@ -139,18 +139,19 @@
     return deep_lcp<BITS, RUNS>(P, n, a, b, TextTraits<BITS>::KCH, RUNS && block_period<BITS>(ka) != 0);
 }
 
-HD uint32_t key32_of(uint64_t key, uint32_t cs) { return (uint32_t)((key << cs) >> 32); }
-
-template <int BITS, bool RUNS = false>
-HD uint64_t pair_lcp32(const uint32_t* __restrict__ P, uint64_t n, uint32_t ka, uint64_t a, uint32_t kb, uint64_t b, uint32_t cs)
-{
-    const uint32_t x = ka ^ kb;
-    if (x) {
-        const uint64_t maxlen = n - (a > b ? a : b);
-        const uint64_t l = (cs + (uint32_t)__builtin_clz(x)) / BITS;
-        return l < maxlen ? l : maxlen;
-    }
-    return deep_lcp<BITS, RUNS>(P, n, a, b, (cs + 32u) / BITS);
+HD uint32_t key32_shift(uint64_t lo, uint64_t hi)
+{
+    uint32_t s = 0;
+    while ((hi >> s) - (lo >> s) > 0xFFFFFFFFull) ++s;
+    return s;
+}
+HD uint32_t key32_of(uint64_t key, uint32_t s, uint32_t base_lo32) { return (uint32_t)(key >> s) - base_lo32; }
+
+template <int BITS>
+HD uint32_t key32_lcp(uint32_t ka, uint32_t kb, uint32_t s, uint64_t base)
+{
+    const uint64_t x = (base + ka) ^ (base + kb);
+    return ((uint32_t)caps_clz64(x) - s) / BITS;
 }
 
 template <int BITS, bool RUNS = true>
@@ -185,13 +186,14 @@
 }
 
 template <int BITS>
-HD uint32_t tie_order_lcp_bounded(const uint32_t* __restrict__ P, uint64_t n, uint64_t a, uint64_t b, uint32_t& lcp)
+HD uint32_t tie_order_lcp_bounded(const uint32_t* __restrict__ P, uint64_t n, uint64_t a, uint64_t b, uint32_t& lcp,
+                                  uint32_t from = TextTraits<BITS>::KCH)
 {
     constexpr uint32_t KCH = TextTraits<BITS>::KCH;
     lcp = 0;
     if (a >= n || b >= n) return a > b ? 1u : 0u;
     const uint64_t maxlen = n - (a > b ? a : b);
-    uint64_t l = KCH;
+    uint64_t l = from;
     for (uint32_t k = 0; k < TIE_WINDOWS / 2 && l < maxlen; ++k, l += 2 * KCH) {
         const bool more = l + KCH < maxlen;
         const uint64_t l1 = more ? l + KCH : l;
```
